# MakiseChris666/MVXNet-Makise

Hardware: AMD Instinct MI355X
Metric: KITTI frames/sec (voxelize+VFE+fusion+3Dconv fwd+bwd) (higher is better)
Workload: dtype f32 (bf16x6: three bf16 pieces = the f32 operand exactly, six MFMAs per product, f32 accumulate); 1 GPU; S2 ring frames (64-beam model, KITTI-like occupancy), 120000 raw pts -> 20000 pts after crop, grid 10x352x400, T=35, 4 frames/GPU/step: crop+cropToSight+lidar2Img, voxelize, fusion sampling+MLP, VFE, reindex+CML fwd+bwd, all-reduce, AdamW; convmath=bf16x6; mode=hot, frames_per_gpu=4, parallelism=dp1

## Files before the change

include/mvx_hip.h:

```cpp
#ifndef MVX_HIP_H
#define MVX_HIP_H
#include <stddef.h>
#include <stdint.h>

#ifdef __cplusplus
extern "C" {
#endif

#define MVX_STATS_REPLICAS 32

#define MVX_FLAG_RELU 1
#define MVX_FLAG_PREZEROED 2
#define MVX_FLAG_ACCUMULATE 4
#define MVX_FLAG_CONV2D 8
#define MVX_FLAG_TAPS2 16
#define MVX_FLAG_BG_TAPS 32
#define MVX_FLAG_SPLIT 64

#define MVX_FLAG_SPLIT3 128

#define MVX_FLAG_PRE_XCD_STRIPS 4096
#define MVX_FLAG_SPLIT_F16 512

#define MVX_FLAG_AMAX_COARSE 1024

#define MVX_FLAG_NO_BG_FILL 2048

#define MVX_OK 0
#define MVX_EINVAL (-1)
#define MVX_ESIZE (-2)

#define MVX_MAX_FRAMES 16
#define MVX_ROWS_SINGLE 0
#define MVX_ROWS_FUSION 1
#define MVX_ROWS_VFE 2
#define MVX_ROWS_VOXELS 3
#define MVX_ROWS_GRID 4
#define MVX_ROWS_REAL 5
typedef struct {
    int32_t n_frames;
    int32_t t;
    int32_t real_off[MVX_MAX_FRAMES + 1];
    int32_t vox_off[MVX_MAX_FRAMES + 1];
} mvx_frames_t;

int mvx_abi_version(void);
#define MVX_TUNE_SPLIT16_MIN_UNITS 1
#define MVX_TUNE_GATHER_NARROW_MAX_UNITS 2
#define MVX_TUNE_ROWGEMM_K128 3
int mvx_tuning_set(int32_t key, int64_t value);

int mvx_split_operand_amax(const float *amax_a, const float *amax_b);
int mvx_tensor_amax(const float *x, int64_t n, float *amax, int32_t flags, void *stream);
#define MVX_STATUS_F16_WEIGHT_RANGE 8
int mvx_split_f16_weight_check(const float *w, int64_t n, int32_t *status, void *stream);
uint64_t mvx_launch_count(void);

size_t mvx_voxelize_workspace_bytes(int32_t n_frames, int32_t cap_points);

int mvx_voxelize(const float *pcd, const int32_t *perm, const int32_t *n_points,
                 const int32_t *ext_idx, int32_t n_frames, int32_t cap_points, int32_t ncol,
                 double lo_x, double lo_y, double lo_z,
                 double size_x, double size_y, double size_z,
                 int32_t T, int32_t out_channels, int32_t cap_voxels,
                 float *voxels, int64_t *coords, int32_t *counts, int32_t *n_voxels,
                 int32_t *status, void *workspace, size_t workspace_bytes, void *stream);
int mvx_voxelize_frames(const float *pcd, const int32_t *perm, const int32_t *n_points,
                        const int32_t *ext_idx, int32_t n_frames, int32_t cap_points, int32_t ncol,
                        double lo_x, double lo_y, double lo_z,
                        double size_x, double size_y, double size_z,
                        int32_t T, int32_t out_channels, int32_t cap_voxels, int32_t concat,
                        float *voxels, int64_t *coords, int32_t *counts, int32_t *n_voxels, int32_t *vox_off,
                        int32_t *status, void *workspace, size_t workspace_bytes, void *stream);

int mvx_scatter_voxels(const float *feat, const int64_t *coords, float *grid, int32_t n_voxels,
                       int32_t channels, int32_t d, int32_t h, int32_t w, int32_t zero_grid,
                       int32_t *status, int32_t *occupancy, int32_t tile_h, int32_t tile_w,
                       uint32_t *site_bits, void *stream);
int mvx_gather_voxels(const float *grid, const int64_t *coords, float *feat, int32_t n_voxels,
// ... 219 lines not shown
                                            int32_t part, int32_t nparts, int64_t *part_rows, void *stream);
int mvx_vfe_bn_max_concat_frames(const float *y, const float *mean_inv, float *out, int32_t *argmax, int32_t n_voxels,
                                 int32_t t, int32_t channels, const int32_t *voff, const int32_t *vcnt, int32_t n_real,
                                 const mvx_frames_t *frames_host, void *stream);
int mvx_bn_segment_max_frames(const float *y, const float *mean_inv, float *out, int32_t *argmax, int32_t n_voxels,
                              int32_t t, int32_t channels, const int32_t *voff, const int32_t *vcnt, int32_t n_real,
                              const mvx_frames_t *frames_host, void *stream);
int mvx_voxel_row_offsets_frames(const int32_t *row_map, int32_t n_voxels, int32_t t, int32_t n_real, int32_t *voff,
                                 int32_t *vcnt, float *row_w, float *fusion_row_w, const mvx_frames_t *frames_host,
                                 void *stream);
int mvx_vfe_compact_input_frames(const float *voxels, int32_t vox_channels, const int32_t *rows_sel, const float *imfeat,
                                 int32_t feat_channels, int32_t n_real, int32_t n_voxels, float *out,
                                 const mvx_frames_t *frames_host, void *stream);
int mvx_vfe_compact_input_pitch_frames(const float *voxels, int32_t vox_channels, const int32_t *rows_sel, const float *imfeat,
                                       int32_t feat_channels, int32_t n_real, int32_t n_voxels, float *out, int32_t ld,
                                       const mvx_frames_t *frames_host, void *stream);
int mvx_vfe_compact_input_backward_frames(const float *grad_out, int32_t feat_channels, int32_t n_real, int32_t n_voxels,
                                          float *dimfeat, double *scratch, const mvx_frames_t *frames_host, void *stream);
int mvx_row_compact_map_frames(float *voxels, int32_t vox_channels, int64_t rows, int32_t *row_map, int32_t *rows_sel,
                               int32_t *n_real, void *workspace, size_t workspace_bytes, const mvx_frames_t *frames_host,
                               int32_t *real_off, void *stream);
int mvx_feature_sample_rows_frames(const float *voxels, int32_t vox_channels, const int32_t *rows_sel, int32_t n_real,
                                   const float *const *feats_host, const int32_t *feat_hw_host, int32_t n_levels,
                                   int32_t channels, float imsize_h, float imsize_w, float eps, float *out, int32_t *status,
                                   const mvx_frames_t *frames_host,
                                   float *out_amax , void *stream);
int mvx_feature_sample_rows_planes_frames(const float *voxels, int32_t vox_channels, const int32_t *rows_sel, int32_t n_real,
                                          const float *const *feats_host, const int32_t *feat_hw_host, int32_t n_levels,
                                          int32_t channels, float imsize_h, float imsize_w, float eps, float *out, int32_t *status,
                                          const mvx_frames_t *frames_host, float *out_amax, void *planes, int64_t plane_rows,
                                          void *stream);
size_t mvx_index_grid_bytes_frames(int32_t d, int32_t h, int32_t w, int32_t n_frames);
int mvx_index_grid_frames(const int64_t *coords, int32_t n_voxels, int32_t d, int32_t h, int32_t w, int32_t *grid,
                          int32_t *status, const mvx_frames_t *frames_host, void *stream);
int mvx_sparse_conv_output_frames(const float *p, const int32_t *index_grid, const float *bias, float *out, double *stats,
                                  int32_t din, int32_t dout, int32_t h, int32_t w, int32_t cout, int32_t stride_d,
                                  int32_t pad_d, int32_t flags, int32_t n_frames, void *stream);
int mvx_sparse_conv_output_tiles_frames(const float *p, const int32_t *index_grid, const float *bias, float *out, double *stats,
                                        int32_t din, int32_t dout, int32_t h, int32_t w, int32_t cout, int32_t stride_d,
                                        int32_t pad_d, int32_t flags, int32_t n_frames, const int32_t *tile_flags, void *stream);
int mvx_sparse_conv_gather_dz_frames(const float *dz, const int64_t *coords, int32_t n_voxels, float *g_rows, int32_t din,
                                     int32_t dout, int32_t h, int32_t w, int32_t cout, int32_t stride_d, int32_t pad_d,
                                     const mvx_frames_t *frames_host, void *stream);
int mvx_activity_dilate_frames(const void *src, int32_t src_is_index, int32_t din, int32_t dout, int32_t h, int32_t w,
                               int32_t stride_d, int32_t pad_d, int32_t mark_border, uint8_t *dst_mask,
                               int32_t *dst_halo_flags, int32_t *dst_tile_flags, int32_t n_frames, void *stream);
int mvx_tile_dilate_flags_frames(const int32_t *in_tile_flags, const int32_t *self_tile_flags, int32_t din, int32_t dout,
                                 int32_t h, int32_t w, int32_t stride_d, int32_t pad_d, int32_t *out_tile_flags,
                                 int32_t n_frames, void *stream);
int mvx_conv3d_background_frames(const float *w, const float *c_in, int32_t din, int32_t dout, int32_t cin, int32_t cout,
                                 int32_t stride_d, int32_t pad_d, float *bg_pre, int32_t n_frames, void *stream);
int mvx_bn_background_frames(const float *bg_pre, const float *bias, const float *mean_inv, int32_t planes, int32_t channels,
                             int32_t flags, float *y_bg, float *c_out, int32_t n_frames, void *stream);
int mvx_conv3d_forward_bg_frames(const float *in, const float *wpk, const float *bias, float *out, double *stats,
                                 int32_t din, int32_t dout, int32_t h, int32_t w, int32_t cin, int32_t cout,
                                 int32_t stride_d, int32_t pad_d, int32_t flags, const int32_t *in_halo_flags,
                                 const uint8_t *out_mask, const float *bg_pre, int32_t border_active, uint64_t *exec_stages,
                                 uint32_t *done_counter, double count, double eps, float *mean_inv, uint32_t *work_counter,
                                 int32_t n_frames, void *stream);
int mvx_conv3d_dgrad_tiles_frames(const float *dz, const float *wpk_dgrad, float *dx, int32_t din, int32_t dout, int32_t h,
                                  int32_t w, int32_t cin, int32_t cout, int32_t stride_d, int32_t pad_d,
                                  const int32_t *dx_tile_flags, uint64_t *exec_stages, uint32_t *work_counter,
                                  int32_t n_frames, void *stream);
int mvx_conv3d_input_grad_sums_frames(const float *w, const float *tap_sums, int32_t din, int32_t dout, int32_t cin,
                                      int32_t cout, int32_t stride_d, int32_t pad_d, float *plane_grad_sums,
                                      int32_t n_frames, void *stream);
size_t mvx_conv3d_wgrad_bg_workspace_bytes_frames(int32_t dout, int32_t h, int32_t w, int32_t cin, int32_t cout,
                                                  int32_t n_frames);
int mvx_conv3d_wgrad_bg_frames(const float *in, const float *dz, float *dw, int32_t din, int32_t dout, int32_t h, int32_t w,
                               int32_t cin, int32_t cout, int32_t stride_d, int32_t pad_d, int32_t flags,
                               const int32_t *in_halo_flags, const float *c_in, const float *tap_sums, void *workspace,
                               size_t workspace_bytes, int32_t n_frames, void *stream);
size_t mvx_bn_relu_backward_tiles_workspace_bytes_frames(int32_t planes, int32_t h, int32_t w, int32_t channels,
                                                         int32_t n_frames);
int mvx_bn_relu_backward_tiles_frames(const float *dyhat, const float *y, const float *mean_inv, const float *c_bg,
                                      const float *y_bg, const float *plane_grad_sums, const int32_t *tile_flags,
                                      int32_t planes, int32_t h, int32_t w, int32_t channels, float *dz, float *dbias,
                                      float *dz_inactive_sums, float *dz_amax ,
                                      int32_t flags, void *workspace, size_t workspace_bytes, int32_t n_frames, void *stream);
int mvx_cl_to_bev_frames(const float *cl, float *bev, int32_t d, int32_t h, int32_t w, int32_t channels, int32_t reverse,
                         int32_t n_frames, void *stream);
int mvx_bev_to_cl_broadcast(const float *bev, float *cl, int32_t d, int32_t h, int32_t w, int32_t channels, int32_t copies,
                            void *stream);

int mvx_conv2d_forward_frames(const float *in, const float *wpk, const float *bias, float *out, double *stats, int32_t h,
                              int32_t w, int32_t cin, int32_t cout, int32_t flags, uint32_t *done_counter, double eps,
                              float *mean_inv, uint32_t *work_counter, int32_t n_frames, void *stream);
int mvx_conv2d_dgrad_frames(const float *dz, const float *wpk_dgrad, float *dx, int32_t h, int32_t w, int32_t cin,
                            int32_t cout, int32_t flags, uint32_t *work_counter, int32_t n_frames, void *stream);
size_t mvx_conv2d_wgrad_workspace_bytes_frames(int32_t h, int32_t w, int32_t cin, int32_t cout, int32_t n_frames);
int mvx_conv2d_wgrad_frames(const float *in, const float *dz, float *dw, int32_t h, int32_t w, int32_t cin, int32_t cout,
                            int32_t flags, void *workspace, size_t workspace_bytes, int32_t n_frames, void *stream);
int mvx_space_to_depth_frames(const float *in, float *out, int32_t n_frames, int32_t planes, int32_t h, int32_t w,
                              int32_t channels, int32_t reverse, void *stream);
int mvx_d2s_bn_apply_frames(float *t, const float *mean_inv, float *out, int32_t n_frames, int32_t h, int32_t w, int32_t s,
                            int32_t channels, int32_t ld_out, int32_t col_offset, int32_t reverse, void *stream);
int mvx_bn_apply_strided_frames(float *y, const float *mean_inv, float *out, int64_t rows, int32_t channels, int32_t ld_out,
                                int32_t col_offset, int32_t n_frames, int32_t reverse, void *stream);
int mvx_row_stats_frames(const float *y, double *stats, int64_t rows, int32_t channels, int32_t n_frames, void *stream);

int mvx_bbox_pairwise(const float *boxes1, int32_t n1, const float *boxes2, int32_t n2, int32_t want_iou, float *out,
                      void *stream);
size_t mvx_classify_anchors_workspace_bytes(int32_t n_gt, int32_t anchors_per_loc, int32_t window_radius);
int mvx_classify_anchors(const float *gts, int32_t n_gt, const float *anchors, int32_t l, int32_t w,
                         int32_t anchors_per_loc, const int64_t *nls, const int64_t *nws, float neg_thr, float pos_thr,
                         int32_t window_radius, int64_t *pos_idx, int64_t *neg_idx, int64_t *gi, int64_t cap,
                         int32_t *counts, int32_t *status, void *workspace, size_t workspace_bytes, void *stream);
int mvx_classify_anchors_frames(const float *gts, const int32_t *gt_off_host, int32_t n_frames, const float *anchors, int32_t l,
                                int32_t w, int32_t anchors_per_loc, const int64_t *nls, const int64_t *nws, float neg_thr,
                                float pos_thr, int32_t window_radius, int64_t *pos_idx, int64_t *neg_idx, int64_t *gi,
                                int64_t cap, int32_t *counts, int32_t *status, void *workspace, size_t workspace_bytes,
                                void *stream);
size_t mvx_assign_anchors_frames_workspace_bytes(int32_t n_gt_total, int32_t n_frames, int32_t l, int32_t w,
                                                 int32_t anchors_per_loc);
int mvx_assign_anchors_frames(const float *gts, const int32_t *gt_off_host, int32_t n_frames, const float *anchors, int32_t l,
                              int32_t w, int32_t anchors_per_loc, float neg_thr, float pos_thr, float force_thr,
                              int32_t window_radius, int64_t *pos_idx, int64_t *neg_idx, int64_t *gi, int64_t cap,
                              int32_t *counts, float *gt_best, int32_t *status, void *workspace, size_t workspace_bytes,
                              void *stream);
int mvx_box_point_counts_frames(const float *points6, int32_t n_frames, int32_t cap_points, int32_t ld, const int32_t *n_points,
                                const float *boxes, const int32_t *gt_off, int32_t n_boxes_total, int32_t *counts, void *stream);
size_t mvx_ignore_anchors_frames_workspace_bytes(int32_t n_frames, int32_t l, int32_t w, int32_t anchors_per_loc);
int mvx_ignore_anchors_frames(const int64_t *pos_idx, const int64_t *neg_idx, const int64_t *gi, int64_t cap,
                              const int32_t *counts, int32_t n_frames, const int32_t *gt_off, const int32_t *gt_points,
                              int32_t min_points, const float *anchors, const float *anchor_quads, int32_t l, int32_t w,
// ... 160 lines not shown
```

mvxnet-makise_amd/csrc/activity.hip:

```cpp
#include "common.h"
#include "quad.h"

namespace {

constexpr int ATH = QTH, ATW = QTW;

__global__ void activity_sites(const void *__restrict__ src, int src_is_index, int Din, int Dout, int H, int W, int sd,
                               int pd, int mark_border, unsigned char *__restrict__ dst, int n_frames) {
    const size_t n = (size_t)n_frames * Dout * H * W;
    for (size_t e = blockIdx.x * (size_t)blockDim.x + threadIdx.x; e < n; e += (size_t)gridDim.x * blockDim.x) {
        const int x = (int)(e % W), y = (int)((e / W) % H), d = (int)(e / ((size_t)W * H));
        int on = mark_border && (y == 0 || y == H - 1 || x == 0 || x == W - 1);
        for (int kd = 0; kd < 3 && !on; ++kd) {
            const int ds = mvx_src_plane(d, Din, Dout, sd, pd, kd);
            if (ds < 0) continue;
            for (int a = -1; a <= 1 && !on; ++a) {
                const int yy = y + a;
                if (yy < 0 || yy >= H) continue;
                for (int b = -1; b <= 1; ++b) {
                    const int xx = x + b;
                    if (xx < 0 || xx >= W) continue;
                    const size_t s = ((size_t)ds * H + yy) * W + xx;
                    on |= src_is_index ? (((const int *)src)[s] >= 0) : (((const unsigned char *)src)[s] != 0);
                }
// ... 34 lines not shown
                } else {
                    const unsigned char *row = (const unsigned char *)src + s;
                    const unsigned v = *(const unsigned *)row;
                    m = ((v & 0xffu) ? 2u : 0u) | ((v & 0xff00u) ? 4u : 0u) | ((v & 0xff0000u) ? 8u : 0u) | ((v & 0xff000000u) ? 16u : 0u);
                    if (x > 0 && row[-1]) m |= 1u;
                    if (x + 4 < W && row[4]) m |= 32u;
                }
                on |= (m | (m >> 1) | (m >> 2)) & 15u;
            }
        }
        *(unsigned *)(dst + e * 4) = ((on & 1u) ? 1u : 0u) | ((on & 2u) ? 0x100u : 0u) | ((on & 4u) ? 0x10000u : 0u) | ((on & 8u) ? 0x1000000u : 0u);
    }
}

__global__ __launch_bounds__(256) void activity_halo_flags(const unsigned char *__restrict__ mask, int D, int H, int W,
                                                           int *__restrict__ flags, int *__restrict__ tile_flags) {
    const int tiles_x = (W + ATW - 1) / ATW;
    const int tx0 = (blockIdx.x % tiles_x) * ATW - 1, ty0 = (blockIdx.x / tiles_x) * ATH - 1;
    const int d = blockIdx.y;
    int on = 0, inner = 0;
    if (threadIdx.x < (ATH + 2) * (ATW + 2)) {
        const int hy = threadIdx.x / (ATW + 2), hx = threadIdx.x % (ATW + 2);
        const int y = ty0 + hy, x = tx0 + hx;
        if (y >= 0 && y < H && x >= 0 && x < W) on = mask[((size_t)d * H + y) * W + x];
        inner = on && hy >= 1 && hy <= ATH && hx >= 1 && hx <= ATW;
    }
    on = __syncthreads_or(on);
    inner = __syncthreads_or(inner);
    if (threadIdx.x == 0) {
        if (flags) flags[(size_t)d * gridDim.x + blockIdx.x] = on ? 1 : 0;
        if (tile_flags) tile_flags[(size_t)d * gridDim.x + blockIdx.x] = inner ? 1 : 0;
    }
}

__global__ void tile_dilate_flags(const int *__restrict__ in, const int *__restrict__ self, int Din, int Dout, int tiles_y,
                                  int tiles_x, int sd, int pd, int *__restrict__ out, int n_frames) {
    const int e = blockIdx.x * blockDim.x + threadIdx.x;
    const int nt = tiles_y * tiles_x;
    if (e >= n_frames * Dout * nt) return;
    const int d = e / nt, t = e - d * nt, ty = t / tiles_x, tx = t - ty * tiles_x;
    int on = self ? self[e] : 0;
    for (int kd = 0; kd < 3 && !on; ++kd) {
        const int ds = mvx_src_plane(d, Din, Dout, sd, pd, kd);
        if (ds < 0) continue;
        for (int a = -1; a <= 1 && !on; ++a)
            for (int b = -1; b <= 1; ++b) {
                const int yy = ty + a, xx = tx + b;
                if (yy >= 0 && yy < tiles_y && xx >= 0 && xx < tiles_x) on |= in[(size_t)ds * nt + yy * tiles_x + xx];
            }
    }
    out[e] = on ? 1 : 0;
}

__global__ __launch_bounds__(64) void conv_background(const float *__restrict__ w, const float *__restrict__ c_in, int Din,
                                                      int Dout, int Cin, int Cout, int sd, int pd,
                                                      float *__restrict__ bg_pre, float *__restrict__ bg_tap,
                                                      float *__restrict__ bg_cls) {
    const int n = blockIdx.x, d = blockIdx.y;
    double s = 0.0;
    double cls[9];
#pragma unroll
    for (int q = 0; q < 9; ++q) cls[q] = 0.0;
    for (int kd = 0; kd < 3; ++kd) {
        const int ds = mvx_src_plane(d, Din, Dout, sd, pd, kd);
        double sk = 0.0;
        if (ds >= 0)
            for (int e = threadIdx.x; e < Cin * 9; e += 64) {
                const int c = e / 9, k = e - c * 9, a = k / 3, b = k - a * 3;
                const double t = (double)w[(((size_t)n * Cin + c) * 3 + kd) * 9 + k] * (double)c_in[(size_t)ds * Cin + c];
                sk += t;
                if (bg_cls) {
#pragma unroll
                    for (int q = 0; q < 9; ++q) {
                        const int ry = q / 3, rx = q - ry * 3;
                        const bool inside = !(ry == 0 && a == 0) && !(ry == 2 && a == 2) && !(rx == 0 && b == 0) && !(rx == 2 && b == 2);
                        if (inside) cls[q] += t;
                    }
                }
            }
        s += sk;
        if (bg_tap) {
            sk = wave_sum_f64(sk);
            if (threadIdx.x == 0) bg_tap[((size_t)d * 3 + kd) * Cout + n] = (float)sk;
        }
    }
    s = wave_sum_f64(s);
    if (threadIdx.x == 0) bg_pre[(size_t)d * Cout + n] = (float)s;
    if (bg_cls) {
#pragma unroll
        for (int q = 0; q < 9; ++q) {
            const double v = wave_sum_f64(cls[q]);
            if (threadIdx.x == 0) bg_cls[((size_t)d * 9 + q) * Cout + n] = (float)v;
        }
    }
}

__global__ void bn_background(const float *__restrict__ bg_pre, const float *__restrict__ bias, const float *__restrict__ mi,
                              int D, int C, int relu, float *__restrict__ y_bg, float *__restrict__ c_out, int n_frames) {
    const int e = blockIdx.x * blockDim.x + threadIdx.x;
    if (e >= n_frames * D * C) return;
    const int c = e % C;
    mi += (size_t)(e / (D * C)) * 2 * C;
    float v = (bg_pre ? bg_pre[e] : 0.f) + (bias ? bias[c] : 0.f);
    if (relu) v = fmaxf(v, 0.f);
    if (y_bg) y_bg[e] = v;
    c_out[e] = (v - mi[c]) * mi[C + c];
}

__global__ __launch_bounds__(256) void bn_apply_tiles(const float *__restrict__ y, const float *__restrict__ mi,
                                                      const float *__restrict__ c_bg, const int *__restrict__ tile_flags,
                                                      float *__restrict__ out, int D, int H, int W, int C, int ntiles,
                                                      const int *__restrict__ read_flags) {
    const int t = blockIdx.x, d = blockIdx.y, frame = d / D;
    if (read_flags && !read_flags[(size_t)d * ntiles + t] && !tile_flags[(size_t)d * ntiles + t]) return;
    const TileThreads tt(C, t, W);
    const bool on = tile_flags[(size_t)d * ntiles + t] != 0;
    const float4 cb = ld4(c_bg + (size_t)d * C + tt.ct * 4);
    const float *fmi = mi + (size_t)frame * 2 * C;
    const float4 m = ld4(fmi + tt.ct * 4), iv = ld4(fmi + C + tt.ct * 4);
    tt.for_each_site([&](int, int gy, int gx) {
        if (gy >= H || gx >= W) return;
        const size_t off = (((size_t)d * H + gy) * W + gx) * C + tt.ct * 4;
        st4(out + off, on ? bn4(ld4(y + off), m, iv) : cb);
    });
}

__global__ void tile_read_flags(const int *__restrict__ hflag, int Din, int Dout, int ty_n, int tx_n, int sd, int pd,
                                int *__restrict__ read, int n_frames) {
    const int ntiles = ty_n * tx_n;
    const long long e = blockIdx.x * (long long)blockDim.x + threadIdx.x;
    if (e >= (long long)n_frames * Din * ntiles) return;
    const int p = (int)(e / ntiles), t = (int)(e - (long long)p * ntiles);
    const int ty = t / tx_n, tx = t - ty * tx_n;
    int r = 0;
    for (int kd = 0; kd < 3 && !r; ++kd) {
        const int d = mvx_dst_plane(p, Din, Dout, sd, pd, kd);
        if (d < 0) continue;
        for (int y = max(ty - 1, 0); y <= min(ty + 1, ty_n - 1) && !r; ++y)
            for (int x = max(tx - 1, 0); x <= min(tx + 1, tx_n - 1) && !r; ++x) {
                const int y0 = y & ~1, y1 = min(y0 + 1, ty_n - 1);
                const bool border = x == 0 || x == tx_n - 1 || y0 == 0 || y1 == ty_n - 1;
                int c = border ? 1 : 0;
                for (int k2 = 0; k2 < 3 && !c; ++k2) {
                    const int ds = mvx_src_plane(d, Din, Dout, sd, pd, k2);
                    if (ds >= 0) c = hflag[(size_t)ds * ntiles + y0 * tx_n + x] | hflag[(size_t)ds * ntiles + y1 * tx_n + x];
// ... 276 lines not shown
    MVX_CHECK_ARG(n_frames >= 1 && n_frames <= MVX_MAX_FRAMES);
    hipStream_t st = (hipStream_t)stream;
    const size_t n = (size_t)n_frames * dout * h * w;
    if (w % 4 == 0 && ((uintptr_t)src & 15) == 0 && ((uintptr_t)dst_mask & 3) == 0)
        hipLaunchKernelGGL(activity_sites4, dim3(mvx_cdiv(n / 4, 256) > 4096 ? 4096 : mvx_cdiv(n / 4, 256)), dim3(256), 0, st, src,
                           src_is_index, din, dout, h, w, stride_d, pad_d, mark_border, dst_mask, n_frames);
    else
        hipLaunchKernelGGL(activity_sites, dim3(mvx_cdiv(n, 256) > 4096 ? 4096 : mvx_cdiv(n, 256)), dim3(256), 0, st, src,
                           src_is_index, din, dout, h, w, stride_d, pad_d, mark_border, dst_mask, n_frames);
    MVX_LAUNCH_CHECK();
    if (dst_halo_flags || dst_tile_flags) {
        hipLaunchKernelGGL(activity_halo_flags, dim3(mvx_cdiv(w, ATW) * mvx_cdiv(h, ATH), dout * n_frames), dim3(256), 0, st,
                           (const unsigned char *)dst_mask, dout * n_frames, h, w, dst_halo_flags, dst_tile_flags);
        MVX_LAUNCH_CHECK();
    }
    return MVX_OK;
}

extern "C" int mvx_activity_dilate(const void *src, int32_t src_is_index, int32_t din, int32_t dout, int32_t h, int32_t w,
                                   int32_t stride_d, int32_t pad_d, int32_t mark_border, uint8_t *dst_mask,
                                   int32_t *dst_halo_flags, int32_t *dst_tile_flags, void *stream) {
    return mvx_activity_dilate_frames(src, src_is_index, din, dout, h, w, stride_d, pad_d, mark_border, dst_mask,
                                      dst_halo_flags, dst_tile_flags, 1, stream);
}

extern "C" int mvx_tile_dilate_flags_frames(const int32_t *in_tile_flags, const int32_t *self_tile_flags, int32_t din,
                                            int32_t dout, int32_t h, int32_t w, int32_t stride_d, int32_t pad_d,
                                            int32_t *out_tile_flags, int32_t n_frames, void *stream) {
    MVX_CHECK_ARG(in_tile_flags && out_tile_flags && din > 0 && dout > 0 && h > 0 && w > 0);
    MVX_CHECK_ARG(n_frames >= 1 && n_frames <= MVX_MAX_FRAMES);
    MVX_CHECK_ARG(stride_d >= 1 && stride_d <= 2 && pad_d >= 0 && pad_d <= 1);
    MVX_CHECK_ARG(dout == (din + 2 * pad_d - 3) / stride_d + 1);
    const int ty = (int)mvx_cdiv(h, ATH), tx = (int)mvx_cdiv(w, ATW);
    hipLaunchKernelGGL(tile_dilate_flags, dim3(mvx_cdiv((long long)n_frames * dout * ty * tx, 256)), dim3(256), 0,
                       (hipStream_t)stream, in_tile_flags, self_tile_flags, din, dout, ty, tx, stride_d, pad_d, out_tile_flags,
                       n_frames);
    MVX_LAUNCH_CHECK();
    return MVX_OK;
}

extern "C" int mvx_tile_dilate_flags(const int32_t *in_tile_flags, const int32_t *self_tile_flags, int32_t din, int32_t dout,
                                     int32_t h, int32_t w, int32_t stride_d, int32_t pad_d, int32_t *out_tile_flags,
                                     void *stream) {
    return mvx_tile_dilate_flags_frames(in_tile_flags, self_tile_flags, din, dout, h, w, stride_d, pad_d, out_tile_flags, 1,
                                        stream);
}

extern "C" int mvx_conv3d_background_frames(const float *w, const float *c_in, int32_t din, int32_t dout, int32_t cin,
                                            int32_t cout, int32_t stride_d, int32_t pad_d, float *bg_pre, int32_t n_frames,
                                            void *stream) {
    MVX_CHECK_ARG(w && c_in && bg_pre && din > 0 && dout > 0 && cin > 0 && cout > 0);
    MVX_CHECK_ARG(n_frames >= 1 && n_frames <= MVX_MAX_FRAMES);
    hipLaunchKernelGGL(conv_background, dim3(cout, dout * n_frames), dim3(64), 0, (hipStream_t)stream, w, c_in, din, dout, cin,
                       cout, stride_d, pad_d, bg_pre, (float *)nullptr, (float *)nullptr);
    MVX_LAUNCH_CHECK();
    return MVX_OK;
}

extern "C" int mvx_conv3d_background_taps_frames(const float *w, const float *c_in, int32_t din, int32_t dout, int32_t cin,
                                                 int32_t cout, int32_t stride_d, int32_t pad_d, float *bg, int32_t n_frames,
                                                 void *stream) {
    MVX_CHECK_ARG(w && c_in && bg && din > 0 && dout > 0 && cin > 0 && cout > 0);
    MVX_CHECK_ARG(n_frames >= 1 && n_frames <= MVX_MAX_FRAMES);
    hipLaunchKernelGGL(conv_background, dim3(cout, dout * n_frames), dim3(64), 0, (hipStream_t)stream, w, c_in, din, dout, cin,
                       cout, stride_d, pad_d, bg, bg + (size_t)dout * n_frames * cout, bg + (size_t)4 * dout * n_frames * cout);
    MVX_LAUNCH_CHECK();
    return MVX_OK;
}

extern "C" int mvx_conv3d_background(const float *w, const float *c_in, int32_t din, int32_t dout, int32_t cin,
                                     int32_t cout, int32_t stride_d, int32_t pad_d, float *bg_pre, void *stream) {
    return mvx_conv3d_background_frames(w, c_in, din, dout, cin, cout, stride_d, pad_d, bg_pre, 1, stream);
}

extern "C" int mvx_bn_background_frames(const float *bg_pre, const float *bias, const float *mean_inv, int32_t planes,
                                        int32_t channels, int32_t flags, float *y_bg, float *c_out, int32_t n_frames,
                                        void *stream) {
    MVX_CHECK_ARG(mean_inv && c_out && planes > 0 && channels > 0 && n_frames >= 1 && n_frames <= MVX_MAX_FRAMES);
    hipLaunchKernelGGL(bn_background, dim3(mvx_cdiv((long long)n_frames * planes * channels, 256)), dim3(256), 0,
                       (hipStream_t)stream, bg_pre, bias, mean_inv, planes, channels, flags & MVX_FLAG_RELU, y_bg, c_out, n_frames);
    MVX_LAUNCH_CHECK();
    return MVX_OK;
}

extern "C" int mvx_bn_apply_tiles_frames(const float *y, const float *mean_inv, const float *c_bg, const int32_t *tile_flags,
                                         float *out, int32_t planes, int32_t h, int32_t w, int32_t channels, int32_t n_frames,
                                         void *stream) {
    MVX_CHECK_ARG(y && mean_inv && c_bg && tile_flags && out && planes > 0 && h > 0 && w > 0);
    MVX_CHECK_ARG(channels > 0 && channels % 4 == 0 && channels <= 1024 && 256 % (channels / 4) == 0);
    MVX_CHECK_ARG(n_frames >= 1 && n_frames <= MVX_MAX_FRAMES);
    const int ntiles = (int)(mvx_cdiv(w, ATW) * mvx_cdiv(h, ATH));
    hipLaunchKernelGGL(bn_apply_tiles, dim3(ntiles, planes * n_frames), dim3(256), 0, (hipStream_t)stream, y, mean_inv, c_bg,
                       (const int *)tile_flags, out, planes, h, w, channels, ntiles, (const int *)nullptr);
    MVX_LAUNCH_CHECK();
    return MVX_OK;
}

extern "C" int mvx_bn_apply_tiles_read_frames(const float *y, const float *mean_inv, const float *c_bg, const int32_t *tile_flags,
                                              const int32_t *read_flags, float *out, int32_t planes, int32_t h, int32_t w,
                                              int32_t channels, int32_t n_frames, void *stream) {
    MVX_CHECK_ARG(y && mean_inv && c_bg && tile_flags && read_flags && out && planes > 0 && h > 0 && w > 0);
    MVX_CHECK_ARG(channels > 0 && channels % 4 == 0 && channels <= 1024 && 256 % (channels / 4) == 0);
    MVX_CHECK_ARG(n_frames >= 1 && n_frames <= MVX_MAX_FRAMES);
    const int ntiles = (int)(mvx_cdiv(w, ATW) * mvx_cdiv(h, ATH));
    hipLaunchKernelGGL(bn_apply_tiles, dim3(ntiles, planes * n_frames), dim3(256), 0, (hipStream_t)stream, y, mean_inv, c_bg,
                       (const int *)tile_flags, out, planes, h, w, channels, ntiles, (const int *)read_flags);
    MVX_LAUNCH_CHECK();
    return MVX_OK;
}

extern "C" int mvx_tile_read_flags_frames(const int32_t *in_halo_flags, int32_t din, int32_t dout, int32_t h, int32_t w,
                                          int32_t stride_d, int32_t pad_d, int32_t *read_flags, int32_t n_frames, void *stream) {
    MVX_CHECK_ARG(in_halo_flags && read_flags && din > 0 && dout > 0 && h > 0 && w > 0);
    MVX_CHECK_ARG(n_frames >= 1 && n_frames <= MVX_MAX_FRAMES && stride_d >= 1 && stride_d <= 2 && pad_d >= 0 && pad_d <= 1);
    MVX_CHECK_ARG(dout == (din + 2 * pad_d - 3) / stride_d + 1);
    const int ty = (int)mvx_cdiv(h, ATH), tx = (int)mvx_cdiv(w, ATW);
    hipLaunchKernelGGL(tile_read_flags, dim3(mvx_cdiv((long long)n_frames * din * ty * tx, 256)), dim3(256), 0, (hipStream_t)stream,
                       (const int *)in_halo_flags, din, dout, ty, tx, stride_d, pad_d, (int *)read_flags, n_frames);
// ... 22 lines not shown
```

mvxnet-makise_amd/csrc/conv3d.hip:

```cpp
#include "common.h"
#include "conv_kernels.h"

namespace {

#ifdef MVX_GATHER_STAMPS
__device__ unsigned long long g_stamps[256];
__device__ int g_stamp_unit[3] = {0, 0, 0};
__device__ volatile int g_stamp_wg = -1;
#define MVX_STAMP(k)                                                                                       \
    do {                                                                                                   \
        if (stamped && threadIdx.x == 0 && (k) < 256) g_stamps[(k)] = __builtin_amdgcn_s_memtime();        \
    } while (0)
#else
#define MVX_STAMP(k) do { } while (0)
#endif

constexpr int PITCH = BK + 4;

__global__ void pack_weights(const float *__restrict__ w, float *__restrict__ wpk, int Co, int Ci, int dgrad, int src2d) {
    const int K = dgrad ? Co : Ci, N = dgrad ? Ci : Co;
    const int nch = K / BK;
    const long long total = 27ll * K * N;
    for (long long e = blockIdx.x * (long long)blockDim.x + threadIdx.x; e < total;
         e += (long long)gridDim.x * blockDim.x) {
        const int k = (int)(e % BK);
        long long r = e / BK;
        const int n = (int)(r % N); r /= N;
        const int ch = (int)(r % nch); r /= nch;
        const int tap = (int)(r % 9);
        const int kd = (int)(r / 9);
        const int a = tap / 3, b = tap % 3;
        const int kk = ch * BK + k;
        const int co = dgrad ? kk : n, ci = dgrad ? n : kk;
        const int kh = dgrad ? 2 - a : a, kw = dgrad ? 2 - b : b;
        if (src2d) wpk[e] = kd == 1 ? w[(((long long)co * Ci + ci) * 3 + kh) * 3 + kw] : 0.f;
        else wpk[e] = w[((((long long)co * Ci + ci) * 3 + kd) * 3 + kh) * 3 + kw];
    }
}

constexpr int WROW = BN * BK;
constexpr int HROW = ((HW * PITCH + 63) / 64) * 64;

inline dim3 gather_grid(const Geom &g) { return dim3(mvx_cdiv(g.W, TW) * mvx_cdiv(g.H, TH), g.Dout * g.F, g.Cout / BN); }

template <int TLO, int THI, int NB2 = 2>
__device__ __forceinline__ void gather_unit(const int tile, const int d, const int nb, const int ntiles,
                                            float *__restrict__ s_halo, float *__restrict__ s_w, double (*s_red)[2 * BN],
                                            const float *__restrict__ in, const float *__restrict__ wpk,
                                            const float *__restrict__ bias, float *__restrict__ out,
                                            double *__restrict__ stats, const Geom &g, int relu,
                                            const int *__restrict__ in_hflag, const unsigned char *__restrict__ out_mask,
                                            const float *__restrict__ bg_pre, int border_active,
                                            unsigned long long *__restrict__ exec_stages,
                                            const int *__restrict__ only_tiles) {
    const int tiles_x = (g.W + TW - 1) / TW;
    const int tx0 = (tile % tiles_x) * TW, ty0 = (tile / tiles_x) * TH;
    const int tid = threadIdx.x, lane = tid & 63, wv = tid >> 6;
    const int li = lane & 31, lh = lane >> 5;
    const int nchunks = g.Cin / BK;
    constexpr int BNW = 32 * NB2;
    if (only_tiles && !only_tiles[(size_t)d * ntiles + tile]) return;

    f32x16 acc[1][2];
    f32x16 &acc0 = acc[0][0], &acc1 = acc[0][1];
#pragma unroll
    for (int r = 0; r < 16; ++r) { acc0[r] = 0.f; acc1[r] = 0.f; }

    const int my_ty = 2 * wv + (li >> 4), my_tx = li & 15;
    const int a_base = my_ty * HROW + my_tx * PITCH + 4 * lh;
    const int wkey = (li >> 1) & 7;
    int b_off[BK / 8];
#pragma unroll
    for (int q = 0; q < BK / 8; ++q) b_off[q] = li * BK + 4 * (((2 * q) | lh) ^ wkey);

    const bool on_border = tx0 == 0 || ty0 == 0 || tx0 + TW >= g.W || ty0 + TH >= g.H;
    const TilePlan plan = tile_plan<1>(g, d, on_border, in_hflag, border_active, ntiles, tile, tile);
    const bool active = plan.active;
    const int nstages = plan.nk * nchunks;

    if (exec_stages && active && threadIdx.x == 0 && (NB2 == 2 || !(nb & 1))) atomicAdd(exec_stages, (unsigned long long)nstages);
    if (active && nstages > 0) {

    int h_off[6];
    int h_lds[6];
#pragma unroll
    for (int u = 0; u < 6; ++u) {
        const int c = tid + 256 * u;
        h_off[u] = -1;
        h_lds[u] = -1;
        if (c < HH * HW * 8) {
            const int r = c >> 3, part = c & 7;
            const int ry = r / HW, rx = r - ry * HW;
            const int gy = ty0 - 1 + ry, gx = tx0 - 1 + rx;
            h_lds[u] = ry * HROW + rx * PITCH + part * 4;
            if (gy >= 0 && gy < g.H && gx >= 0 && gx < g.W) h_off[u] = (gy * g.W + gx) * g.Cin + part * 4;
        }
    }
    f32x4 hreg[6], wreg[6];
    auto load_halo = [&](int st) __attribute__((always_inline)) {
        int kd, ds, cc;
        plan_stage(plan, nchunks, st, kd, ds, cc);
        const float *img = in + (size_t)ds * g.H * g.W * g.Cin + cc * BK;
#pragma unroll
        for (int u = 0; u < 6; ++u)
            hreg[u] = h_off[u] >= 0 ? *(const f32x4 *)(img + h_off[u]) : f32x4{0.f, 0.f, 0.f, 0.f};
    };
    auto store_halo = [&]() __attribute__((always_inline)) {
#pragma unroll
        for (int u = 0; u < 6; ++u)
            if (h_lds[u] >= 0) *(f32x4 *)(s_halo + h_lds[u]) = hreg[u];
    };
    auto load_wrow = [&](int st, int row) __attribute__((always_inline)) {
        int kd, ds, cc;
        plan_stage(plan, nchunks, st, kd, ds, cc);
        const float *row0 = wpk + ((((size_t)kd * 9 + row * 3) * nchunks + cc) * g.Cout + (size_t)nb * BNW) * BK + (size_t)tid * 4;
        const size_t tap_stride = (size_t)nchunks * g.Cout * BK;
        if (NB2 == 2) {
#pragma unroll
            for (int v = 0; v < 6; ++v) wreg[v] = *(const f32x4 *)(row0 + (v >> 1) * tap_stride + (v & 1) * 1024);
        } else {
#pragma unroll
            for (int v = 0; v < 3; ++v) wreg[v] = *(const f32x4 *)(row0 + v * tap_stride);
        }
    };
    auto store_wrow = [&]() __attribute__((always_inline)) {
        if (NB2 == 2) {
#pragma unroll
            for (int v = 0; v < 6; ++v) {
// ... 595 lines not shown
    for (int kind = 0; kind < RK; ++kind) {
        const bool need = kind == 0 || (kind == 1 && ty0 == 0) || (kind == 2 && ty0 + TH >= H) || (kind == 3 && tx0 == 0) ||
                          (kind == 4 && tx0 + TW >= W) || (kind == 5 && ty0 == 0 && tx0 == 0) ||
                          (kind == 6 && ty0 == 0 && tx0 + TW >= W) || (kind == 7 && ty0 + TH >= H && tx0 == 0) ||
                          (kind == 8 && ty0 + TH >= H && tx0 + TW >= W);
        if (!need) continue;
        float4 s = make_float4(0.f, 0.f, 0.f, 0.f);
        for (int sidx = st; sidx < TH * TW; sidx += spb) {
            const int gy = ty0 + sidx / TW, gx = tx0 + sidx % TW;
            if (gy >= H || gx >= W) continue;
            const bool top = gy == 0, bot = gy == H - 1, lef = gx == 0, rig = gx == W - 1;
            const bool in = kind == 0 || (kind == 1 && top) || (kind == 2 && bot) || (kind == 3 && lef) || (kind == 4 && rig) ||
                            (kind == 5 && top && lef) || (kind == 6 && top && rig) || (kind == 7 && bot && lef) ||
                            (kind == 8 && bot && rig);
            if (!in) continue;
            const float4 v = *(const float4 *)(dz + (((size_t)d * H + gy) * W + gx) * C + ct * 4);
            s.x += v.x; s.y += v.y; s.z += v.z; s.w += v.w;
        }
        __syncthreads();
        red[threadIdx.x][0] = s.x; red[threadIdx.x][1] = s.y; red[threadIdx.x][2] = s.z; red[threadIdx.x][3] = s.w;
        __syncthreads();
        if (st == 0)
            for (int j = 0; j < 4; ++j) {
                double tt = 0.0;
                for (int q = 0; q < spb; ++q) tt += (double)red[q * c4n + ct][j];
                atomicAdd(Rp + (size_t)kind * C + ct * 4 + j, tt);
            }
    }
}

__global__ void region_tap_sums(const double *__restrict__ R, const float *__restrict__ extra_total, int D, int C,
                                float *__restrict__ T) {
    const int e = blockIdx.x * blockDim.x + threadIdx.x;
    if (e >= D * 9 * C) return;
    const int n = e % C, tap = (e / C) % 9, d = e / (9 * C);
    const int a = tap / 3, b = tap % 3;
    double k[RK];
    for (int q = 0; q < RK; ++q) {
        double t = 0.0;
        for (int rep = 0; rep < RREP; ++rep) t += R[(((size_t)rep * D + d) * RK + q) * C + n];
        k[q] = t;
    }
    if (extra_total) k[0] += (double)extra_total[(size_t)d * C + n];
    double t = k[0];
    if (a == 0) t -= k[1];
    if (a == 2) t -= k[2];
    if (b == 0) t -= k[3];
    if (b == 2) t -= k[4];
    if (a == 0 && b == 0) t += k[5];
    if (a == 0 && b == 2) t += k[6];
    if (a == 2 && b == 0) t += k[7];
    if (a == 2 && b == 2) t += k[8];
    T[e] = (float)t;
}

__global__ void wgrad_rank1(const float *__restrict__ T, const float *__restrict__ c_in, float *__restrict__ dw, Geom g) {
    const size_t total = (size_t)27 * g.Cin * g.Cout;
    for (size_t e = blockIdx.x * (size_t)blockDim.x + threadIdx.x; e < total; e += (size_t)gridDim.x * blockDim.x) {
        const int tap = (int)(e % 9), kd = (int)((e / 9) % 3);
        const int ci = (int)((e / 27) % g.Cin), co = (int)(e / ((size_t)27 * g.Cin));
        float s = 0.f;
        for (int d = 0; d < g.Dout * g.F; ++d) {
            const int ds = mvx_src_plane(d, g.Din, g.Dout, g.sd, g.pd, kd);
            if (ds < 0) continue;
            s += c_in[(size_t)ds * g.Cin + ci] * T[((size_t)d * 9 + tap) * g.Cout + co];
        }
        dw[e] += s;
    }
}

__global__ void wgrad_reduce(const float *__restrict__ slabs, float *__restrict__ dw, int nstrips, int Ci, int accumulate,
                             int dst2d, Strips ks, int zero_block) {
    const size_t per = (size_t)27 * Ci * BN;
    slabs += (size_t)blockIdx.y * nstrips * per;
    dw += (size_t)blockIdx.y * (dst2d ? per / 3 : per);
    for (size_t e = blockIdx.x * (size_t)blockDim.x + threadIdx.x; e < per; e += (size_t)gridDim.x * blockDim.x) {
        const int co = (int)(e % BN);
        size_t r = e / BN;
        const int ci = (int)(r % Ci); r /= Ci;
        const int tap = (int)(r % 9);
        const int kd = (int)(r / 9);
        const int nkd = kd == 0 ? ks.n[0] : (kd == 1 ? ks.n[1] : ks.n[2]);
        const int nk = nkd < nstrips ? nkd : nstrips;
        float s = 0.f;
        for (int k = 0; k < nk; ++k) s += slabs[(size_t)k * per + e];
        if (dst2d && kd != 1) continue;
        if (zero_block > 0) {
            const int ta = tap / 3, tb = tap % 3;
            if (ta > 1 || tb > 1 || !((s2d_tap_mask(ci / zero_block) >> (ta * 2 + tb)) & 1u)) s = 0.f;
        }
        float *dst = dst2d ? dw + (((size_t)co * Ci + ci) * 3 + tap / 3) * 3 + tap % 3
                           : dw + ((((size_t)co * Ci + ci) * 3 + kd) * 3 + tap / 3) * 3 + tap % 3;
        *dst = accumulate ? *dst + s : s;
    }
}

__global__ __launch_bounds__(64) void input_grad_sums(const float *__restrict__ w, const float *__restrict__ T, Geom g,
                                                      float *__restrict__ A) {
    const int c = blockIdx.x, d = blockIdx.y;
    double s = 0.0;
    for (int kd = 0; kd < 3; ++kd) {
        const int dp = mvx_dst_plane(d, g.Din, g.Dout, g.sd, g.pd, kd);
        if (dp < 0) continue;
        for (int e = threadIdx.x; e < g.Cout * 9; e += 64) {
            const int n = e / 9, k = e - n * 9;
            s += (double)w[(((size_t)n * g.Cin + c) * 3 + kd) * 9 + k] * (double)T[((size_t)dp * 9 + k) * g.Cout + n];
// ... 51 lines not shown
                               (int)grid.x, (int)grid.y, (int)grid.z);                                                            \
        else                                                                                                                     \
            hipLaunchKernelGGL((conv3d_gather_pf<TLO, THI, NB2>), grid, dim3(256), 0, st, a.in, wpk, a.bias, a.out, a.stats, g,   \
                               a.relu, a.in_hflag, a.out_mask, a.bg_pre, a.border_active, a.exec_stages, a.only_tiles,            \
                               a.done_counter, a.fin_count, a.fin_eps, a.fin_mean_inv);                                           \
    } while (0)
#define MVX_LAUNCH_GATHER(TLO, THI)                                                                                              \
    do {                                                                                                                         \
        if (narrow) MVX_LAUNCH_GATHER_N(TLO, THI, 1);                                                                            \
        else MVX_LAUNCH_GATHER_N(TLO, THI, 2);                                                                                   \
    } while (0)
    if (g.tap_lo == 0 && g.tap_hi == 3) MVX_LAUNCH_GATHER(0, 3);
    else if (g.tap_lo == 0 && g.tap_hi == 2) MVX_LAUNCH_GATHER(0, 2);
    else MVX_LAUNCH_GATHER(1, 3);
#undef MVX_LAUNCH_GATHER
#undef MVX_LAUNCH_GATHER_N
}

extern "C" void mvx_conv3d_tile_shape(int32_t *tile_h, int32_t *tile_w) {
    if (tile_h) *tile_h = TH;
    if (tile_w) *tile_w = TW;
}

extern "C" int mvx_conv3d_forward(const float *in, const float *wpk, const float *bias, float *out,
                                  double *stats, int32_t din, int32_t dout, int32_t h, int32_t w,
                                  int32_t cin, int32_t cout, int32_t stride_d, int32_t pad_d,
                                  int32_t flags, uint32_t *work_counter, void *stream) {
    MVX_CHECK_ARG(in && wpk && out);
    int rc = conv_check_forward(din, dout, h, w, cin, cout, stride_d, pad_d);
    if (rc) return rc;
    hipStream_t st = (hipStream_t)stream;
    hipError_t e = conv_zero_stats(stats, nullptr, cout, 1, flags, st);
    if (e != hipSuccess) return (int)e;
    Geom g{din, dout, h, w, cin, cout, stride_d, pad_d, 0};
    GatherArgs a;
    a.in = in; a.bias = bias; a.out = out; a.stats = stats; a.relu = flags & MVX_FLAG_RELU;
    a.work_counter = (unsigned *)work_counter;
    launch_gather(st, g, wpk, a);
    MVX_LAUNCH_CHECK();
    return MVX_OK;
}

extern "C" int mvx_conv3d_forward_bg_frames(const float *in, const float *wpk, const float *bias, float *out, double *stats,
                                            int32_t din, int32_t dout, int32_t h, int32_t w, int32_t cin, int32_t cout,
                                            int32_t stride_d, int32_t pad_d, int32_t flags, const int32_t *in_halo_flags,
                                            const uint8_t *out_mask, const float *bg_pre, int32_t border_active,
                                            uint64_t *exec_stages, uint32_t *done_counter, double count, double eps,
                                            float *mean_inv, uint32_t *work_counter, int32_t n_frames, void *stream) {
    MVX_CHECK_ARG(in && wpk && out && in_halo_flags && out_mask && bg_pre);
    int rc = conv_check_forward(din, dout, h, w, cin, cout, stride_d, pad_d);
    if (rc) return rc;
    if ((rc = conv_check_frames(n_frames))) return rc;
    MVX_CHECK_ARG(!done_counter || (stats && mean_inv && count > 0));
    hipStream_t st = (hipStream_t)stream;
    hipError_t e = conv_zero_stats(stats, done_counter, cout, n_frames, flags, st);
    if (e != hipSuccess) return (int)e;
    Geom g{din, dout, h, w, cin, cout, stride_d, pad_d, 0, n_frames};
    GatherArgs a;
    a.in = in; a.bias = bias; a.out = out; a.stats = stats; a.relu = flags & MVX_FLAG_RELU;
    a.in_hflag = in_halo_flags; a.out_mask = out_mask; a.bg_pre = bg_pre;
    a.border_active = (border_active ? 1 : 0) | ((flags & MVX_FLAG_BG_TAPS) ? 2 : 0);
    a.exec_stages = (unsigned long long *)exec_stages;
    a.done_counter = (unsigned *)done_counter; a.fin_count = count; a.fin_eps = eps; a.fin_mean_inv = mean_inv;
    a.work_counter = (unsigned *)work_counter;
    launch_gather(st, g, wpk, a);
    MVX_LAUNCH_CHECK();
    return MVX_OK;
}

extern "C" int mvx_conv3d_forward_bg(const float *in, const float *wpk, const float *bias, float *out, double *stats,
                                     int32_t din, int32_t dout, int32_t h, int32_t w, int32_t cin, int32_t cout,
                                     int32_t stride_d, int32_t pad_d, int32_t flags, const int32_t *in_halo_flags,
                                     const uint8_t *out_mask, const float *bg_pre, int32_t border_active,
                                     uint64_t *exec_stages, uint32_t *done_counter, double count, double eps,
                                     float *mean_inv, uint32_t *work_counter, void *stream) {
    return mvx_conv3d_forward_bg_frames(in, wpk, bias, out, stats, din, dout, h, w, cin, cout, stride_d, pad_d, flags,
                                        in_halo_flags, out_mask, bg_pre, border_active, exec_stages, done_counter, count, eps,
                                        mean_inv, work_counter, 1, stream);
}

static int launch_dgrad(const float *dz, const float *wpk_dgrad, float *dx, int32_t din, int32_t dout, int32_t h,
                        int32_t w, int32_t cin, int32_t cout, int32_t stride_d, int32_t pad_d, const int32_t *only_tiles,
                        uint64_t *exec_stages, uint32_t *work_counter, void *stream, int32_t n_frames = 1, int32_t flags = 0) {
    MVX_CHECK_ARG(dz && wpk_dgrad && dx);
    int rc = conv_check_frames(n_frames);
    if (rc) return rc;
    if ((rc = conv_check_geom(din, dout, h, w, cout, cin, stride_d, pad_d))) return rc;
    Geom g{dout, din, h, w, cout, cin, stride_d, pad_d, 1, n_frames};
    conv_set_taps2(g, flags, CONV_INPUT_GRAD, BN);
    GatherArgs a;
    a.in = dz; a.out = dx; a.only_tiles = only_tiles; a.exec_stages = (unsigned long long *)exec_stages;
    a.work_counter = (unsigned *)work_counter;
    launch_gather((hipStream_t)stream, g, wpk_dgrad, a);
    MVX_LAUNCH_CHECK();
    return MVX_OK;
}

extern "C" int mvx_conv3d_dgrad(const float *dz, const float *wpk_dgrad, float *dx, int32_t din,
                                int32_t dout, int32_t h, int32_t w, int32_t cin, int32_t cout,
                                int32_t stride_d, int32_t pad_d, uint32_t *work_counter, void *stream) {
    return launch_dgrad(dz, wpk_dgrad, dx, din, dout, h, w, cin, cout, stride_d, pad_d, nullptr, nullptr, work_counter, stream);
}

extern "C" int mvx_conv3d_dgrad_tiles(const float *dz, const float *wpk_dgrad, float *dx, int32_t din, int32_t dout,
                                      int32_t h, int32_t w, int32_t cin, int32_t cout, int32_t stride_d, int32_t pad_d,
                                      const int32_t *dx_tile_flags, uint64_t *exec_stages, uint32_t *work_counter,
                                      void *stream) {
    MVX_CHECK_ARG(dx_tile_flags);
    return launch_dgrad(dz, wpk_dgrad, dx, din, dout, h, w, cin, cout, stride_d, pad_d, dx_tile_flags, exec_stages,
                        work_counter, stream);
}

extern "C" int mvx_conv3d_dgrad_tiles_frames(const float *dz, const float *wpk_dgrad, float *dx, int32_t din, int32_t dout,
                                             int32_t h, int32_t w, int32_t cin, int32_t cout, int32_t stride_d, int32_t pad_d,
// ... 33 lines not shown
    const int per = wgrad_strips(h, w, cin);
    const int nstrips = (conv_ntiles(h, w) + per - 1) / per;
    MVX_CHECK_ARG(workspace_bytes >= mvx_conv3d_wgrad_workspace_bytes(h, w, cin, cout));
    Geom g{din, dout, h, w, cin, cout, stride_d, pad_d, 0};
    hipStream_t st = (hipStream_t)stream;
    if (cin % W4_C == 0)
        launch_wgrad4<false>(flags, dim3(nstrips, 3 * (cin / W4_C), nblk), st, in, dz, (float *)workspace, g, per, nullptr, nullptr,
                             nullptr, Strips{{nstrips, nstrips, nstrips}}, am);
    else
        hipLaunchKernelGGL(conv3d_wgrad, dim3(nstrips, 3 * (cin / BK)), dim3(WG_THREADS), 0, st, in, dz,
                           (float *)workspace, g, per);
    MVX_LAUNCH_CHECK();
    const size_t per_slab = (size_t)27 * cin * BN;
    hipLaunchKernelGGL(wgrad_reduce, dim3(mvx_cdiv(per_slab, 256), nblk), dim3(256), 0, st, (const float *)workspace, dw,
                       nstrips, cin, flags & MVX_FLAG_ACCUMULATE, (flags & MVX_FLAG_CONV2D) ? 1 : 0,
                       Strips{{nstrips, nstrips, nstrips}}, 0);
    MVX_LAUNCH_CHECK();
    return MVX_OK;
}

static int wgrad_bg_strips(int cin) {
    const int s = 128 / (cin / W4_C);
    return s < 1 ? 1 : s;
}
static size_t wgrad_bg_slab_bytes(int cin) { return (size_t)wgrad_bg_strips(cin) * 27 * cin * BN * sizeof(float); }

extern "C" size_t mvx_plane_tap_sums_workspace_bytes(int32_t planes, int32_t channels) {
    return planes > 0 && channels > 0 ? sizeof(double) * RREP * planes * RK * channels : 0;
}

extern "C" int mvx_plane_tap_sums(const float *dz, int32_t planes, int32_t h, int32_t w, int32_t channels,
                                  const int32_t *tile_flags, const float *inactive_sums, float *tap_sums,
                                  void *workspace, size_t workspace_bytes, void *stream) {
    MVX_CHECK_ARG(dz && tap_sums && workspace && planes > 0 && h > 0 && w > 0 && channels > 0);
    MVX_CHECK_ARG(channels % 4 == 0 && 256 % (channels / 4) == 0);
    MVX_CHECK_ARG((tile_flags == nullptr) == (inactive_sums == nullptr));
    MVX_CHECK_ARG(workspace_bytes >= mvx_plane_tap_sums_workspace_bytes(planes, channels));
    hipStream_t st = (hipStream_t)stream;
    double *R = (double *)workspace;
    hipError_t e = hipMemsetAsync(R, 0, sizeof(double) * RREP * planes * RK * channels, st);
    if (e != hipSuccess) return (int)e;
    if (tile_flags)
        hipLaunchKernelGGL(plane_region_sums_tiles, dim3(conv_ntiles(h, w), planes), dim3(256), 0, st, dz,
                           tile_flags, planes, h, w, channels, R);
    else
        hipLaunchKernelGGL(plane_region_sums, dim3(h, planes), dim3(256), 0, st, dz, planes, h, w, channels, R);
    MVX_LAUNCH_CHECK();
    hipLaunchKernelGGL(region_tap_sums, dim3(mvx_cdiv((long long)planes * 9 * channels, 64)), dim3(64), 0, st,
                       (const double *)R, inactive_sums, planes, channels, tap_sums);
    MVX_LAUNCH_CHECK();
    return MVX_OK;
}

extern "C" int mvx_conv3d_input_grad_sums_frames(const float *w, const float *tap_sums, int32_t din, int32_t dout, int32_t cin,
                                                 int32_t cout, int32_t stride_d, int32_t pad_d, float *plane_grad_sums,
                                                 int32_t n_frames, void *stream) {
    MVX_CHECK_ARG(w && tap_sums && plane_grad_sums && din > 0 && dout > 0 && cin > 0 && cout > 0);
    if (int rc = conv_check_frames(n_frames)) return rc;
    Geom g{din, dout, 0, 0, cin, cout, stride_d, pad_d, 0, n_frames};
    hipLaunchKernelGGL(input_grad_sums, dim3(cin, din * n_frames), dim3(64), 0, (hipStream_t)stream, w, tap_sums, g,
                       plane_grad_sums);
    MVX_LAUNCH_CHECK();
    return MVX_OK;
}

extern "C" int mvx_conv3d_input_grad_sums(const float *w, const float *tap_sums, int32_t din, int32_t dout, int32_t cin,
                                          int32_t cout, int32_t stride_d, int32_t pad_d, float *plane_grad_sums,
                                          void *stream) {
    return mvx_conv3d_input_grad_sums_frames(w, tap_sums, din, dout, cin, cout, stride_d, pad_d, plane_grad_sums, 1, stream);
}

extern "C" size_t mvx_conv3d_wgrad_bg_workspace_bytes_frames(int32_t dout, int32_t h, int32_t w, int32_t cin, int32_t cout,
                                                            int32_t n_frames) {
    if (dout <= 0 || h <= 0 || w <= 0 || cin <= 0 || cout != BN || cin % W4_C || n_frames <= 0) return 0;
    return conv_carve_wgrad(nullptr, wgrad_bg_slab_bytes(cin), dout * n_frames, conv_ntiles(h, w), false).bytes;
}

extern "C" size_t mvx_conv3d_wgrad_bg_workspace_bytes(int32_t dout, int32_t h, int32_t w, int32_t cin, int32_t cout) {
    return mvx_conv3d_wgrad_bg_workspace_bytes_frames(dout, h, w, cin, cout, 1);
}

extern "C" int mvx_conv3d_wgrad_bg_frames(const float *in, const float *dz, float *dw, int32_t din, int32_t dout, int32_t h,
                                          int32_t w, int32_t cin, int32_t cout, int32_t stride_d, int32_t pad_d, int32_t flags,
                                          const int32_t *in_halo_flags, const float *c_in, const float *tap_sums,
                                          void *workspace, size_t workspace_bytes, int32_t n_frames, void *stream) {
    const SplitAmax am = mvxi_take_split_amax();
    MVX_CHECK_ARG(in && dz && dw && workspace && in_halo_flags && c_in && tap_sums);
    int rc = conv_check_geom(din, dout, h, w, cin, cout, stride_d, pad_d);
    if (rc) return rc;
    if (cout != BN || cin % W4_C) return MVX_ESIZE;
    if ((rc = conv_check_frames(n_frames))) return rc;
    const int ntiles = conv_ntiles(h, w);
    const WgradWorkspace ws = conv_carve_wgrad(workspace, wgrad_bg_slab_bytes(cin), dout * n_frames, ntiles, false);
    MVX_CHECK_ARG(workspace_bytes >= ws.bytes);
    const int nstrips = wgrad_bg_strips(cin);
    Geom g{din, dout, h, w, cin, cout, stride_d, pad_d, 0, n_frames};
    hipStream_t st = (hipStream_t)stream;
    int nd[3], ndsum = 0;
    for (int kd = 0; kd < 3; ++kd) {
        nd[kd] = 0;
        for (int d = 0; d < dout; ++d) {
            const int ds = d * stride_d - pad_d + kd;
            nd[kd] += ds >= 0 && ds < din;
        }
        ndsum += nd[kd];
    }
    Strips ks;
    int widest = 1;
    for (int kd = 0; kd < 3; ++kd) {
        int share = ndsum > 0 ? (2 * nstrips * nd[kd]) / ndsum : nstrips;
        if (share < 1) share = 1;
        if (share > nstrips) share = nstrips;
        ks.n[kd] = share;
        if (share > widest) widest = share;
    }
    hipLaunchKernelGGL(wgrad_step_list, dim3(3), dim3(1024), 0, st, in_halo_flags, g, ntiles, ws.list, ws.count);
    MVX_LAUNCH_CHECK();
    launch_wgrad4<false>(flags, dim3(widest, 3 * (cin / W4_C)), st, in, dz, ws.slabs, g, 0, ws.list, ws.count, c_in, ks, am);
    MVX_LAUNCH_CHECK();
    const size_t per_slab = (size_t)27 * cin * BN;
    hipLaunchKernelGGL(wgrad_reduce, dim3(mvx_cdiv(per_slab, 256)), dim3(256), 0, st, (const float *)ws.slabs, dw, widest, cin,
                       flags & MVX_FLAG_ACCUMULATE, 0, ks, 0);
    MVX_LAUNCH_CHECK();
    hipLaunchKernelGGL(wgrad_rank1, dim3(mvx_cdiv(per_slab, 256)), dim3(256), 0, st, tap_sums, c_in, dw, g);
    MVX_LAUNCH_CHECK();
    return MVX_OK;
}

extern "C" int mvx_conv3d_wgrad_bg(const float *in, const float *dz, float *dw, int32_t din, int32_t dout, int32_t h,
                                   int32_t w, int32_t cin, int32_t cout, int32_t stride_d, int32_t pad_d, int32_t flags,
                                   const int32_t *in_halo_flags, const float *c_in, const float *tap_sums,
                                   void *workspace, size_t workspace_bytes, void *stream) {
    return mvx_conv3d_wgrad_bg_frames(in, dz, dw, din, dout, h, w, cin, cout, stride_d, pad_d, flags, in_halo_flags, c_in,
                                      tap_sums, workspace, workspace_bytes, 1, stream);
}

extern "C" int mvx_conv2d_forward_frames(const float *in, const float *wpk, const float *bias, float *out, double *stats,
                                         int32_t h, int32_t w, int32_t cin, int32_t cout, int32_t flags,
                                         uint32_t *done_counter, double eps, float *mean_inv, uint32_t *work_counter,
                                         int32_t n_frames, void *stream) {
    MVX_CHECK_ARG(in && wpk && out);
    int rc = conv_check_frames(n_frames);
    if (rc) return rc;
    if ((rc = conv_check_geom(1, 1, h, w, cin, cout, 1, 1))) return rc;
    MVX_CHECK_ARG(!done_counter || (stats && mean_inv));
    hipStream_t st = (hipStream_t)stream;
    hipError_t e = conv_zero_stats(stats, done_counter, cout, n_frames, flags, st);
    if (e != hipSuccess) return (int)e;
    Geom g{1, 1, h, w, cin, cout, 1, 1, 0, n_frames};
    conv_set_taps2(g, flags, CONV_FORWARD, BK);
    GatherArgs a;
    a.in = in; a.bias = bias; a.out = out; a.stats = stats; a.relu = flags & MVX_FLAG_RELU;
    a.done_counter = (unsigned *)done_counter; a.fin_count = (double)h * w; a.fin_eps = eps; a.fin_mean_inv = mean_inv;
    a.work_counter = (unsigned *)work_counter;
    launch_gather(st, g, wpk, a);
    MVX_LAUNCH_CHECK();
    return MVX_OK;
}

extern "C" int mvx_conv2d_dgrad_frames(const float *dz, const float *wpk_dgrad, float *dx, int32_t h, int32_t w, int32_t cin,
                                       int32_t cout, int32_t flags, uint32_t *work_counter, int32_t n_frames, void *stream) {
    return launch_dgrad(dz, wpk_dgrad, dx, 1, 1, h, w, cin, cout, 1, 1, nullptr, nullptr, work_counter, stream, n_frames, flags);
}

static int conv2d_wgrad_strips(int cin, int cout) {
    int s = 256 / ((cin / W4_C) * (cout / BN));
    if (s > 128) s = 128;
    return s < 1 ? 1 : s;
}

static size_t conv2d_wgrad_slab_bytes(int cin, int cout) {
    return (size_t)(cout / BN) * conv2d_wgrad_strips(cin, cout) * 27 * cin * BN * sizeof(float);
}

extern "C" size_t mvx_conv2d_wgrad_workspace_bytes_frames(int32_t h, int32_t w, int32_t cin, int32_t cout, int32_t n_frames) {
    if (h <= 0 || w <= 0 || cin <= 0 || cout <= 0 || cin % W4_C || cout % BN || n_frames <= 0) return 0;
    return conv_carve_wgrad(nullptr, conv2d_wgrad_slab_bytes(cin, cout), n_frames, conv_ntiles(h, w), true).bytes;
}

// ... 37 lines not shown
```

mvxnet-makise_amd/csrc/conv3d_split.hip:

```cpp
#include "common.h"
#include "conv_kernels.h"
#include "rowgemm_common.h"

namespace {

constexpr int TH2 = 16;

__global__ void pack_weights_split(const float *__restrict__ w, unsigned short *__restrict__ wsp, int Co, int Ci, int dgrad, int np, int fmt) {
    const int K = dgrad ? Co : Ci, N = dgrad ? Ci : Co;
    const int nch = K / BK;
    const long long total = 27ll * K * N;
    for (long long e = blockIdx.x * (long long)blockDim.x + threadIdx.x; e < total; e += (long long)gridDim.x * blockDim.x) {
        const int k = (int)(e % BK);
        long long r = e / BK;
        const int n = (int)(r % N); r /= N;
        const int ch = (int)(r % nch); r /= nch;
        const int tap = (int)(r % 9);
        const int kd = (int)(r / 9);
        const int a = tap / 3, b = tap % 3;
        const int kk = ch * BK + k;
        const int co = dgrad ? kk : n, ci = dgrad ? n : kk;
        const int kh = dgrad ? 2 - a : a, kw = dgrad ? 2 - b : b;
        float x = w[((((long long)co * Ci + ci) * 3 + kd) * 3 + kh) * 3 + kw];
        const long long row = (((long long)kd * 9 + tap) * nch + ch) * N + n;
        for (int q = 0; q < np; ++q) {
            if (fmt == 0) {
                const __bf16 pb = (__bf16)x;
                wsp[(row * np + q) * BK + k] = __builtin_bit_cast(unsigned short, pb);
                x -= (float)pb;
            } else {
                if (q == 0) x *= SPLIT_F16_WSCALE;
                const _Float16 pb = (_Float16)x;
                wsp[(row * np + q) * BK + k] = __builtin_bit_cast(unsigned short, pb);
                x -= (float)pb;
            }
        }
    }
}

template <int NP, int BKT, int MT, bool WIN, int FMT>
__global__ __launch_bounds__(256, 2) void conv3d_gather_splitT(const float *__restrict__ in,
                                                               const unsigned short *__restrict__ wsp,
                                                               const float *__restrict__ bias,
                                                               float *__restrict__ out, double *__restrict__ stats,
                                                               Geom g, int relu, const int *__restrict__ in_hflag,
                                                               const unsigned char *__restrict__ out_mask,
                                                               const float *__restrict__ bg_pre, int border_active,
                                                               const int *__restrict__ only_tiles,
                                                               unsigned long long *__restrict__ exec_stages,
                                                               const float *__restrict__ in_amax) {
    float a_scale = 1.f;
    if constexpr (FMT == 1) a_scale = split_scale_of(in_amax);
    constexpr int THT = TH * MT, HHT = THT + 2;
    constexpr int ROWBT = NP * BKT * 2 + 16;
    constexpr int HROW = (HW * ROWBT + 255) / 256 * 256;
    constexpr int PPR = NP * BKT / 8;
    constexpr int PT = BN * PPR;
    constexpr int NWU = (3 * PT + 255) / 256;
    constexpr int PARTS = BKT / 4;
    constexpr int NH = (HHT * HW * PARTS + 255) / 256;
    constexpr int KS = BKT / 16;
    __shared__ __attribute__((aligned(256))) unsigned char s_halo[HHT * HROW];
    __shared__ __attribute__((aligned(16))) unsigned char s_w[3][BN * ROWBT];
    __shared__ float s_red[4][2 * BN];
    const int tiles_x = (g.W + TW - 1) / TW, tiles_y8 = (g.H + TH - 1) / TH;
    const int ntiles8 = tiles_x * tiles_y8;
    const int tx = blockIdx.x % tiles_x, tyb = blockIdx.x / tiles_x;
    const int tx0 = tx * TW, ty0 = tyb * THT;
    const int t_top = (MT * tyb) * tiles_x + tx;
    const bool has_bot = MT == 2 && 2 * tyb + 1 < tiles_y8;
    const int t_bot = has_bot ? t_top + tiles_x : t_top;
    const int d = blockIdx.y, nb = blockIdx.z;
    const int tid = threadIdx.x, lane = tid & 63, wv = tid >> 6, li = lane & 31, lh = lane >> 5;
    const int nchunks = g.Cin / BKT;
    if (only_tiles && !(only_tiles[(size_t)d * ntiles8 + t_top] | only_tiles[(size_t)d * ntiles8 + t_bot])) return;
    const bool on_border = tx0 == 0 || ty0 == 0 || tx0 + TW >= g.W || ty0 + THT >= g.H;
    const TilePlan plan = tile_plan<MT>(g, d, on_border, in_hflag, border_active, ntiles8, t_top, t_bot);

    f32x16 acc[MT][2];
#pragma unroll
    for (int m = 0; m < MT; ++m)
#pragma unroll
        for (int n = 0; n < 2; ++n)
#pragma unroll
            for (int r = 0; r < 16; ++r) acc[m][n][r] = 0.f;
    int a_base[MT];
#pragma unroll
    for (int m = 0; m < MT; ++m) a_base[m] = (2 * MT * wv + 2 * m + (li >> 4)) * HROW + (li & 15) * ROWBT + lh * 16;
    const int b_base = li * ROWBT + lh * 16;

    typedef unsigned u32x4 __attribute__((ext_vector_type(4)));
    u32x4 wreg[NWU];
    auto load_w3 = [&](int kd, int a, int cc) __attribute__((always_inline)) {
        const int c32 = (cc * BKT) / BK, half = BKT == 16 ? (cc & 1) : 0;
#pragma unroll
        for (int u = 0; u < NWU; ++u) {
            int c = tid + 256 * u;
            if (3 * PT % 256 && c >= 3 * PT) c = 3 * PT - 1;
            const int t = c / PT, rem = c - t * PT;
            const int n = rem / PPR, piece = rem - n * PPR;
            const int q = piece / (BKT / 8), sub = piece - q * (BKT / 8);
            const unsigned char *row = (const unsigned char *)wsp +
                (((((size_t)kd * 9 + a * 3 + t) * (g.Cin / BK) + c32) * g.Cout + (size_t)nb * BN + n) * NP + q) * (BK * 2);
            wreg[u] = *(const u32x4 *)(row + half * 32 + sub * 16);
        }
    };
    auto store_w3 = [&]() __attribute__((always_inline)) {
#pragma unroll
        for (int u = 0; u < NWU; ++u) {
            const int c = tid + 256 * u;
            if (3 * PT % 256 == 0 || c < 3 * PT) {
                const int t = c / PT, rem = c - t * PT;
                const int n = rem / PPR, piece = rem - n * PPR;
                *(u32x4 *)(s_w[t] + n * ROWBT + piece * 16) = wreg[u];
            }
        }
    };

    const int nstages = plan.active ? plan.nk * nchunks : 0;
    if (exec_stages && nstages > 0 && threadIdx.x == 0)
        atomicAdd(exec_stages, (unsigned long long)(plan.nk * (g.Cin / BK)) * (has_bot ? 2 : 1));
    int h_off[NH], h_lds[NH];
#pragma unroll
    for (int u = 0; u < NH; ++u) {
        const int c = tid + 256 * u;
        h_off[u] = -1;
        h_lds[u] = -1;
        if (c < HHT * HW * PARTS) {
            const int r = c / PARTS, part = c - r * PARTS;
// ... 166 lines not shown
                               a.stats, g, a.relu, a.in_hflag, a.out_mask, a.bg_pre, a.border_active, a.only_tiles,                  \
                               a.exec_stages, am.a);                                                                                 \
    } while (0)
    if (fmt_of(flags)) { if (big) MVX_GO(2, 32, 2, 1); else MVX_GO(2, 32, 1, 1); }
    else if (pieces_of(flags) == 3) { if (big) MVX_GO(3, 16, 2, 0); else MVX_GO(3, 32, 1, 0); }
    else              { if (big) MVX_GO(2, 32, 2, 0); else MVX_GO(2, 32, 1, 0); }
#undef MVX_GO
}

}

extern "C" size_t mvx_conv3d_packed_weight_bytes_split(int32_t cout, int32_t cin, int32_t flags) {
    if (cout <= 0 || cin <= 0) return 0;
    return (size_t)27 * cout * cin * pieces_of(flags) * sizeof(unsigned short);
}

extern "C" int mvx_conv3d_pack_weights_split(const float *w, void *wsplit, int32_t cout, int32_t cin, int32_t for_dgrad,
                                             int32_t flags, void *stream) {
    MVX_CHECK_ARG(w && wsplit && cout > 0 && cin > 0);
    MVX_CHECK_ARG((for_dgrad ? cout : cin) % BK == 0);
    const long long total = 27ll * cout * cin;
    hipLaunchKernelGGL(pack_weights_split, dim3(mvx_cdiv(total, 256) > 2048 ? 2048 : mvx_cdiv(total, 256)), dim3(256), 0,
                       (hipStream_t)stream, w, (unsigned short *)wsplit, cout, cin, for_dgrad, pieces_of(flags), fmt_of(flags));
    MVX_LAUNCH_CHECK();
    return MVX_OK;
}

extern "C" int mvx_conv3d_forward_split(const float *in, const void *wsplit, const float *bias, float *out, double *stats,
                                        int32_t din, int32_t dout, int32_t h, int32_t w, int32_t cin, int32_t cout,
                                        int32_t stride_d, int32_t pad_d, int32_t flags, void *stream) {
    MVX_CHECK_ARG(in && wsplit && out);
    int rc = conv_check_forward(din, dout, h, w, cin, cout, stride_d, pad_d);
    if (rc) return rc;
    hipStream_t st = (hipStream_t)stream;
    hipError_t e = conv_zero_stats(stats, nullptr, cout, 1, flags, st);
    if (e != hipSuccess) return (int)e;
    Geom g{din, dout, h, w, cin, cout, stride_d, pad_d, 0};
    GatherArgs a;
    a.in = in; a.bias = bias; a.out = out; a.stats = stats; a.relu = flags & MVX_FLAG_RELU;
    launch_gather_split(st, flags, g, (const unsigned short *)wsplit, a);
    MVX_LAUNCH_CHECK();
    return MVX_OK;
}

extern "C" int mvx_conv3d_forward_bg_split_frames(const float *in, const void *wsplit, const float *bias, float *out,
                                                  double *stats, int32_t din, int32_t dout, int32_t h, int32_t w, int32_t cin,
                                                  int32_t cout, int32_t stride_d, int32_t pad_d, int32_t flags,
                                                  const int32_t *in_halo_flags, const uint8_t *out_mask, const float *bg_pre,
                                                  int32_t border_active, uint64_t *exec_stages, int32_t n_frames, void *stream) {
    MVX_CHECK_ARG(in && wsplit && out && in_halo_flags && out_mask && bg_pre);
    int rc = conv_check_frames(n_frames);
    if (rc) return rc;
    if ((rc = conv_check_forward(din, dout, h, w, cin, cout, stride_d, pad_d))) return rc;
    hipStream_t st = (hipStream_t)stream;
    hipError_t e = conv_zero_stats(stats, nullptr, cout, n_frames, flags, st);
    if (e != hipSuccess) return (int)e;
    Geom g{din, dout, h, w, cin, cout, stride_d, pad_d, 0, n_frames};
    GatherArgs a;
    a.in = in; a.bias = bias; a.out = out; a.stats = stats; a.relu = flags & MVX_FLAG_RELU;
    a.in_hflag = in_halo_flags; a.out_mask = out_mask; a.bg_pre = bg_pre;
    a.border_active = (border_active ? 1 : 0) | ((flags & MVX_FLAG_BG_TAPS) ? 2 : 0);
    a.exec_stages = (unsigned long long *)exec_stages;
    launch_gather_split(st, flags, g, (const unsigned short *)wsplit, a);
    MVX_LAUNCH_CHECK();
    return MVX_OK;
}

extern "C" int mvx_conv3d_forward_bg_split(const float *in, const void *wsplit, const float *bias, float *out, double *stats,
                                           int32_t din, int32_t dout, int32_t h, int32_t w, int32_t cin, int32_t cout,
                                           int32_t stride_d, int32_t pad_d, int32_t flags, const int32_t *in_halo_flags,
                                           const uint8_t *out_mask, const float *bg_pre, int32_t border_active,
                                           void *stream) {
    return mvx_conv3d_forward_bg_split_frames(in, wsplit, bias, out, stats, din, dout, h, w, cin, cout, stride_d, pad_d, flags,
                                              in_halo_flags, out_mask, bg_pre, border_active, nullptr, 1, stream);
}

static int launch_dgrad_split(const float *dz, const void *wsplit_dgrad, float *dx, int32_t din, int32_t dout, int32_t h,
                              int32_t w, int32_t cin, int32_t cout, int32_t stride_d, int32_t pad_d, int32_t flags,
                              const int32_t *only_tiles, uint64_t *exec_stages, int32_t n_frames, void *stream) {
    MVX_CHECK_ARG(dz && wsplit_dgrad && dx);
    int rc = conv_check_frames(n_frames);
    if (rc) return rc;
    if ((rc = conv_check_geom(din, dout, h, w, cout, cin, stride_d, pad_d))) return rc;
    Geom g{dout, din, h, w, cout, cin, stride_d, pad_d, 1, n_frames};
    conv_set_taps2(g, flags, CONV_INPUT_GRAD, BN);
    GatherArgs a;
    a.in = dz; a.out = dx; a.only_tiles = only_tiles; a.exec_stages = (unsigned long long *)exec_stages;
    launch_gather_split((hipStream_t)stream, flags, g, (const unsigned short *)wsplit_dgrad, a);
    MVX_LAUNCH_CHECK();
    return MVX_OK;
}

extern "C" int mvx_conv3d_dgrad_tiles_split_frames(const float *dz, const void *wsplit_dgrad, float *dx, int32_t din,
                                                   int32_t dout, int32_t h, int32_t w, int32_t cin, int32_t cout,
                                                   int32_t stride_d, int32_t pad_d, int32_t flags,
                                                   const int32_t *dx_tile_flags, uint64_t *exec_stages, int32_t n_frames,
                                                   void *stream) {
    MVX_CHECK_ARG(dx_tile_flags);
    return launch_dgrad_split(dz, wsplit_dgrad, dx, din, dout, h, w, cin, cout, stride_d, pad_d, flags, dx_tile_flags,
                              exec_stages, n_frames, stream);
}

extern "C" int mvx_conv3d_dgrad_tiles_split(const float *dz, const void *wsplit_dgrad, float *dx, int32_t din, int32_t dout,
                                            int32_t h, int32_t w, int32_t cin, int32_t cout, int32_t stride_d,
                                            int32_t pad_d, int32_t flags, const int32_t *dx_tile_flags, void *stream) {
    MVX_CHECK_ARG(dx_tile_flags);
    return launch_dgrad_split(dz, wsplit_dgrad, dx, din, dout, h, w, cin, cout, stride_d, pad_d, flags, dx_tile_flags, nullptr, 1,
                              stream);
}

extern "C" int mvx_conv3d_dgrad_split(const float *dz, const void *wsplit_dgrad, float *dx, int32_t din, int32_t dout,
                                      int32_t h, int32_t w, int32_t cin, int32_t cout, int32_t stride_d, int32_t pad_d,
                                      int32_t flags, void *stream) {
    return launch_dgrad_split(dz, wsplit_dgrad, dx, din, dout, h, w, cin, cout, stride_d, pad_d, flags, nullptr, nullptr, 1, stream);
// ... 26 lines not shown
```

mvxnet-makise_amd/csrc/conv_geom.h:

```cpp
#pragma once
#include "common.h"

namespace {

constexpr int TH = 8, TW = 16;
constexpr int HH = TH + 2, HW = TW + 2;
constexpr int BK = 32;
constexpr int BN = 64;

struct Geom {
    int Din, Dout, H, W, Cin, Cout;
    int sd, pd;
    int mode;
    int F = 1;
    int tap_lo = 0, tap_hi = 3;
    int s2d = 0;
};

__device__ __forceinline__ unsigned s2d_tap_mask(int p) {
    const int pr = p >> 1, pc = p & 1;
    unsigned m = 8u;
    if (pr) m |= 2u;
    if (pc) m |= 4u;
    if (pr && pc) m |= 1u;
    return m;
}

__device__ __forceinline__ int src_depth(const Geom &g, int d, int kd) {
    if (g.mode == 0) return mvx_src_plane(d, g.Din, g.Dout, g.sd, g.pd, kd);
    return mvx_dst_plane(d, g.Dout, g.Din, g.sd, g.pd, kd);
}

static inline int conv_check_geom(int32_t din, int32_t dout, int32_t h, int32_t w, int32_t cin, int32_t cout, int32_t sd,
                                  int32_t pd) {
    MVX_CHECK_ARG(din > 0 && dout > 0 && h > 0 && w > 0 && cin > 0 && cout > 0);
    MVX_CHECK_ARG(sd >= 1 && sd <= 2 && pd >= 0 && pd <= 1);
    if (cin % BK || cout % BN) {
        mvxi_drop_split_amax();
        return MVX_ESIZE;
    }
    return MVX_OK;
}

static inline int conv_check_forward(int32_t din, int32_t dout, int32_t h, int32_t w, int32_t cin, int32_t cout, int32_t sd,
                                     int32_t pd) {
    const int rc = conv_check_geom(din, dout, h, w, cin, cout, sd, pd);
    if (rc) return rc;
    MVX_CHECK_ARG(dout == (din + 2 * pd - 3) / sd + 1);
    return MVX_OK;
}

static inline int conv_check_frames(int32_t n_frames) {
    MVX_CHECK_ARG(n_frames >= 1 && n_frames <= MVX_MAX_FRAMES);
    return MVX_OK;
}

static inline int conv_ntiles(int32_t h, int32_t w) { return (int)(mvx_cdiv(w, TW) * mvx_cdiv(h, TH)); }

static inline hipError_t conv_zero_stats(double *stats, uint32_t *done_counter, int32_t cout, int32_t n_frames, int32_t flags,
                                         hipStream_t st) {
    if (flags & MVX_FLAG_PREZEROED) return hipSuccess;
    if (stats) {
        const hipError_t e = hipMemsetAsync(stats, 0, sizeof(double) * MVX_REP * 2 * cout * n_frames, st);
        if (e != hipSuccess) return e;
    }
    return done_counter ? hipMemsetAsync(done_counter, 0, sizeof(uint32_t), st) : hipSuccess;
}

enum ConvDir { CONV_FORWARD, CONV_INPUT_GRAD, CONV_WEIGHT_GRAD };
static inline void conv_set_taps2(Geom &g, int32_t flags, ConvDir dir, int granule) {
    if (!(flags & MVX_FLAG_TAPS2)) return;
    g.tap_lo = dir == CONV_INPUT_GRAD ? 1 : 0;
    g.tap_hi = g.tap_lo + 2;
    const int c = dir == CONV_INPUT_GRAD ? g.Cout : g.Cin;
    if (c % 4 == 0 && (c / 4) % granule == 0) g.s2d = c / 4;
}

struct GatherArgs {
    const float *in = nullptr, *bias = nullptr;
    float *out = nullptr;
    double *stats = nullptr;
    int relu = 0;
    const int *in_hflag = nullptr;
    const unsigned char *out_mask = nullptr;
    const float *bg_pre = nullptr;
    int border_active = 0;
    const int *only_tiles = nullptr;
    unsigned long long *exec_stages = nullptr;
    unsigned *done_counter = nullptr;
    double fin_count = 0.0, fin_eps = 0.0;
    float *fin_mean_inv = nullptr;
    unsigned *work_counter = nullptr;
};

struct WgradWorkspace {
    float *slabs;
    int *list, *count, *ones;
    size_t bytes;
};
static inline WgradWorkspace conv_carve_wgrad(void *workspace, size_t slab_bytes, int planes, int ntiles, bool with_ones) {
    const size_t steps = (size_t)planes * ntiles;
    WgradWorkspace c{nullptr, nullptr, nullptr, nullptr, slab_bytes + sizeof(int) * (3 * steps + 4 + (with_ones ? steps : 0))};
    if (workspace) {
        c.slabs = (float *)workspace;
        c.list = (int *)((char *)workspace + slab_bytes);
        c.count = c.list + 3 * steps;
// ... 7 lines not shown
```

mvxnet-makise_amd/csrc/conv_kernels.h:

```cpp
#pragma once
#include "conv_geom.h"
#include "split_common.h"

namespace {

struct TilePlan {
    int kd[3], ds[3], nk;
    unsigned skipped;
    bool active;
    bool idle_border;
};

template <int NT>
__device__ __forceinline__ TilePlan tile_plan(const Geom &g, const int d, const bool on_border,
                                              const int *__restrict__ in_hflag, const int border_active, const int ntiles,
                                              const int t0, const int t1) {
    TilePlan p{{0, 0, 0}, {0, 0, 0}, 0, 0u, true, false};
    const bool skip_taps = in_hflag && (border_active & 2) && !on_border;
    int any_flag = 0;
#pragma unroll
    for (int kd = 0; kd < 3; ++kd) {
        const int ds = src_depth(g, d, kd);
        if (ds >= 0) {
            int fl = 1;
            if (in_hflag) {
                fl = in_hflag[(size_t)ds * ntiles + t0];
                if (NT == 2) fl |= in_hflag[(size_t)ds * ntiles + t1];
            }
            any_flag |= fl;
            if (skip_taps && !fl) { p.skipped |= 1u << kd; continue; }
            if (p.nk == 0) { p.kd[0] = kd; p.ds[0] = ds; }
            else if (p.nk == 1) { p.kd[1] = kd; p.ds[1] = ds; }
            else { p.kd[2] = kd; p.ds[2] = ds; }
            ++p.nk;
        }
    }
    p.idle_border = in_hflag && (border_active & 2) && on_border && !any_flag;
    if (p.idle_border) p.nk = 0;
    if (in_hflag) p.active = (((border_active & 1) && on_border) || any_flag) != 0;
    return p;
}

__device__ __forceinline__ void plan_stage(const TilePlan &p, const int nchunks, const int st, int &kd, int &ds, int &cc) {
    const int i = st / nchunks;
    cc = st - i * nchunks;
    const int k0 = p.kd[0], k1 = p.kd[1], k2 = p.kd[2], s0 = p.ds[0], s1 = p.ds[1], s2 = p.ds[2];
    kd = i == 0 ? k0 : (i == 1 ? k1 : k2);
    ds = i == 0 ? s0 : (i == 1 ? s1 : s2);
}

template <int MT, int NB2, typename S>
__device__ __forceinline__ void gather_epilogue(f32x16 (&acc)[MT][2], const TilePlan &p, const Geom &g, const int d,
                                                const int nb, const int tx0, const int ty0, const unsigned unit,
                                                S (*s_red)[2 * BN], const float *__restrict__ bias,
                                                float *__restrict__ out, double *__restrict__ stats, const int relu,
                                                const unsigned char *__restrict__ out_mask,
                                                const float *__restrict__ bg_pre) {
    const int tid = threadIdx.x, lane = tid & 63, wv = tid >> 6, li = lane & 31, lh = lane >> 5;
    constexpr int BNW = 32 * NB2;
    const int n0 = nb * BNW + li, n1 = NB2 == 2 ? n0 + 32 : n0;
    const float bias0 = bias ? bias[n0] : 0.f, bias1 = bias ? bias[n1] : 0.f;
    float skip0 = 0.f, skip1 = 0.f;
    if (p.skipped && p.active) {
        const float *bg_tap = bg_pre + (size_t)g.Dout * g.F * g.Cout + (size_t)d * 3 * g.Cout;
#pragma unroll
        for (int kd = 0; kd < 3; ++kd)
            if ((p.skipped >> kd) & 1u) { skip0 += bg_tap[kd * g.Cout + n0]; skip1 += bg_tap[kd * g.Cout + n1]; }
    }
    float bgv0 = (bg_pre ? bg_pre[(size_t)d * g.Cout + n0] : 0.f) + bias0, bgv1 = (bg_pre ? bg_pre[(size_t)d * g.Cout + n1] : 0.f) + bias1;
    if (relu) { bgv0 = fmaxf(bgv0, 0.f); bgv1 = fmaxf(bgv1, 0.f); }
    S s1a = 0, s2a = 0, s1b = 0, s2b = 0;
#pragma unroll
    for (int m = 0; m < MT; ++m) {
        const int py = ty0 + 2 * MT * wv + 2 * m;
        if (p.idle_border) {
            const float *bg_cls = bg_pre + (size_t)4 * g.Dout * g.F * g.Cout + (size_t)d * 9 * g.Cout;
#pragma unroll
            for (int r = 0; r < 16; ++r) {
                const int row = mfma32_row(r) + 4 * lh;
                const int gy = py + (row >> 4), gx = tx0 + (row & 15);
                const int q = 3 * (gy == 0 ? 0 : (gy >= g.H - 1 ? 2 : 1)) + (gx == 0 ? 0 : (gx >= g.W - 1 ? 2 : 1));
                acc[m][0][r] = bg_cls[q * g.Cout + n0];
                acc[m][1][r] = bg_cls[q * g.Cout + n1];
            }
        }
        unsigned site_on = p.active ? 0xffffu : 0u;
        if (out_mask && p.active) {
            unsigned char mk[16];
#pragma unroll
            for (int r = 0; r < 16; ++r) {
                const int row = mfma32_row(r) + 4 * lh;
                const int gy = min(py + (row >> 4), g.H - 1), gx = min(tx0 + (row & 15), g.W - 1);
                mk[r] = out_mask[((size_t)d * g.H + gy) * g.W + gx];
            }
            site_on = 0u;
#pragma unroll
            for (int r = 0; r < 16; ++r) site_on |= (mk[r] ? 1u : 0u) << r;
        }
#pragma unroll
        for (int r = 0; r < 16; ++r) {
            const int row = mfma32_row(r) + 4 * lh;
            const int gy = py + (row >> 4), gx = tx0 + (row & 15);
            float v0 = (acc[m][0][r] + skip0) + bias0, v1 = (acc[m][1][r] + skip1) + bias1;
            if (relu) { v0 = fmaxf(v0, 0.f); v1 = fmaxf(v1, 0.f); }
            if (out_mask && !((site_on >> r) & 1u)) { v0 = bgv0; v1 = bgv1; }
            if (gy < g.H && gx < g.W) {
                float *o = out + (((size_t)d * g.H + gy) * g.W + gx) * g.Cout;
                o[n0] = v0;
                if (NB2 == 2) o[n1] = v1;
                s1a += (S)v0; s2a += (S)v0 * (S)v0;
                s1b += (S)v1; s2b += (S)v1 * (S)v1;
            }
        }
    }
    if (stats) {
        s1a += __shfl_xor(s1a, 32, 64); s2a += __shfl_xor(s2a, 32, 64);
        s1b += __shfl_xor(s1b, 32, 64); s2b += __shfl_xor(s2b, 32, 64);
        __syncthreads();
        if (lh == 0) {
            s_red[wv][li] = s1a; s_red[wv][32 + li] = s1b;
            s_red[wv][BN + li] = s2a; s_red[wv][BN + 32 + li] = s2b;
        }
        __syncthreads();
        if (tid < 2 * BNW) {
            const int which = tid / BNW, c = tid % BNW, j = which * BN + c;
            const double t = (double)s_red[0][j] + (double)s_red[1][j] + (double)s_red[2][j] + (double)s_red[3][j];
            const unsigned rep = unit % MVX_REP;
            double *fstats = stats + (size_t)(d / g.Dout) * MVX_REP * 2 * g.Cout;
            atomicAdd(fstats + ((size_t)rep * 2 + which) * g.Cout + nb * BNW + c, t);
        }
    }
}

struct Strips { int n[3]; };
constexpr int W4_THREADS = 512;
constexpr int W4_C = 64;
constexpr int W4_NX = (HH * HW * 16 + W4_THREADS - 1) / W4_THREADS;
constexpr int W4_NZ = TH * TW * 16 / W4_THREADS;

__host__ __device__ constexpr int w4_own(bool t2, int grp, int i) {
    return t2 ? (grp == 0 ? (i < 3 ? i : i + 2) : (i < 2 ? i + 3 : (i < 4 ? i + 5 : -1)))
              : (grp == 0 ? i : (i < 4 ? i + 5 : -1));
}
__host__ __device__ constexpr int w4_ncomp(bool t2, int grp) { return t2 ? 2 : (grp == 0 ? 5 : 4); }

struct W4Walk {
    int tiles_x, ntiles, kd, cc, strip, nstrips;
    int dlo, per, nsteps;
    const int *list;

    __device__ __forceinline__ bool init(const Geom &g, const int tiles_per_strip, const int *__restrict__ step_list,
                                         const int *__restrict__ step_count, const Strips &ks) {
        tiles_x = (g.W + TW - 1) / TW;
        ntiles = tiles_x * ((g.H + TH - 1) / TH);
        const int nchunks = g.Cin / W4_C;
        kd = blockIdx.y / nchunks, cc = blockIdx.y % nchunks;
        strip = blockIdx.x, nstrips = step_list ? (kd == 0 ? ks.n[0] : (kd == 1 ? ks.n[1] : ks.n[2])) : (int)gridDim.x;
        if (strip >= nstrips) return false;
        int dhi = -1;
        dlo = 0;
        for (int d = 0; d < g.Dout; ++d) {
            const int ds = d * g.sd - g.pd + kd;
            if (ds >= 0 && ds < g.Din) { if (dhi < 0) dlo = d; dhi = d; }
        }
        const int nd = dhi >= dlo ? dhi - dlo + 1 : 0;
        per = tiles_per_strip;
        list = step_list ? step_list + (size_t)kd * g.Dout * g.F * ntiles : nullptr;
        const int nlist = step_list ? step_count[kd] : 0;
        nsteps = step_list ? (nlist > strip ? (nlist - strip + nstrips - 1) / nstrips : 0) : nd * per;
        return true;
    }
    __device__ __forceinline__ void step_of(const int i, int &d, int &t) const {
        if (list) { const int e = list[strip + i * nstrips]; d = e / ntiles; t = e - d * ntiles; }
        else { d = dlo + i / per; t = strip * per + i % per; }
    }
    __device__ __forceinline__ int next_live(int i) const {
        if (list) return i < nsteps ? i : nsteps;
        while (i < nsteps && strip * per + i % per >= ntiles) ++i;
        return i < nsteps ? i : nsteps;
    }
    __device__ __forceinline__ void load_step(const int i, const Geom &g, const float *__restrict__ in,
                                              const float *__restrict__ dz, const float *__restrict__ c_in,
                                              f32x4 (&xr)[W4_NX], f32x4 (&zr)[W4_NZ]) const {
        const int tid = threadIdx.x;
        int d, t;
        step_of(i, d, t);
        const int ds = mvx_src_plane(d, g.Din, g.Dout, g.sd, g.pd, kd);
        const int tx0 = (t % tiles_x) * TW, ty0 = (t / tiles_x) * TH;
#pragma unroll
        for (int u = 0; u < W4_NX; ++u) {
            const int c = tid + W4_THREADS * u;
            f32x4 v = {0.f, 0.f, 0.f, 0.f};
            if (c < HH * HW * 16) {
                const int r = c >> 4, part = c & 15;
                const int gy = ty0 - 1 + r / HW, gx = tx0 - 1 + r % HW;
                if (gy >= 0 && gy < g.H && gx >= 0 && gx < g.W) {
                    v = *(const f32x4 *)(in + (((size_t)ds * g.H + gy) * g.W + gx) * g.Cin + cc * W4_C + part * 4);
                    if (c_in) v -= *(const f32x4 *)(c_in + (size_t)ds * g.Cin + cc * W4_C + part * 4);
                }
            }
            xr[u] = v;
        }
#pragma unroll
        for (int u = 0; u < W4_NZ; ++u) {
            const int c = tid + W4_THREADS * u;
            const int r = c >> 4, part = c & 15;
            const int gy = ty0 + (r >> 4), gx = tx0 + (r & 15);
            f32x4 v = {0.f, 0.f, 0.f, 0.f};
            if (gy < g.H && gx < g.W)
                v = *(const f32x4 *)(dz + (((size_t)d * g.H + gy) * g.W + gx) * g.Cout + part * 4);
            zr[u] = v;
        }
    }
};

template <bool T2>
__device__ __forceinline__ unsigned w4_slots(const Geom &g, const int cc, const int grp) {
    if (!(T2 && g.s2d > 0)) return 0x1fu;
    const unsigned m = s2d_tap_mask((cc * W4_C) / g.s2d);
    return grp == 0 ? (m & 3u) : ((m >> 2) & 3u);
}

template <bool T2>
__device__ __forceinline__ void w4_store_slabs(const f32x16 (&acc)[5], float *__restrict__ slabs, const W4Walk &wk,
                                               const Geom &g, const float o_scale) {
    const int lane = threadIdx.x & 63, wv = threadIdx.x >> 6, li = lane & 31, lh = lane >> 5;
    const int grp = wv >> 2, wm = (wv >> 1) & 1, wn = wv & 1;
#pragma unroll
    for (int i = 0; i < 5; ++i) {
        const int t9 = grp == 0 ? w4_own(T2, 0, i) : w4_own(T2, 1, i);
        if (t9 < 0) continue;
        float *o = slabs + ((((size_t)wk.strip * 3 + wk.kd) * 9 + t9) * g.Cin + wk.cc * W4_C + wm * 32) * BN + wn * 32;
#pragma unroll
        for (int r = 0; r < 16; ++r) {
            const int row = mfma32_row(r) + 4 * lh;
            o[(size_t)row * BN + li] = acc[i][r] * o_scale;
        }
    }
}

}
```

mvxnet-makise_amd/modules/Extension.py:

```python
import ctypes
import os

import numpy as np
import torch

_HERE = os.path.dirname(os.path.abspath(__file__))
LIB_PATH = os.environ.get('MVX_HIP_LIB', os.path.join(os.path.dirname(_HERE), 'lib', 'libmvx_hip.so'))
ABI_VERSION = 10

_p = ctypes.c_void_p
_i32 = ctypes.c_int32
_i64 = ctypes.c_int64
_f64 = ctypes.c_double
_f32 = ctypes.c_float
_sz = ctypes.c_size_t

PROTOTYPES = {
    'mvx_abi_version': (_i32, []),
    'mvx_tuning_set': (_i32, [_i32, _i64]),
    'mvx_launch_count': (ctypes.c_uint64, []),
    'mvx_voxelize_workspace_bytes': (_sz, [_i32, _i32]),
    'mvx_voxelize': (_i32, [_p, _p, _p, _p, _i32, _i32, _i32, _f64, _f64, _f64, _f64, _f64, _f64,
                            _i32, _i32, _i32, _p, _p, _p, _p, _p, _p, _sz, _p]),
    'mvx_voxelize_frames': (_i32, [_p, _p, _p, _p, _i32, _i32, _i32, _f64, _f64, _f64, _f64, _f64, _f64,
# ... 56 lines not shown
                                     _i32, _p, _p, _f64, _f64, _p, _p, _p]),
    'mvx_linear_forward_bn': (_i32, [_p, _i32, _p, _i32, _i32, _p, _p, _i32, _p, _p, _i64, _i32, _i32, _i32, _p, _f64, _f64, _p, _p]),
    'mvx_conv3d_wgrad_bg_workspace_bytes': (_sz, [_i32, _i32, _i32, _i32, _i32]),
    'mvx_conv3d_wgrad_bg': (_i32, [_p, _p, _p, _i32, _i32, _i32, _i32, _i32, _i32, _i32, _i32, _i32, _p, _p, _p, _p, _sz, _p]),
    'mvx_conv3d_forward_bg_split': (_i32, [_p, _p, _p, _p, _p, _i32, _i32, _i32, _i32, _i32, _i32, _i32, _i32, _i32, _p, _p, _p,
                                           _i32, _p]),
    'mvx_conv3d_dgrad_tiles_split': (_i32, [_p, _p, _p, _i32, _i32, _i32, _i32, _i32, _i32, _i32, _i32, _i32, _p, _p]),
    'mvx_conv3d_forward_bg_split_frames': (_i32, [_p, _p, _p, _p, _p, _i32, _i32, _i32, _i32, _i32, _i32, _i32, _i32, _i32, _p, _p,
                                                  _p, _i32, _p, _i32, _p]),
    'mvx_conv3d_dgrad_tiles_split_frames': (_i32, [_p, _p, _p, _i32, _i32, _i32, _i32, _i32, _i32, _i32, _i32, _i32, _p, _p, _i32, _p]),
    'mvx_conv2d_forward_split_frames': (_i32, [_p, _p, _p, _p, _p, _i32, _i32, _i32, _i32, _i32, _i32, _p]),
    'mvx_conv2d_dgrad_split_frames': (_i32, [_p, _p, _p, _i32, _i32, _i32, _i32, _i32, _i32, _p]),
    'mvx_plane_tap_sums_workspace_bytes': (_sz, [_i32, _i32]),
    'mvx_plane_tap_sums': (_i32, [_p, _i32, _i32, _i32, _i32, _p, _p, _p, _p, _sz, _p]),
    'mvx_tile_dilate_flags': (_i32, [_p, _p, _i32, _i32, _i32, _i32, _i32, _i32, _p, _p]),
    'mvx_conv3d_input_grad_sums': (_i32, [_p, _p, _i32, _i32, _i32, _i32, _i32, _i32, _p, _p]),
    'mvx_conv3d_dgrad_tiles': (_i32, [_p, _p, _p, _i32, _i32, _i32, _i32, _i32, _i32, _i32, _i32, _p, _p, _p, _p]),
    'mvx_bn_relu_backward_tiles_workspace_bytes': (_sz, [_i32, _i32, _i32, _i32]),
    'mvx_bn_relu_backward_tiles': (_i32, [_p, _p, _p, _p, _p, _p, _p, _i32, _i32, _i32, _i32, _p, _p, _p, _i32, _p, _sz, _p]),
    'mvx_linear_forward_bn_frames': (_i32, [_p, _i32, _p, _i32, _i32, _p, _p, _i32, _p, _p, _i64, _i32, _i32, _i32, _p, _f64, _p, _p, _i32, _p]),
    'mvx_bn_finalize_frames': (_i32, [_p, _f64, _f64, _p, _i32, _i32, _p]),
    'mvx_bn_apply_frames': (_i32, [_p, _p, _p, _i64, _i32, _p, _i32, _p]),
    'mvx_bn_backward_scratch_bytes_frames': (_sz, [_i32, _i32]),
    'mvx_split_operand_amax': (_i32, [_p, _p]),
    'mvx_tensor_amax': (_i32, [_p, _i64, _p, _i32, _p]),
    'mvx_split_f16_weight_check': (_i32, [_p, _i64, _p, _p]),
    'mvx_bn_relu_backward_frames': (_i32, [_p, _p, _p, _f64, _p, _p, _p, _p, _i64, _i32, _i32, _p, _i32, _p, _p]),
    'mvx_bn_relu_backward_planes_frames': (_i32, [_p, _p, _p, _f64, _p, _p, _p, _p, _i64, _i32, _i32, _p, _i32, _p, _p]),
    'mvx_bn_relu_backward_planes_part_frames': (_i32, [_p, _p, _p, _f64, _p, _p, _p, _p, _i64, _i32, _i32, _p, _i32, _i32, _i32, _p,
                                                       _p]),
    'mvx_vfe_bn_max_concat_frames': (_i32, [_p, _p, _p, _p, _i32, _i32, _i32, _p, _p, _i32, _p, _p]),
    'mvx_bn_segment_max_frames': (_i32, [_p, _p, _p, _p, _i32, _i32, _i32, _p, _p, _i32, _p, _p]),
    'mvx_voxel_row_offsets_frames': (_i32, [_p, _i32, _i32, _i32, _p, _p, _p, _p, _p, _p]),
    'mvx_vfe_compact_input_frames': (_i32, [_p, _i32, _p, _p, _i32, _i32, _i32, _p, _p, _p]),
    'mvx_vfe_compact_input_pitch_frames': (_i32, [_p, _i32, _p, _p, _i32, _i32, _i32, _p, _i32, _p, _p]),
    'mvx_vfe_compact_input_backward_frames': (_i32, [_p, _i32, _i32, _i32, _p, _p, _p, _p]),
    'mvx_row_compact_map_frames': (_i32, [_p, _i32, _i64, _p, _p, _p, _p, _sz, _p, _p, _p]),
    'mvx_feature_sample_rows_frames': (_i32, [_p, _i32, _p, _i32, _p, _p, _i32, _i32, _f32, _f32, _f32, _p, _p, _p, _p, _p]),
    'mvx_feature_sample_rows_planes_frames': (_i32, [_p, _i32, _p, _i32, _p, _p, _i32, _i32, _f32, _f32, _f32, _p, _p, _p, _p, _p,
                                                     _i64, _p]),
    'mvx_index_grid_bytes_frames': (_sz, [_i32, _i32, _i32, _i32]),
    'mvx_index_grid_frames': (_i32, [_p, _i32, _i32, _i32, _i32, _p, _p, _p, _p]),
    'mvx_sparse_conv_output_frames': (_i32, [_p, _p, _p, _p, _p, _i32, _i32, _i32, _i32, _i32, _i32, _i32, _i32, _i32, _p]),
    'mvx_sparse_conv_output_tiles_frames': (_i32, [_p, _p, _p, _p, _p, _i32, _i32, _i32, _i32, _i32, _i32, _i32, _i32, _i32, _p, _p]),
    'mvx_sparse_conv_gather_dz_frames': (_i32, [_p, _p, _i32, _p, _i32, _i32, _i32, _i32, _i32, _i32, _i32, _p, _p]),
    'mvx_activity_dilate_frames': (_i32, [_p, _i32, _i32, _i32, _i32, _i32, _i32, _i32, _i32, _p, _p, _p, _i32, _p]),
    'mvx_tile_dilate_flags_frames': (_i32, [_p, _p, _i32, _i32, _i32, _i32, _i32, _i32, _p, _i32, _p]),
    'mvx_conv3d_background_frames': (_i32, [_p, _p, _i32, _i32, _i32, _i32, _i32, _i32, _p, _i32, _p]),
    'mvx_bn_apply_tiles_frames': (_i32, [_p, _p, _p, _p, _p, _i32, _i32, _i32, _i32, _i32, _p]),
    'mvx_bn_apply_tiles_bev_frames': (_i32, [_p, _p, _p, _p, _p, _i32, _i32, _i32, _i32, _i32, _p]),
    'mvx_bn_apply_tiles_read_frames': (_i32, [_p, _p, _p, _p, _p, _p, _i32, _i32, _i32, _i32, _i32, _p]),
    'mvx_tile_read_flags_frames': (_i32, [_p, _i32, _i32, _i32, _i32, _i32, _i32, _p, _i32, _p]),
    'mvx_conv3d_background_taps_frames': (_i32, [_p, _p, _i32, _i32, _i32, _i32, _i32, _i32, _p, _i32, _p]),
    'mvx_bn_background_frames': (_i32, [_p, _p, _p, _i32, _i32, _i32, _p, _p, _i32, _p]),
    'mvx_conv3d_forward_bg_frames': (_i32, [_p, _p, _p, _p, _p, _i32, _i32, _i32, _i32, _i32, _i32, _i32, _i32, _i32, _p, _p, _p,
                                            _i32, _p, _p, _f64, _f64, _p, _p, _i32, _p]),
    'mvx_conv3d_dgrad_tiles_frames': (_i32, [_p, _p, _p, _i32, _i32, _i32, _i32, _i32, _i32, _i32, _i32, _p, _p, _p, _i32, _p]),
    'mvx_conv3d_input_grad_sums_frames': (_i32, [_p, _p, _i32, _i32, _i32, _i32, _i32, _i32, _p, _i32, _p]),
    'mvx_conv3d_wgrad_bg_workspace_bytes_frames': (_sz, [_i32, _i32, _i32, _i32, _i32, _i32]),
    'mvx_conv3d_wgrad_bg_frames': (_i32, [_p, _p, _p, _i32, _i32, _i32, _i32, _i32, _i32, _i32, _i32, _i32, _p, _p, _p, _p, _sz, _i32, _p]),
    'mvx_bn_relu_backward_tiles_workspace_bytes_frames': (_sz, [_i32, _i32, _i32, _i32, _i32]),
    'mvx_bn_relu_backward_tiles_frames': (_i32, [_p, _p, _p, _p, _p, _p, _p, _i32, _i32, _i32, _i32, _p, _p, _p, _p, _i32, _p, _sz, _i32, _p]),
    'mvx_cl_to_bev_frames': (_i32, [_p, _p, _i32, _i32, _i32, _i32, _i32, _i32, _p]),
    'mvx_bev_to_cl_broadcast': (_i32, [_p, _p, _i32, _i32, _i32, _i32, _i32, _p]),
    'mvx_conv2d_forward_frames': (_i32, [_p, _p, _p, _p, _p, _i32, _i32, _i32, _i32, _i32, _p, _f64, _p, _p, _i32, _p]),
    'mvx_conv2d_dgrad_frames': (_i32, [_p, _p, _p, _i32, _i32, _i32, _i32, _i32, _p, _i32, _p]),
    'mvx_conv2d_wgrad_workspace_bytes_frames': (_sz, [_i32, _i32, _i32, _i32, _i32]),
    'mvx_conv2d_wgrad_frames': (_i32, [_p, _p, _p, _i32, _i32, _i32, _i32, _i32, _p, _sz, _i32, _p]),
    'mvx_space_to_depth_frames': (_i32, [_p, _p, _i32, _i32, _i32, _i32, _i32, _i32, _p]),
    'mvx_d2s_bn_apply_frames': (_i32, [_p, _p, _p, _i32, _i32, _i32, _i32, _i32, _i32, _i32, _i32, _p]),
    'mvx_bn_apply_strided_frames': (_i32, [_p, _p, _p, _i64, _i32, _i32, _i32, _i32, _i32, _p]),
    'mvx_row_stats_frames': (_i32, [_p, _p, _i64, _i32, _i32, _p]),
    'mvx_bbox_pairwise': (_i32, [_p, _i32, _p, _i32, _i32, _p, _p]),
    'mvx_classify_anchors_workspace_bytes': (_sz, [_i32, _i32, _i32]),
    'mvx_classify_anchors': (_i32, [_p, _i32, _p, _i32, _i32, _i32, _p, _p, _f32, _f32, _i32, _p, _p, _p, _i64, _p, _p, _p, _sz, _p]),
    'mvx_classify_anchors_frames': (_i32, [_p, _p, _i32, _p, _i32, _i32, _i32, _p, _p, _f32, _f32, _i32, _p, _p, _p, _i64, _p, _p, _p, _sz, _p]),
    'mvx_assign_anchors_frames_workspace_bytes': (_sz, [_i32, _i32, _i32, _i32, _i32]),
    'mvx_assign_anchors_frames': (_i32, [_p, _p, _i32, _p, _i32, _i32, _i32, _f32, _f32, _f32, _i32, _p, _p, _p, _i64, _p, _p, _p, _p,
                                         _sz, _p]),
    'mvx_box_point_counts_frames': (_i32, [_p, _i32, _i32, _i32, _p, _p, _p, _i32, _p, _p]),
    'mvx_ignore_anchors_frames_workspace_bytes': (_sz, [_i32, _i32, _i32, _i32]),
    'mvx_ignore_anchors_frames': (_i32, [_p, _p, _p, _i64, _p, _i32, _p, _p, _i32, _p, _p, _i32, _i32, _i32, _p, _p, _p, _p, _p, _f32,
                                         _p, _p, _p, _i64, _p, _p, _p, _p, _sz, _p]),
    'mvx_voxel_loss': (_i32, [_p, _i64, _i64, _i64, _p, _i64, _i64, _i64, _p, _i64, _p, _i64, _p, _p, _i32, _i32, _p, _i32, _p,
                              _i32, _i32, _i32, _f32, _f32, _f32, _p, _i64, _i64, _i64, _p, _i64, _i64, _i64, _p, _p, _p]),
    'mvx_focal_loss_frames_workspace_bytes': (_i64, [_i32, _i32, _i32, _i32]),
    'mvx_focal_loss_frames': (_i32, [_p, _i32, _i32, _i32, _i32, _p, _p, _p, _i64, _p, _p, _i32, _p, _p, _f32, _f32, _f32, _f32,
                                     _p, _p, _p, _i64, _p]),
    'mvx_focal_loss_dir_frames_workspace_bytes': (_i64, [_i32, _i32, _i32, _i32, _i32]),
    'mvx_focal_loss_dir_frames': (_i32, [_p, _i32, _p, _i32, _i32, _i32, _i32, _i32, _p, _p, _p, _i64, _p, _p, _i32, _p, _p, _f32, _f32,
                                         _f32, _f32, _f32, _f32, _p, _i32, _p, _i32, _p, _p, _i64, _p]),
    'mvx_detect_workspace_bytes': (_sz, [_i32, _i32, _i32]),
    'mvx_detect_frames': (_i32, [_p, _i64, _i64, _i64, _i64, _p, _i64, _i64, _i64, _i64, _p, _i32, _i32, _i32, _i32, _f32, _f32, _i32,
                                 _i32, _i32, _p, _p, _p, _p, _p, _p, _p, _p, _p, _p, _sz, _p]),
    'mvx_detect_frames_dir': (_i32, [_p, _i64, _i64, _i64, _i64, _p, _i64, _i64, _i64, _i64, _p, _i64, _i64, _i64, _i64, _f32, _p, _i32,
                                     _i32, _i32, _i32, _f32, _f32, _i32, _i32, _i32, _p, _p, _p, _p, _p, _p, _p, _p, _p, _p, _sz, _p]),
    'mvx_kitti_eval_workspace_bytes': (_sz, [_i32, _i32]),
    'mvx_kitti_eval_overlaps': (_i32, [_i32, _p, _p, _p, _p, _p, _p, _p, _p, _p, _p, _p]),
    'mvx_kitti_eval_tp_scores': (_i32, [_i32, _p, _p, _p, _i32, _p, _p, _i32, _p, _p, _p, _p, _p, _p, _p]),
    'mvx_kitti_eval_thresholds': (_i32, [_i32, _i32, _i64, _p, _p, _p, _p, _p, _p]),
    'mvx_kitti_eval_counts': (_i32, [_i32, _p, _p, _p, _i32, _p, _p, _i32, _p, _p, _p, _p, _p, _p, _p, _p, _p, _p, _p, _p,
                                     _sz, _p]),
    'mvx_gt_paste_workspace_bytes': (_sz, [_i32, _i32, _i32]),
    'mvx_gt_paste_ground_frames': (_i32, [_p, _p, _i32, _i32, _f64, _f64, _f64, _f64, _f64, _i32, _i32, _p, _sz, _p]),
    'mvx_gt_paste_place_frames': (_i32, [_p, _i32, _i32, _f32, _f32, _f32, _f32, _f32, _p, _p, _p, _p, _i32, _i32, _i32, _p, _p, _i32,
                                         _i32, _p, _p, _p, _i32, _p, _p, _p, _p, _p, _p]),
    'mvx_gt_paste_points_frames': (_i32, [_p, _p, _p, _i32, _i32, _p, _i32, _p, _p, _i32, _p, _p]),
    'mvx_gt_paste_image_frames': (_i32, [_p, _i32, _i32, _i32, _p, _i32, _p, _p, _p, _p, _i32, _i64, _p]),
    'mvx_geom_workspace_bytes': (_sz, [_i32, _i32]),
    'mvx_geom_place_frames': (_i32, [_p, _p, _i32, _i32, _p, _i32, _p, _f32, _p, _p, _p, _p, _p, _p, _p, _p, _p]),
    'mvx_geom_points_frames': (_i32, [_p, _p, _i32, _i32, _p, _p, _i32, _p, _p, _p, _p, _p, _p, _p, _sz, _p]),
    'mvx_gtdb_workspace_bytes': (_sz, [_i32, _i32]),
    'mvx_gtdb_match': (_i32, [_p, _p, _p, _i32, _p, _p, _i32, _p, _i32, _f32, _p, _p, _p, _p, _p, _p]),
# ... 180 lines not shown
```

mvxnet-makise_amd/modules/_hip.py:

```python
import collections
import ctypes
import math
import os

import torch

from modules import Extension as X

VoxelizeResult = collections.namedtuple('VoxelizeResult', 'voxels coords counts n_voxels status')

_ws_cache = {}
STATS_REPLICAS = 32
FLAG_RELU, FLAG_PREZEROED, FLAG_ACCUMULATE, FLAG_CONV2D = 1, 2, 4, 8
FLAG_SPLIT = 64
FLAG_SPLIT3 = 128
FLAG_AMAX_COARSE = 1024
FLAG_NO_BG_FILL = 2048
FLAG_SPLIT_F16 = 512


def split_flags(split, row=False):
    if not split:
        return 0
    return (FLAG_SPLIT if row else 0) | (FLAG_SPLIT3 if int(split) == 3 else 0) | (FLAG_SPLIT_F16 if int(split) == 4 else 0)
# ... 70 lines not shown
    am = amax_of(t)
    if am is not None:
        tag_amax(t2, am * abs(float(f)))
    return t2


STATUS_F16_WEIGHT_RANGE = 8
_W16_STATUS = {}


def fp16_weight_status(device):
    idx = device.index if device.index is not None else torch.cuda.current_device()
    st = _W16_STATUS.get(idx)
    if st is None:
        st = _W16_STATUS[idx] = torch.zeros((1,), dtype=torch.int32, device=torch.device('cuda', idx))
    return st


def guard_fp16_weight(w):
    base = w._base if w._base is not None else w
    seen = base.__dict__.setdefault('_mvx_w16', {})
    tag = (base._version, w.data_ptr())
    if seen.get(tuple(w.shape)) != tag:
        seen[tuple(w.shape)] = tag
        wc = w.detach()
        wc = wc if wc.is_contiguous() else wc.contiguous()
        X.call('mvx_split_f16_weight_check', wc, wc.numel(), fp16_weight_status(w.device))


def raise_on_status(word):
    word = int(word)
    if word & STATUS_F16_WEIGHT_RANGE:
        raise X.MvxHipError('convmath fp16x3: a weight reached |w| >= 255.9 (or is not finite): its fp16 pieces overflow.  The results '
                            'of this step are invalid; use convmath bf16x6 (three bf16 pieces: the exponent range of f32)')
    if word & 1:
        raise AssertionError('projected point outside the feature map (imhead/Pipe.py:71)')
    if word:
        raise X.MvxHipError('a kernel reported a data-dependent error (status %d)' % word)


def grad_split(split, dz):
    if split and int(split) == 4 and amax_of(dz) is None:
        return 3
    return split


def split_pieces():
    import modules.config as cfg
    m = cfg.config.get('convmath', 'f32')
    if m not in ('f32', 'bf16x3', 'bf16x6', 'fp16x3'):
        raise X.MvxHipError('convmath must be f32, bf16x3, bf16x6 or fp16x3, not %r' % (m,))
    return {'f32': 0, 'bf16x3': 2, 'bf16x6': 3, 'fp16x3': 4}[m]
FLAG_BG_TAPS = 32

GRAD_SINK = False


ASYNC_WGRAD = False
_SIDE = {}


def side_stream(device):
    st = _SIDE.get(device.index)
    if st is None:
        st = torch.cuda.Stream(device=device, priority=0)
        _SIDE[device.index] = st
    return st


_KEEP = {}
_COMM = {}
_TAIL = {}


def comm_stream(device):
    st = _COMM.get(device.index)
    if st is None:
        st = _COMM[device.index] = torch.cuda.Stream(device)
    return st


def mark_tail(device):
    if device.index in _SIDE:
        ev = torch.cuda.Event()
        ev.record(_SIDE[device.index])
        _TAIL[device.index] = [ev, None]


def tail_events(device):
    t = _TAIL.pop(device.index, None)
    return tuple(t) if t is not None and t[1] is not None else None


def drop_tail(device=None):
    if device is None:
        _TAIL.clear()
    else:
        _TAIL.pop(device.index, None)


def join_side_stream(device=None):
    for idx, st in _SIDE.items():
        if device is None or device.index == idx:
            cur = torch.cuda.current_stream(st.device)
            t = _TAIL.get(idx)
            if t is not None:
# ... 531 lines not shown


class Background:
    __slots__ = ('c', 'y_bg', 'mask', 'hflag', 'tflag', 'bflag', 'back')

    def __init__(self, c, mask, hflag, tflag=None, y_bg=None, back=None, bflag=None):
        self.c, self.mask, self.hflag, self.tflag, self.y_bg, self.back = c, mask, hflag, tflag, y_bg, back
        self.bflag = bflag if bflag is not None else tflag


EXEC_STAGES = None
STAGE_FLOP = 2.0 * 9 * 128 * 32 * 64


def n_tiles(H, W):
    return ((H + 7) // 8) * ((W + 15) // 16)


def _exec_stages(device):
    global EXEC_STAGES
    if KERNEL_TIMERS is None:
        return None
    if EXEC_STAGES is None:
        EXEC_STAGES = torch.zeros((1,), dtype=torch.int64, device=device)
    return EXEC_STAGES


def activity_dilate(src, src_is_index, din, H, W, sd, pd, mark_border, want_tile_flags=False, F=1):
    dout = conv_out_depth(din, sd, pd)
    mask = torch.empty((F * dout, H, W), dtype=torch.uint8, device=src.device)
    hflag = torch.empty((F * dout, n_tiles(H, W)), dtype=torch.int32, device=src.device)
    tflag = torch.empty_like(hflag) if want_tile_flags else None
    X.call('mvx_activity_dilate_frames', src, 1 if src_is_index else 0, din, dout, H, W, sd, pd, 1 if mark_border else 0, mask,
           hflag, tflag, F)
    return (mask, hflag, tflag) if want_tile_flags else (mask, hflag)


def conv3d_background(w, c_in, din, sd, pd):
    cout, cin = w.shape[0], w.shape[1]
    dout = conv_out_depth(din, sd, pd)
    bg_pre = torch.empty((dout, cout), dtype=torch.float32, device=w.device)
    X.call('mvx_conv3d_background', w.contiguous(), c_in, din, dout, cin, cout, sd, pd, bg_pre)
    return bg_pre


def conv3d_background_taps(w, c_in, din, sd, pd, F=1):
    cout, cin = w.shape[0], w.shape[1]
    dout = conv_out_depth(din, sd, pd)
    bg_all = torch.empty((F * dout * 13, cout), dtype=torch.float32, device=w.device)
    X.call('mvx_conv3d_background_taps_frames', w, c_in, din, dout, cin, cout, sd, pd, bg_all, F)
    return bg_all


def bn_background(bg_pre, bias, mi, planes, channels, relu=True, want_y=False, F=1):
    c_out = torch.empty((F * planes, channels), dtype=torch.float32, device=mi.device)
    y_bg = torch.empty_like(c_out) if want_y else None
    X.call('mvx_bn_background_frames', bg_pre, bias, mi, planes, channels, FLAG_RELU if relu else 0, y_bg, c_out, F)
    return (c_out, y_bg) if want_y else c_out


def bn_apply_tiles(y, mi, c_bg, tflag, F=1, read=None, out=None):
    FD, H, W, C = y.shape
    if out is None:
        out = torch.empty_like(y)
    nbytes = (lambda: (tflag.ne(0).sum() + (torch.logical_or(tflag.ne(0), read.ne(0)).sum() if read is not None else tflag.numel()))
              * (128 * C * 4)) if KERNEL_TIMERS is not None else 0
    with _timed_bytes('bn_apply', nbytes):
        if read is not None:
            X.call('mvx_bn_apply_tiles_read_frames', y, mi, c_bg, tflag, read, out, FD // F, H, W, C, F)
        else:
            X.call('mvx_bn_apply_tiles_frames', y, mi, c_bg, tflag, out, FD // F, H, W, C, F)
    return out


def bn_apply_tiles_bev(y, mi, c_bg, tflag, F=1):
    FD, H, W, C = y.shape
    D = FD // F
    bev = torch.empty((F, C * D, H, W), dtype=torch.float32, device=y.device)
    nbytes = (lambda: (tflag.ne(0).sum() + tflag.numel()) * (128 * C * 4)) if KERNEL_TIMERS is not None else 0
    with _timed_bytes('bn_apply', nbytes):
        X.call('mvx_bn_apply_tiles_bev_frames', y, mi, c_bg, tflag, bev, D, H, W, C, F)
    return bev


def plane_tap_sums(dz, tile_flags=None, inactive_sums=None):
    D, H, W, C = dz.shape
    T = torch.empty((D, 9, C), dtype=torch.float32, device=dz.device)
    ws = workspace(X.lib.mvx_plane_tap_sums_workspace_bytes(D, C), dz.device, 'tap_sums')
    X.call('mvx_plane_tap_sums', dz, D, H, W, C, tile_flags, inactive_sums, T, ws, ws.numel())
    return T


def tile_dilate_flags(in_tflag, self_tflag, din, H, W, sd, pd, F=1):
    dout = conv_out_depth(din, sd, pd)
    out = torch.empty((F * dout, n_tiles(H, W)), dtype=torch.int32, device=in_tflag.device)
    X.call('mvx_tile_dilate_flags_frames', in_tflag, self_tflag, din, dout, H, W, sd, pd, out, F)
    return out


def tile_read_flags(hflag, din, H, W, sd, pd, F=1):
    dout = conv_out_depth(din, sd, pd)
    out = torch.empty_like(hflag)
    X.call('mvx_tile_read_flags_frames', hflag, din, dout, H, W, sd, pd, out, F)
    return out


def conv3d_input_grad_sums(w, T, din, sd, pd, F=1):
    cout, cin = w.shape[0], w.shape[1]
    A = torch.empty((F * din, cin), dtype=torch.float32, device=w.device)
    X.call('mvx_conv3d_input_grad_sums_frames', w.contiguous(), T, din, T.shape[0] // F, cin, cout, sd, pd, A, F)
    return A


def conv3d_dgrad_tiles(dz, wpk_d, din, cin, sd, pd, tflag, split=False, F=1):
    FD, H, W, cout = dz.shape
    dout = FD // F
    dx = torch.empty((F * din, H, W, cin), dtype=torch.float32, device=dz.device)
    counter = _exec_stages(dz.device)
    with _Timed('conv3d_gather_tiles', F * conv_flops(din, dout, H, W, cout, cin, sd, pd, True) if KERNEL_TIMERS is not None else 0):
        if split:
            bind_amax(split, dz)
            X.call('mvx_conv3d_dgrad_tiles_split_frames', dz, wpk_d, dx, din, dout, H, W, cin, cout, sd, pd, split_flags(split),
                   tflag, counter, F)
        else:
            X.call('mvx_conv3d_dgrad_tiles_frames', dz, wpk_d, dx, din, dout, H, W, cin, cout, sd, pd, tflag, counter,
                   _work_counter(dz.device), F)
    return dx


def bn_relu_backward_tiles(dyhat, y, mi, bg, plane_grad_sums, dbias_out=None, want_inactive_sums=False, F=1):
    FD, H, W, C = y.shape
    dz = torch.empty_like(y)
    if dbias_out is not None:
        db, flags = dbias_out, FLAG_ACCUMULATE
    else:
        db, flags = torch.empty((C,), dtype=torch.float32, device=y.device), 0
    ws = workspace(X.lib.mvx_bn_relu_backward_tiles_workspace_bytes_frames(FD // F, H, W, C, F), y.device, 'bn_tiles')
    inact = torch.empty((FD, C), dtype=torch.float32, device=y.device) if want_inactive_sums else None
    amax = new_amax(y.device)
    bflag = bg.bflag
    nbytes = (lambda: bflag.ne(0).sum() * (128 * C * 4 * 5)) if KERNEL_TIMERS is not None else 0
    with _timed_bytes('bn_relu_backward_tiles', nbytes):
        X.call('mvx_bn_relu_backward_tiles_frames', dyhat, y, mi, bg.c, bg.y_bg, plane_grad_sums, bflag, FD // F, H, W, C, dz, db,
               inact, amax, flags, ws, ws.numel(), F)
    tag_amax(dz, amax)
    db = None if dbias_out is not None else db
    return (dz, db, inact) if want_inactive_sums else (dz, db)


def conv3d_forward_bg(x, wpk, bias, cout, sd, pd, bg_in, out_mask, bg_pre, relu=True, want_stats=True, finalize_eps=None,
                      split=False, F=None, bg_taps=False):
    nf = F or 1
    FD, H, W, cin = x.shape
    din = FD // nf
    dout = conv_out_depth(din, sd, pd)
    out = torch.empty((nf * dout, H, W, cout), dtype=torch.float32, device=x.device)
    stats, fz = _acc_f64(_per_frame(F, STATS_REPLICAS, 2, cout), x.device) if want_stats else (None, 0)
    flags = (FLAG_RELU if relu else 0) | fz | split_flags(split) | (FLAG_BG_TAPS if bg_taps else 0)
    fin, mi, npos = None, None, float(dout * H * W)
    if finalize_eps is not None and want_stats:
        fin = _fin_slot(x.device, fz)
        if fin is None:
            fin = torch.zeros((1,), dtype=torch.float64, device=x.device)
        mi = torch.empty(_per_frame(F, 2, cout), dtype=torch.float32, device=x.device)
    counter = _exec_stages(x.device)
    with _Timed('conv3d_gather_bg', nf * conv_flops(dout, din, H, W, cin, cout, sd, pd) if KERNEL_TIMERS is not None else 0):
        if split:
            X.call('mvx_conv3d_forward_bg_split_frames', x, wpk, bias, out, stats, din, dout, H, W, cin, cout, sd, pd, flags,
                   bg_in.hflag, out_mask, bg_pre, 1, counter, nf)
        else:
            X.call('mvx_conv3d_forward_bg_frames', x, wpk, bias, out, stats, din, dout, H, W, cin, cout, sd, pd, flags,
                   bg_in.hflag, out_mask, bg_pre, 1, counter, fin, npos, float(finalize_eps or 0.0), mi, _work_counter(x.device),
                   nf)
    if split and mi is not None:
        X.call('mvx_bn_finalize_frames', stats, npos, float(finalize_eps), mi, cout, nf)
    return (out, mi) if mi is not None else (out, stats)


def conv3d_wgrad_bg(x, dz, sd, pd, bg_in, tap_sums=None, accumulate_into=None, split=False, F=1, flops=0):
    FD, H, W, cin = x.shape
    din = FD // F
    dout, cout = dz.shape[0] // F, dz.shape[3]
    if accumulate_into is not None:
        dw, flags = accumulate_into, FLAG_ACCUMULATE
    else:
        dw, flags = torch.empty((cout, cin, 3, 3, 3), dtype=torch.float32, device=x.device), 0
    flags |= split_flags(split, True)
    nbytes = X.lib.mvx_conv3d_wgrad_bg_workspace_bytes_frames(dout, H, W, cin, cout, F)
    if tap_sums is None:
        tap_sums = plane_tap_sums(dz)
    with _wgrad_scope(accumulate_into, x, dz, tap_sums, bg_in.c, bg_in.hflag) as scope:
        ws = workspace(nbytes, x.device, 'wgrad_bg_side' if isinstance(scope, _SideStream) else 'wgrad_bg')
        with _Timed('conv3d_wgrad_bg', flops):
            bind_amax(split, None, dz)
            X.call('mvx_conv3d_wgrad_bg_frames', x, dz, dw, din, dout, H, W, cin, cout, sd, pd, flags, bg_in.hflag, bg_in.c,
                   tap_sums, ws, ws.numel(), F)
    return None if accumulate_into is not None else dw


def _ld(t):
    assert t.dim() == 2 and t.stride(1) == 1, 'need a row-major 2-D view'
    return t.stride(0) if t.shape[0] > 1 else max(t.stride(0), t.shape[1])


def _vptr(t):
    if t is None:
        return None
    if not t.is_cuda:
        raise X.MvxHipError('libmvx_hip needs device tensors (no CPU fallback)')
    import ctypes
    return ctypes.c_void_p(t.data_ptr())


def _fin_slot(device, zeroed):
    if zeroed:
        a = _ARENAS.get(_arena_key(device))
        v = a.take(1) if a is not None else None
        if v is not None:
            return v
    return None


def _work_counter(device):
    if _ARENA_ON:
        a = _ARENAS.get(_arena_key(device))
        v = a.take(1) if a is not None else None
        if v is not None:
            return v
    return torch.zeros((1,), dtype=torch.float64, device=device)


ROW_SPLIT = ('dgrad', 'wgrad', 'rpn')


def row_split(tag):
    np_ = split_pieces()
    if np_ == 2:
        return 2 if any(tag.startswith(k) for k in ROW_SPLIT) else 0
    if np_ in (3, 4):
        return np_
    return 0


def transposed_weight(w2):
    base = w2._base if w2._base is not None else w2
    cache = base.__dict__.setdefault('_mvx_wt', {})
    tag = (base._version, w2.data_ptr())
    hit = cache.get(tuple(w2.shape))
    if hit is None or hit[0] != tag:
# ... 1055 lines not shown
```

mvxnet-makise_amd/modules/frames.py:

```python
import os

import torch

import modules.config as cfg
from modules import _hip
from modules import Extension as X
from modules.layers.Blocks import conv_background_on, conv_split_math

R = _hip.STATS_REPLICAS


class FrameSet:

    def __init__(self, voxels, coords, vox_off, T):
        self.voxels, self.coords = voxels, coords
        self.vox_off = [int(v) for v in vox_off]
        self.F, self.T = len(vox_off) - 1, int(T)
        self.Vt = self.vox_off[-1]
        self.real_off = None
        self.desc = None
        self.sampled = None
        self.grid = None

    def enqueue_map(self):
# ... 170 lines not shown
        y, mi = linear_bn(x, w, b, fs, X.ROWS_FUSION, fs.fusion_row_w, eps, 'fusion_%dx%d' % (w.shape[0], w[0].numel()),
                          foreign=(i == 0))
        S.fusion.append((x, w, b, y, mi))
        x = bn_apply(y, mi, fs, X.ROWS_FUSION)
    return _vfe_forward(bb, fs, x, S, eps)


def _vfe_forward(bb, fs, x, S, eps):
    dev = fs.voxels.device
    F, T, Rt, Vt = fs.F, fs.T, fs.Rt, fs.Vt
    Fc = x.shape[1]
    ldr = (7 + Fc + 3) & ~3
    rows23 = _hip.vfe_compact_input(fs.vox2d, x, fs, pitch=ldr)
    S.fc = Fc
    S.vfe = []
    x = rows23
    for vfe in (bb.svfe.vfe1, bb.svfe.vfe2):
        w, b = vfe.fcn.fc.weight, vfe.fcn.fc.bias
        y, mi = linear_bn(x, _hip.padded_weight(w.reshape(w.shape[0], -1), x.shape[1]), b, fs, X.ROWS_VFE, fs.row_w, eps, 'vfe')
        out, am = _hip.vfe_bn_max_concat(y, mi, Vt, T, fs)
        S.vfe.append((x, w, b, y, mi, am))
        x = out
    w, b = bb.fcn.fc.weight, bb.fcn.fc.bias
    y, mi = linear_bn(x, w, b, fs, X.ROWS_VFE, fs.row_w, eps, 'vfe')
    feat, am = _hip.bn_segment_max(y, mi, Vt, T, fs)
    S.head = (x, w, b, y, mi, am)
    return feat, S


def grid_activity(model, fs):
    bb = model.backbone
    dev = fs.voxels.device
    F, Vt = fs.F, fs.Vt
    D0, H, W = cfg.voxelshape[2], cfg.voxelshape[0], cfg.voxelshape[1]
    idx_grid, st2 = _hip.index_grid(fs.coords, (D0, H, W), fs.desc)
    tensors = [idx_grid, st2]
    layers = []
    src, is_index, din = idx_grid, True, D0
    for li, m in enumerate((bb.cml.conv1, bb.cml.conv2, bb.cml.conv3)):
        lay = _hip.activity_dilate(src, is_index, din, H, W, m._sd, m._pd, li > 0, want_tile_flags=True, F=F)
        layers.append(lay)
        tensors += lay
        src, is_index, din = lay[0], False, _hip.conv_out_depth(din, m._sd, m._pd)
    c2 = bb.cml.conv2
    d1 = _hip.conv_out_depth(D0, bb.cml.conv1._sd, bb.cml.conv1._pd)
    bflag2 = _hip.tile_dilate_flags(layers[0][2], layers[1][2], d1, H, W, c2._sd, c2._pd, F=F)
    tensors.append(bflag2)
    reads = []
    din = d1
    for li, m in enumerate((bb.cml.conv2, bb.cml.conv3)):
        reads.append(_hip.tile_read_flags(layers[li][1], din, H, W, m._sd, m._pd, F=F))
        din = _hip.conv_out_depth(din, m._sd, m._pd)
    tensors += reads
    return dict(idx_grid=idx_grid, status=st2, layers=layers, bflag2=bflag2, reads=reads, tensors=tensors)


def cml_forward(model, fs, feat, S, status_sink, want_bev=True):
    bb = model.backbone
    dev = fs.voxels.device
    F, T, Rt, Vt = fs.F, fs.T, fs.Rt, fs.Vt
    eps = cfg.eps
    _hip.require_plain_batchnorm()
    D0, H, W = cfg.voxelshape[2], cfg.voxelshape[0], cfg.voxelshape[1]
    c1, c2, c3 = bb.cml.conv1, bb.cml.conv2, bb.cml.conv3
    w1, b1 = c1.conv.weight, c1.conv.bias
    cout, cin = w1.shape[0], w1.shape[1]
    w_all = w1.permute(2, 3, 4, 0, 1).reshape(27 * cout, cin).contiguous()
    P, _ = _hip.linear_forward(feat, w_all, None, relu=False, want_stats=False, split=_hip.row_split('conv1'))
    ga = fs.grid if fs.grid is not None else grid_activity(model, fs)
    fs.grid = None
    idx_grid = ga['idx_grid']
    status_sink.append(ga['status'])
    D1 = _hip.conv_out_depth(D0, c1._sd, c1._pd)
    y1 = torch.full((F * D1, H, W, cout), float('nan'), dtype=torch.float32, device=dev) if os.environ.get('MVX_POISON_BG') else None
    if 'sparse_out' in KNOCKOUT:
        y1, stats = _knocked(feat, (F * D1, H, W, cout)), torch.zeros((F, R, 2, cout), dtype=torch.float64, device=dev)
    else:
        y1, stats = _hip.sparse_conv_output_tiles(P, idx_grid, (D0, H, W), b1, cout, c1._sd, c1._pd, ga['layers'][0][2], F, out=y1)
    mi1 = _hip.bn_finalize(stats, D1 * H * W, eps, F)

    def dilate(li):
        return ga['layers'][li]

    def background(bg_pre, bias, mi, planes, C_):
        return _hip.bn_background(bg_pre, bias, mi, planes, C_, want_y=True, F=F)

    def bn_apply_bg(y, mi, c_bg, tflag, read=None):
        if 'bn_apply_cml' in KNOCKOUT:
            return y
        out = torch.full_like(y, float('nan')) if (read is not None and os.environ.get('MVX_POISON_BG')) else None
        return _hip.bn_apply_tiles(y, mi, c_bg, tflag, F, read, out)

    mask1, hflag1, tflag1 = dilate(0)
    cc1, ybg1 = background(None, b1, mi1, D1, cout)
    x1 = bn_apply_bg(y1, mi1, cc1, tflag1, ga['reads'][0])
    S.conv1 = dict(feat=feat, w=w1, b=b1, w_all=w_all, y=y1, mi=mi1, c=cc1, ybg=ybg1, tflag=tflag1, D0=D0, D1=D1)

    split = conv_split_math()
    if not conv_background_on():
        raise X.MvxHipError('the frame-set path needs convbackground (the default configuration)')
    S.split = split
    S.convs = []
    x_in, din, c_in, mask_in, hflag_in, tflag_in = x1, D1, cc1, mask1, hflag1, tflag1
    bflag_in = tflag1
    for li, m in enumerate((c2, c3)):
        w, b = m.conv.weight, m.conv.bias
        co, ci = w.shape[0], w.shape[1]
        sd, pd = m._sd, m._pd
        dout = _hip.conv_out_depth(din, sd, pd)
        wpk = m._packer(False, split)
        bg_pre = _hip.conv3d_background_taps(w, c_in, din, sd, pd, F)[:F * dout]
        mask_o, hflag_o, tflag_o = dilate(li + 1)
        if 'gather_fwd' in KNOCKOUT and not split:
            y, mi = _knocked(x_in, (F * dout, H, W, co)), _knocked(x_in, (F, 2, co))
        else:
            y, mi = _hip.conv3d_forward_bg(x_in, wpk, b, co, sd, pd, _hip.Background(c_in, mask_in, hflag_in), mask_o, bg_pre,
                                           finalize_eps=eps, split=split, F=F, bg_taps=True)
        c_o, ybg_o = background(bg_pre, b, mi, dout, co)
        if want_bev and li == 1 and co <= 64 and 'bn_apply_cml' not in KNOCKOUT and BEV_FUSED:
            mid = _hip.bn_apply_tiles_bev(y, mi, c_o, tflag_o, F)
            x_out = None
        else:
            x_out = bn_apply_bg(y, mi, c_o, tflag_o, ga['reads'][1] if li == 0 else None)
        rec = dict(x=x_in, w=w, b=b, y=y, mi=mi, din=din, dout=dout, sd=sd, pd=pd, m=m, c_in=c_in, hflag_in=hflag_in,
                   bflag_in=bflag_in, split=split)
        if li == 0:
            bflag_o = ga['bflag2']
            rec.update(c_out=c_o, ybg_out=ybg_o, bflag_out=bflag_o)
            c_in, bflag_in = c_o, bflag_o
        S.convs.append(rec)
        x_in, din, mask_in, hflag_in, tflag_in = x_out, dout, mask_o, hflag_o, tflag_o
    D3 = din
    S.D3, S.H, S.W, S.C3 = D3, H, W, co
    S.x3 = x_in
    if not want_bev:
        return None
    if x_in is None:
        return mid
    return _hip.cl_to_bev(x_in, F)


def _wgrad_bg_flops(rec, F):
    din, dout, sd, pd = rec['din'], rec['dout'], rec['sd'], rec['pd']
    hflag = rec['hflag_in']
    co, ci = rec['w'].shape[0], rec['w'].shape[1]

    def count():
        hf = hflag.view(F, din, -1).ne(0)
        steps = 0
        for kd in range(3):
            for d in range(dout):
                ds = d * sd - pd + kd
                if 0 <= ds < din:
                    steps = steps + hf[:, ds].sum()
        return float(steps) * (2.0 * 128 * ci * co * 9)
    return count


def _wgrad_bg(rec, dz, tap_sums, F, H, W):
    if 'wgrad_bg' in KNOCKOUT:
        return
    fl = _wgrad_bg_flops(rec, F) if _hip.KERNEL_TIMERS is not None else 0
    _hip.conv3d_wgrad_bg(rec['x'], dz, rec['sd'], rec['pd'], _hip.Background(rec['c_in'], None, rec['hflag_in']), tap_sums,
                         accumulate_into=_grad_of(rec['w']), split=rec.get('split'), F=F, flops=fl)


def _linear_wgrad_side(x, dz, w):
    if 'lin_wgrad' in KNOCKOUT:
        return
    _hip.linear_wgrad(x, dz, accumulate_into=_grad_of(w).view(w.shape[0], -1))


def middle_backward(model, S, grad_mid):
    old_async, _hip.ASYNC_WGRAD = _hip.ASYNC_WGRAD, True
    try:
        rows_backward(model, S, cml_backward(model, S, grad_mid))
    finally:
        _hip.ASYNC_WGRAD = old_async


_MUTATE = {}


def _mut(name, t):
    return _hip.mutate(_MUTATE, name, t) if _MUTATE else t


def cml_backward(model, S, grad_mid, g_cl=None):
    fs = S.fs
    F, T, Rt, Vt = fs.F, fs.T, fs.Rt, fs.Vt
    H, W, D3, C3 = S.H, S.W, S.D3, S.C3
    dev = fs.voxels.device
    gm = grad_mid.contiguous() if g_cl is None else None
    if g_cl is not None:
        g = g_cl
    elif gm.shape[0] == 1 and F > 1:
        g = _hip.bev_to_cl_broadcast(gm, D3, F)
    else:
        g = _hip.bev_to_cl(gm, D3)

    def tap_sums(dz, tile_flags=None, inactive=None):
        if 'tap_sums' in KNOCKOUT:
            return _knocked(dz, (dz.shape[0], 9, dz.shape[3]))
        return _hip.plane_tap_sums(dz, tile_flags, inactive)

    def tap_sums_side(name, dz, tile_flags=None, inactive=None):
        if not _hip.ASYNC_WGRAD or 'tap_sums' in KNOCKOUT:
            return _mut(name, tap_sums(dz, tile_flags, inactive)), None
        main = torch.cuda.current_stream(dev)
        with _hip._SideStream(dz, tile_flags, inactive):
            Tt = _mut(name, tap_sums(dz, tile_flags, inactive))
            ev = torch.cuda.Event()
            ev.record(torch.cuda.current_stream(dev))
        Tt.record_stream(main)
        return Tt, ev

    def dgrad_tiles(rec, dz, bflag):
        split = rec.get('split') or 0
        wpd = rec['m']._packer(True, split)
        if 'gather_dgrad' in KNOCKOUT and not split:
            return _knocked(dz, (F * rec['din'], H, W, rec['w'].shape[1]))
        return _hip.conv3d_dgrad_tiles(dz, wpd, rec['din'], rec['w'].shape[1], rec['sd'], rec['pd'], bflag, split, F)

    def input_grad_sums(rec, Tt):
        return _hip.conv3d_input_grad_sums(rec['w'], Tt, rec['din'], rec['sd'], rec['pd'], F)

    def bn_bwd_tiles(gin, y, mi, c_bg, y_bg, A, bflag, bias, want_inactive):
        if 'bn_bwd_tiles' in KNOCKOUT:
            return _knocked(y), (_knocked(y, (y.shape[0], y.shape[3])) if want_inactive else None)
        bg = _hip.Background(c_bg, None, None, y_bg=y_bg, bflag=bflag)
        out = _hip.bn_relu_backward_tiles(gin, y, mi, bg, A, _grad_of(bias), want_inactive, F)
        return out[0], (out[2] if want_inactive else None)

    r3, r2 = S.convs[1], S.convs[0]
    dz3 = bn_relu_backward(g, r3['y'], r3['mi'], fs, X.ROWS_GRID, None, _grad_of(r3['b']))
    T3, ev3 = tap_sums_side('T3', dz3)
    _wgrad_bg(r3, dz3, T3, F, H, W)
    g2 = dgrad_tiles(r3, dz3, r3['bflag_in'])
    if ev3 is not None:
        torch.cuda.current_stream(dev).wait_event(ev3)
    A2 = _mut('A2', input_grad_sums(r3, T3))
    dz2, inact2 = bn_bwd_tiles(g2, r2['y'], r2['mi'], r2['c_out'], r2['ybg_out'], A2, r2['bflag_out'], r2['b'], True)
    inact2 = _mut('inact2', inact2)
    T2, ev2 = tap_sums_side('T2', dz2, r2['bflag_out'], inact2)
    _wgrad_bg(r2, dz2, T2, F, H, W)
    g1 = dgrad_tiles(r2, dz2, r2['bflag_in'])
    if ev2 is not None:
        torch.cuda.current_stream(dev).wait_event(ev2)
    A1 = _mut('A1', input_grad_sums(r2, T2))
    c1 = S.conv1
    w1 = c1['w']
    cout, cin = w1.shape[0], w1.shape[1]
    dz1, _ = bn_bwd_tiles(g1, c1['y'], c1['mi'], c1['c'], c1['ybg'], A1, c1['tflag'], c1['b'], False)
    cm = model.backbone.cml.conv1
    G = _hip.sparse_conv_gather_dz(dz1, fs.coords, c1['D0'], cm._sd, cm._pd, fs.desc)
    with _hip._SideStream(c1['feat'], G):
        dw_all = _hip.linear_wgrad(c1['feat'], G)
    with _hip._SideStream(dw_all):
        _grad_of(w1).add_(dw_all.reshape(3, 3, 3, cout, cin).permute(3, 4, 0, 1, 2))
    dfeat, _ = _hip.linear_forward(G, c1['w_all'].t().contiguous(), None, relu=False, want_stats=False, label='linear_dgrad',
                                   split=_hip.row_split('dgrad'))
    return dfeat


def _rows_dgrad(dz, w2):
    if 'lin_dgrad' in KNOCKOUT:
        return torch.empty((dz.shape[0], w2.shape[1]), dtype=torch.float32, device=dz.device)
    gx, _ = _hip.linear_forward(dz, _hip.transposed_weight(w2), None, relu=False, want_stats=False, label='linear_dgrad',
                                split=_hip.row_split('dgrad'))
    return gx


def rows_backward(model, S, dfeat):
    fs = S.fs
    F, T, Rt, Vt = fs.F, fs.T, fs.Rt, fs.Vt
    dev = dfeat.device
    x, w, b, y, mi, am = S.head
    Cn = w.shape[0]
    dyh = _hip.segment_max_backward(dfeat, am, Vt, T, fs)
    dz = bn_relu_backward(dyh, y, mi, fs, X.ROWS_VFE, fs.row_w, _grad_of(b), dz=dyh)
    _linear_wgrad_side(x, dz, w)
    gx = _rows_dgrad(dz, w)
    for x, w, b, y, mi, am in reversed(S.vfe):
        Cn = w.shape[0]
        dyh = _hip.vfe_max_concat_backward(gx, am, Vt, T, fs)
        dz = bn_relu_backward(dyh, y, mi, fs, X.ROWS_VFE, fs.row_w, _grad_of(b), dz=dyh)
        w2 = w.reshape(w.shape[0], -1)
        if x.shape[1] != w2.shape[1] and 'lin_wgrad' not in KNOCKOUT:
            with _hip._SideStream(x, dz):
                dwp = _hip.linear_wgrad(x, dz)
                _grad_of(w).view(w2.shape).add_(dwp[:, :w2.shape[1]])
        else:
            _linear_wgrad_side(x, dz, w)
        gx = _rows_dgrad(dz, w)
    Fc = S.fc
    gim = _hip.vfe_compact_input_backward(gx, Fc, fs)
    gx = gim
# ... 16 lines not shown
```

Baseline: 538.3 frames/s.

## Track border-class background values so CML layer-3 work skips non-voxel tiles

Adds 9-class (interior, edges, corners) background values for the layer-2 output and 25-region tap sums for layer-3's dz. Layer 3's forward then reads a halo mask dilated from voxels rather than from the whole layer-2 activity, and its weight gradient uses a per-class rank-1 background correction. The aim is to cut the tiles the conv and wgrad kernels must gather and multiply, because border-adjacent background no longer has to be computed explicitly. In exchange it adds extra small kernels (25-region atomics in f64, per-class background conv, per-class rank-1 wgrad) and more edge-case logic where correctness depends on how the border classes are handled.

```diff
diff --git a/include/mvx_hip.h b/include/mvx_hip.h
--- a/include/mvx_hip.h
+++ b/include/mvx_hip.h
@@ -25,6 +25,9 @@
 #define MVX_FLAG_AMAX_COARSE 1024
 
 #define MVX_FLAG_NO_BG_FILL 2048
+
+#define MVX_FLAG_BG_CLS_OUT 8192
+#define MVX_FLAG_BG_CLS_IN 16384
 
 #define MVX_OK 0
 #define MVX_EINVAL (-1)
@@ -350,6 +353,9 @@
                                  int32_t stride_d, int32_t pad_d, float *bg_pre, int32_t n_frames, void *stream);
 int mvx_bn_background_frames(const float *bg_pre, const float *bias, const float *mean_inv, int32_t planes, int32_t channels,
                              int32_t flags, float *y_bg, float *c_out, int32_t n_frames, void *stream);
+int mvx_conv3d_background_cls_frames(const float *w, const float *c_in, const float *c_cls_in, int32_t din, int32_t dout,
+                                     int32_t cin, int32_t cout, int32_t stride_d, int32_t pad_d, float *bg, int32_t n_frames,
+                                     void *stream);
 int mvx_conv3d_forward_bg_frames(const float *in, const float *wpk, const float *bias, float *out, double *stats,
                                  int32_t din, int32_t dout, int32_t h, int32_t w, int32_t cin, int32_t cout,
                                  int32_t stride_d, int32_t pad_d, int32_t flags, const int32_t *in_halo_flags,
@@ -369,6 +375,13 @@
                                int32_t cin, int32_t cout, int32_t stride_d, int32_t pad_d, int32_t flags,
                                const int32_t *in_halo_flags, const float *c_in, const float *tap_sums, void *workspace,
                                size_t workspace_bytes, int32_t n_frames, void *stream);
+int mvx_conv3d_wgrad_bg_cls_frames(const float *in, const float *dz, float *dw, int32_t din, int32_t dout, int32_t h, int32_t w,
+                                   int32_t cin, int32_t cout, int32_t stride_d, int32_t pad_d, int32_t flags,
+                                   const int32_t *in_halo_flags, const float *c_cls_in, const float *tap_sums_cls,
+                                   void *workspace, size_t workspace_bytes, int32_t n_frames, void *stream);
+size_t mvx_plane_tap_sums_cls_workspace_bytes(int32_t planes, int32_t channels);
+int mvx_plane_tap_sums_cls(const float *dz, int32_t planes, int32_t h, int32_t w, int32_t channels, float *tap_sums,
+                           float *tap_sums_cls, void *workspace, size_t workspace_bytes, void *stream);
 size_t mvx_bn_relu_backward_tiles_workspace_bytes_frames(int32_t planes, int32_t h, int32_t w, int32_t channels,
                                                          int32_t n_frames);
 int mvx_bn_relu_backward_tiles_frames(const float *dyhat, const float *y, const float *mean_inv, const float *c_bg,
diff --git a/mvxnet-makise_amd/csrc/activity.hip b/mvxnet-makise_amd/csrc/activity.hip
--- a/mvxnet-makise_amd/csrc/activity.hip
+++ b/mvxnet-makise_amd/csrc/activity.hip
@@ -110,15 +110,26 @@
     out[e] = on ? 1 : 0;
 }
 
+__device__ __forceinline__ int src_cls5(const int r5, const int a) {
+    if (r5 == 0) return a - 1;
+    if (r5 == 1) return a == 0 ? 0 : 1;
+    if (r5 == 2) return 1;
+    if (r5 == 3) return a == 2 ? 2 : 1;
+    return a == 0 ? 1 : (a == 1 ? 2 : -1);
+}
+
 __global__ __launch_bounds__(64) void conv_background(const float *__restrict__ w, const float *__restrict__ c_in, int Din,
                                                       int Dout, int Cin, int Cout, int sd, int pd,
                                                       float *__restrict__ bg_pre, float *__restrict__ bg_tap,
-                                                      float *__restrict__ bg_cls) {
+                                                      float *__restrict__ bg_cls, const float *__restrict__ c_cls_in,
+                                                      float *__restrict__ bg_cls25) {
     const int n = blockIdx.x, d = blockIdx.y;
     double s = 0.0;
-    double cls[9];
+    double cls[9], cls25[25];
 #pragma unroll
     for (int q = 0; q < 9; ++q) cls[q] = 0.0;
+#pragma unroll
+    for (int q = 0; q < 25; ++q) cls25[q] = 0.0;
     for (int kd = 0; kd < 3; ++kd) {
         const int ds = mvx_src_plane(d, Din, Dout, sd, pd, kd);
         double sk = 0.0;
@@ -136,6 +147,22 @@
                     }
                 }
             }
+        if (ds >= 0 && bg_cls25)
+            for (int c = threadIdx.x; c < Cin; c += 64) {
+                double wk[9], c9[9];
+#pragma unroll
+                for (int k = 0; k < 9; ++k) {
+                    wk[k] = (double)w[(((size_t)n * Cin + c) * 3 + kd) * 9 + k];
+                    c9[k] = (double)c_cls_in[((size_t)ds * 9 + k) * Cin + c];
+                }
+#pragma unroll
+                for (int k = 0; k < 9; ++k)
+#pragma unroll
+                    for (int q = 0; q < 25; ++q) {
+                        const int sy = src_cls5(q / 5, k / 3), sx = src_cls5(q % 5, k % 3);
+                        if (sy >= 0 && sx >= 0) cls25[q] += wk[k] * c9[3 * sy + sx];
+                    }
+            }
         s += sk;
         if (bg_tap) {
             sk = wave_sum_f64(sk);
@@ -147,8 +174,15 @@
     if (bg_cls) {
 #pragma unroll
         for (int q = 0; q < 9; ++q) {
-            const double v = wave_sum_f64(cls[q]);
+            const double v = q == 4 ? s : wave_sum_f64(cls[q]);
             if (threadIdx.x == 0) bg_cls[((size_t)d * 9 + q) * Cout + n] = (float)v;
+        }
+    }
+    if (bg_cls25) {
+#pragma unroll
+        for (int q = 0; q < 25; ++q) {
+            const double v = q == 12 ? s : wave_sum_f64(cls25[q]);
+            if (threadIdx.x == 0) bg_cls25[((size_t)d * 25 + q) * Cout + n] = (float)v;
         }
     }
 }
@@ -531,7 +565,7 @@
     MVX_CHECK_ARG(w && c_in && bg_pre && din > 0 && dout > 0 && cin > 0 && cout > 0);
     MVX_CHECK_ARG(n_frames >= 1 && n_frames <= MVX_MAX_FRAMES);
     hipLaunchKernelGGL(conv_background, dim3(cout, dout * n_frames), dim3(64), 0, (hipStream_t)stream, w, c_in, din, dout, cin,
-                       cout, stride_d, pad_d, bg_pre, (float *)nullptr, (float *)nullptr);
+                       cout, stride_d, pad_d, bg_pre, (float *)nullptr, (float *)nullptr, (const float *)nullptr, (float *)nullptr);
     MVX_LAUNCH_CHECK();
     return MVX_OK;
 }
@@ -542,7 +576,20 @@
     MVX_CHECK_ARG(w && c_in && bg && din > 0 && dout > 0 && cin > 0 && cout > 0);
     MVX_CHECK_ARG(n_frames >= 1 && n_frames <= MVX_MAX_FRAMES);
     hipLaunchKernelGGL(conv_background, dim3(cout, dout * n_frames), dim3(64), 0, (hipStream_t)stream, w, c_in, din, dout, cin,
-                       cout, stride_d, pad_d, bg, bg + (size_t)dout * n_frames * cout, bg + (size_t)4 * dout * n_frames * cout);
+                       cout, stride_d, pad_d, bg, bg + (size_t)dout * n_frames * cout, bg + (size_t)4 * dout * n_frames * cout,
+                       (const float *)nullptr, (float *)nullptr);
+    MVX_LAUNCH_CHECK();
+    return MVX_OK;
+}
+
+extern "C" int mvx_conv3d_background_cls_frames(const float *w, const float *c_in, const float *c_cls_in, int32_t din, int32_t dout,
+                                                int32_t cin, int32_t cout, int32_t stride_d, int32_t pad_d, float *bg,
+                                                int32_t n_frames, void *stream) {
+    MVX_CHECK_ARG(w && c_in && c_cls_in && bg && din > 0 && dout > 0 && cin > 0 && cout > 0);
+    MVX_CHECK_ARG(n_frames >= 1 && n_frames <= MVX_MAX_FRAMES);
+    const size_t pc = (size_t)dout * n_frames * cout;
+    hipLaunchKernelGGL(conv_background, dim3(cout, dout * n_frames), dim3(64), 0, (hipStream_t)stream, w, c_in, din, dout, cin,
+                       cout, stride_d, pad_d, bg, bg + pc, bg + 4 * pc, c_cls_in, bg + 13 * pc);
     MVX_LAUNCH_CHECK();
     return MVX_OK;
 }
diff --git a/mvxnet-makise_amd/csrc/conv3d.hip b/mvxnet-makise_amd/csrc/conv3d.hip
--- a/mvxnet-makise_amd/csrc/conv3d.hip
+++ b/mvxnet-makise_amd/csrc/conv3d.hip
@@ -73,7 +73,7 @@
 #pragma unroll
     for (int q = 0; q < BK / 8; ++q) b_off[q] = li * BK + 4 * (((2 * q) | lh) ^ wkey);
 
-    const bool on_border = tx0 == 0 || ty0 == 0 || tx0 + TW >= g.W || ty0 + TH >= g.H;
+    const bool on_border = unit_on_border(g, tx0, ty0, TH, border_active);
     const TilePlan plan = tile_plan<1>(g, d, on_border, in_hflag, border_active, ntiles, tile, tile);
     const bool active = plan.active;
     const int nstages = plan.nk * nchunks;
@@ -775,6 +775,91 @@
     if (a == 2 && b == 0) t += k[7];
     if (a == 2 && b == 2) t += k[8];
     T[e] = (float)t;
+}
+
+constexpr int RK25 = 25;
+__global__ __launch_bounds__(256) void plane_region_sums25(const float *__restrict__ dz, int D, int H, int W, int C,
+                                                           double *__restrict__ R) {
+    __shared__ float red[256][4];
+    const int y = blockIdx.x, d = blockIdx.y;
+    const int c4n = C >> 2, ct = threadIdx.x % c4n, st = threadIdx.x / c4n, spb = 256 / c4n;
+    const float *row = dz + ((size_t)d * H + y) * W * C;
+    float4 s = make_float4(0.f, 0.f, 0.f, 0.f);
+    for (int x = st; x < W; x += spb) {
+        const float4 v = *(const float4 *)(row + (size_t)x * C + ct * 4);
+        s.x += v.x; s.y += v.y; s.z += v.z; s.w += v.w;
+    }
+    red[threadIdx.x][0] = s.x; red[threadIdx.x][1] = s.y; red[threadIdx.x][2] = s.z; red[threadIdx.x][3] = s.w;
+    __syncthreads();
+    if (st == 0) {
+        const unsigned rep = (unsigned)y % RREP;
+        double *Rp = R + ((size_t)rep * D + d) * RK25 * C;
+        const int iy = y == 0 ? 1 : (y == 1 ? 2 : (y == H - 2 ? 3 : (y == H - 1 ? 4 : 0)));
+        const int xs[4] = {0, 1, W - 2, W - 1};
+        double v[5][4];
+        for (int j = 0; j < 4; ++j) {
+            double t = 0.0;
+            for (int q = 0; q < spb; ++q) t += (double)red[q * c4n + ct][j];
+            v[0][j] = t;
+        }
+        for (int k = 0; k < 4; ++k) {
+            const float4 e = *(const float4 *)(row + (size_t)xs[k] * C + ct * 4);
+            v[k + 1][0] = (double)e.x; v[k + 1][1] = (double)e.y; v[k + 1][2] = (double)e.z; v[k + 1][3] = (double)e.w;
+        }
+        for (int k = 0; k < 5; ++k)
+            for (int j = 0; j < 4; ++j) {
+                atomicAdd(Rp + (size_t)k * C + ct * 4 + j, v[k][j]);
+                if (iy) atomicAdd(Rp + (size_t)(5 * iy + k) * C + ct * 4 + j, v[k][j]);
+            }
+    }
+}
+
+__device__ __forceinline__ int cls_set_coef(const int a, const int s, const int i) {
+    if (s == 0) return (a < 2 && i == 2 - a) ? 1 : 0;
+    if (s == 2) return (a > 0 && i == 5 - a) ? 1 : 0;
+    if (i == 0) return 1;
+    if (a == 0) return (i == 1 || i == 2) ? -1 : 0;
+    if (a == 1) return (i == 1 || i == 4) ? -1 : 0;
+    return (i == 4 || i == 3) ? -1 : 0;
+}
+
+__global__ void region_tap_sums_cls(const double *__restrict__ R, int D, int C, float *__restrict__ T, float *__restrict__ T_cls) {
+    const int e = blockIdx.x * blockDim.x + threadIdx.x;
+    if (e >= D * 9 * C) return;
+    const int n = e % C, tap = (e / C) % 9, d = e / (9 * C);
+    const int a = tap / 3, b = tap % 3;
+    double k[RK25];
+    for (int q = 0; q < RK25; ++q) {
+        double t = 0.0;
+        for (int rep = 0; rep < RREP; ++rep) t += R[(((size_t)rep * D + d) * RK25 + q) * C + n];
+        k[q] = t;
+    }
+    double all = 0.0;
+    for (int sy = 0; sy < 3; ++sy)
+        for (int sx = 0; sx < 3; ++sx) {
+            double t = 0.0;
+            for (int i = 0; i < 5; ++i)
+                for (int j = 0; j < 5; ++j) t += (double)(cls_set_coef(a, sy, i) * cls_set_coef(b, sx, j)) * k[5 * i + j];
+            T_cls[(((size_t)d * 9 + tap) * 9 + 3 * sy + sx) * C + n] = (float)t;
+            all += t;
+        }
+    T[e] = (float)all;
+}
+
+__global__ void wgrad_rank1_cls(const float *__restrict__ T_cls, const float *__restrict__ c_cls, float *__restrict__ dw, Geom g) {
+    const size_t total = (size_t)27 * g.Cin * g.Cout;
+    for (size_t e = blockIdx.x * (size_t)blockDim.x + threadIdx.x; e < total; e += (size_t)gridDim.x * blockDim.x) {
+        const int tap = (int)(e % 9), kd = (int)((e / 9) % 3);
+        const int ci = (int)((e / 27) % g.Cin), co = (int)(e / ((size_t)27 * g.Cin));
+        float s = 0.f;
+        for (int d = 0; d < g.Dout * g.F; ++d) {
+            const int ds = mvx_src_plane(d, g.Din, g.Dout, g.sd, g.pd, kd);
+            if (ds < 0) continue;
+            for (int q = 0; q < 9; ++q)
+                s += c_cls[((size_t)ds * 9 + q) * g.Cin + ci] * T_cls[(((size_t)d * 9 + tap) * 9 + q) * g.Cout + co];
+        }
+        dw[e] += s;
+    }
 }
 
 __global__ void wgrad_rank1(const float *__restrict__ T, const float *__restrict__ c_in, float *__restrict__ dw, Geom g) {
@@ -932,6 +1017,8 @@
     if (rc) return rc;
     if ((rc = conv_check_frames(n_frames))) return rc;
     MVX_CHECK_ARG(!done_counter || (stats && mean_inv && count > 0));
+    int border_bits = 0;
+    if ((rc = conv_bg_border_bits(flags, border_active, h, w, &border_bits))) return rc;
     hipStream_t st = (hipStream_t)stream;
     hipError_t e = conv_zero_stats(stats, done_counter, cout, n_frames, flags, st);
     if (e != hipSuccess) return (int)e;
@@ -939,7 +1026,7 @@
     GatherArgs a;
     a.in = in; a.bias = bias; a.out = out; a.stats = stats; a.relu = flags & MVX_FLAG_RELU;
     a.in_hflag = in_halo_flags; a.out_mask = out_mask; a.bg_pre = bg_pre;
-    a.border_active = (border_active ? 1 : 0) | ((flags & MVX_FLAG_BG_TAPS) ? 2 : 0);
+    a.border_active = border_bits;
     a.exec_stages = (unsigned long long *)exec_stages;
     a.done_counter = (unsigned *)done_counter; a.fin_count = count; a.fin_eps = eps; a.fin_mean_inv = mean_inv;
     a.work_counter = (unsigned *)work_counter;
@@ -1079,6 +1166,27 @@
     return MVX_OK;
 }
 
+extern "C" size_t mvx_plane_tap_sums_cls_workspace_bytes(int32_t planes, int32_t channels) {
+    return planes > 0 && channels > 0 ? sizeof(double) * RREP * planes * RK25 * channels : 0;
+}
+
+extern "C" int mvx_plane_tap_sums_cls(const float *dz, int32_t planes, int32_t h, int32_t w, int32_t channels, float *tap_sums,
+                                      float *tap_sums_cls, void *workspace, size_t workspace_bytes, void *stream) {
+    MVX_CHECK_ARG(dz && tap_sums && tap_sums_cls && workspace && planes > 0 && h >= 5 && w >= 5 && channels > 0);
+    MVX_CHECK_ARG(channels % 4 == 0 && 256 % (channels / 4) == 0);
+    MVX_CHECK_ARG(workspace_bytes >= mvx_plane_tap_sums_cls_workspace_bytes(planes, channels));
+    hipStream_t st = (hipStream_t)stream;
+    double *R = (double *)workspace;
+    hipError_t e = hipMemsetAsync(R, 0, sizeof(double) * RREP * planes * RK25 * channels, st);
+    if (e != hipSuccess) return (int)e;
+    hipLaunchKernelGGL(plane_region_sums25, dim3(h, planes), dim3(256), 0, st, dz, planes, h, w, channels, R);
+    MVX_LAUNCH_CHECK();
+    hipLaunchKernelGGL(region_tap_sums_cls, dim3(mvx_cdiv((long long)planes * 9 * channels, 64)), dim3(64), 0, st,
+                       (const double *)R, planes, channels, tap_sums, tap_sums_cls);
+    MVX_LAUNCH_CHECK();
+    return MVX_OK;
+}
+
 extern "C" int mvx_conv3d_input_grad_sums_frames(const float *w, const float *tap_sums, int32_t din, int32_t dout, int32_t cin,
                                                  int32_t cout, int32_t stride_d, int32_t pad_d, float *plane_grad_sums,
                                                  int32_t n_frames, void *stream) {
@@ -1107,10 +1215,10 @@
     return mvx_conv3d_wgrad_bg_workspace_bytes_frames(dout, h, w, cin, cout, 1);
 }
 
-extern "C" int mvx_conv3d_wgrad_bg_frames(const float *in, const float *dz, float *dw, int32_t din, int32_t dout, int32_t h,
-                                          int32_t w, int32_t cin, int32_t cout, int32_t stride_d, int32_t pad_d, int32_t flags,
-                                          const int32_t *in_halo_flags, const float *c_in, const float *tap_sums,
-                                          void *workspace, size_t workspace_bytes, int32_t n_frames, void *stream) {
+static int wgrad_bg_frames(const float *in, const float *dz, float *dw, int32_t din, int32_t dout, int32_t h, int32_t w,
+                           int32_t cin, int32_t cout, int32_t stride_d, int32_t pad_d, int32_t flags,
+                           const int32_t *in_halo_flags, const float *c_in, const float *tap_sums, void *workspace,
+                           size_t workspace_bytes, int32_t n_frames, bool cls, void *stream) {
     const SplitAmax am = mvxi_take_split_amax();
     MVX_CHECK_ARG(in && dz && dw && workspace && in_halo_flags && c_in && tap_sums);
     int rc = conv_check_geom(din, dout, h, w, cin, cout, stride_d, pad_d);
@@ -1121,7 +1229,9 @@
     const WgradWorkspace ws = conv_carve_wgrad(workspace, wgrad_bg_slab_bytes(cin), dout * n_frames, ntiles, false);
     MVX_CHECK_ARG(workspace_bytes >= ws.bytes);
     const int nstrips = wgrad_bg_strips(cin);
+    MVX_CHECK_ARG(!cls || (h >= 5 && w >= 5));
     Geom g{din, dout, h, w, cin, cout, stride_d, pad_d, 0, n_frames};
+    g.cls_in = cls ? 1 : 0;
     hipStream_t st = (hipStream_t)stream;
     int nd[3], ndsum = 0;
     for (int kd = 0; kd < 3; ++kd) {
@@ -1149,9 +1259,27 @@
     hipLaunchKernelGGL(wgrad_reduce, dim3(mvx_cdiv(per_slab, 256)), dim3(256), 0, st, (const float *)ws.slabs, dw, widest, cin,
                        flags & MVX_FLAG_ACCUMULATE, 0, ks, 0);
     MVX_LAUNCH_CHECK();
-    hipLaunchKernelGGL(wgrad_rank1, dim3(mvx_cdiv(per_slab, 256)), dim3(256), 0, st, tap_sums, c_in, dw, g);
+    if (cls) hipLaunchKernelGGL(wgrad_rank1_cls, dim3(mvx_cdiv(per_slab, 256)), dim3(256), 0, st, tap_sums, c_in, dw, g);
+    else hipLaunchKernelGGL(wgrad_rank1, dim3(mvx_cdiv(per_slab, 256)), dim3(256), 0, st, tap_sums, c_in, dw, g);
     MVX_LAUNCH_CHECK();
     return MVX_OK;
+}
+
+extern "C" int mvx_conv3d_wgrad_bg_frames(const float *in, const float *dz, float *dw, int32_t din, int32_t dout, int32_t h,
+                                          int32_t w, int32_t cin, int32_t cout, int32_t stride_d, int32_t pad_d, int32_t flags,
+                                          const int32_t *in_halo_flags, const float *c_in, const float *tap_sums,
+                                          void *workspace, size_t workspace_bytes, int32_t n_frames, void *stream) {
+    return wgrad_bg_frames(in, dz, dw, din, dout, h, w, cin, cout, stride_d, pad_d, flags, in_halo_flags, c_in, tap_sums, workspace,
+                           workspace_bytes, n_frames, false, stream);
+}
+
+extern "C" int mvx_conv3d_wgrad_bg_cls_frames(const float *in, const float *dz, float *dw, int32_t din, int32_t dout, int32_t h,
+                                              int32_t w, int32_t cin, int32_t cout, int32_t stride_d, int32_t pad_d,
+                                              int32_t flags, const int32_t *in_halo_flags, const float *c_cls_in,
+                                              const float *tap_sums_cls, void *workspace, size_t workspace_bytes,
+                                              int32_t n_frames, void *stream) {
+    return wgrad_bg_frames(in, dz, dw, din, dout, h, w, cin, cout, stride_d, pad_d, flags, in_halo_flags, c_cls_in, tap_sums_cls,
+                           workspace, workspace_bytes, n_frames, true, stream);
 }
 
 extern "C" int mvx_conv3d_wgrad_bg(const float *in, const float *dz, float *dw, int32_t din, int32_t dout, int32_t h,
diff --git a/mvxnet-makise_amd/csrc/conv3d_split.hip b/mvxnet-makise_amd/csrc/conv3d_split.hip
--- a/mvxnet-makise_amd/csrc/conv3d_split.hip
+++ b/mvxnet-makise_amd/csrc/conv3d_split.hip
@@ -74,7 +74,7 @@
     const int tid = threadIdx.x, lane = tid & 63, wv = tid >> 6, li = lane & 31, lh = lane >> 5;
     const int nchunks = g.Cin / BKT;
     if (only_tiles && !(only_tiles[(size_t)d * ntiles8 + t_top] | only_tiles[(size_t)d * ntiles8 + t_bot])) return;
-    const bool on_border = tx0 == 0 || ty0 == 0 || tx0 + TW >= g.W || ty0 + THT >= g.H;
+    const bool on_border = unit_on_border(g, tx0, ty0, THT, border_active);
     const TilePlan plan = tile_plan<MT>(g, d, on_border, in_hflag, border_active, ntiles8, t_top, t_bot);
 
     f32x16 acc[MT][2];
@@ -347,6 +347,8 @@
     int rc = conv_check_frames(n_frames);
     if (rc) return rc;
     if ((rc = conv_check_forward(din, dout, h, w, cin, cout, stride_d, pad_d))) return rc;
+    int border_bits = 0;
+    if ((rc = conv_bg_border_bits(flags, border_active, h, w, &border_bits))) return rc;
     hipStream_t st = (hipStream_t)stream;
     hipError_t e = conv_zero_stats(stats, nullptr, cout, n_frames, flags, st);
     if (e != hipSuccess) return (int)e;
@@ -354,7 +356,7 @@
     GatherArgs a;
     a.in = in; a.bias = bias; a.out = out; a.stats = stats; a.relu = flags & MVX_FLAG_RELU;
     a.in_hflag = in_halo_flags; a.out_mask = out_mask; a.bg_pre = bg_pre;
-    a.border_active = (border_active ? 1 : 0) | ((flags & MVX_FLAG_BG_TAPS) ? 2 : 0);
+    a.border_active = border_bits;
     a.exec_stages = (unsigned long long *)exec_stages;
     launch_gather_split(st, flags, g, (const unsigned short *)wsplit, a);
     MVX_LAUNCH_CHECK();
diff --git a/mvxnet-makise_amd/csrc/conv_geom.h b/mvxnet-makise_amd/csrc/conv_geom.h
--- a/mvxnet-makise_amd/csrc/conv_geom.h
+++ b/mvxnet-makise_amd/csrc/conv_geom.h
@@ -15,6 +15,7 @@
     int F = 1;
     int tap_lo = 0, tap_hi = 3;
     int s2d = 0;
+    int cls_in = 0;
 };
 
 __device__ __forceinline__ unsigned s2d_tap_mask(int p) {
@@ -52,6 +53,14 @@
 
 static inline int conv_check_frames(int32_t n_frames) {
     MVX_CHECK_ARG(n_frames >= 1 && n_frames <= MVX_MAX_FRAMES);
+    return MVX_OK;
+}
+
+static inline int conv_bg_border_bits(int32_t flags, int32_t border_active, int32_t h, int32_t w, int *bits) {
+    const int cls = flags & (MVX_FLAG_BG_CLS_OUT | MVX_FLAG_BG_CLS_IN);
+    MVX_CHECK_ARG(!cls || ((flags & MVX_FLAG_BG_TAPS) && h >= 5 && w >= 5));
+    *bits = (border_active ? 1 : 0) | ((flags & MVX_FLAG_BG_TAPS) ? 2 : 0) | ((flags & MVX_FLAG_BG_CLS_OUT) ? 4 : 0) |
+            ((flags & MVX_FLAG_BG_CLS_IN) ? 8 : 0);
     return MVX_OK;
 }
 
diff --git a/mvxnet-makise_amd/csrc/conv_kernels.h b/mvxnet-makise_amd/csrc/conv_kernels.h
--- a/mvxnet-makise_amd/csrc/conv_kernels.h
+++ b/mvxnet-makise_amd/csrc/conv_kernels.h
@@ -9,13 +9,23 @@
     unsigned skipped;
     bool active;
     bool idle_border;
+    bool cls_out;
+    bool cls_in;
 };
+
+__device__ __forceinline__ bool unit_on_border(const Geom &g, const int tx0, const int ty0, const int th, const int border_active) {
+    const int reach = (border_active & 8) ? 1 : 0;
+    return tx0 == 0 || ty0 == 0 || tx0 + TW + reach >= g.W || ty0 + th + reach >= g.H;
+}
+
+__device__ __forceinline__ int cls3(const int i, const int n) { return i == 0 ? 0 : (i >= n - 1 ? 2 : 1); }
+__device__ __forceinline__ int cls5(const int i, const int n) { return i <= 1 ? i : (i >= n - 1 ? 4 : (i == n - 2 ? 3 : 2)); }
 
 template <int NT>
 __device__ __forceinline__ TilePlan tile_plan(const Geom &g, const int d, const bool on_border,
                                               const int *__restrict__ in_hflag, const int border_active, const int ntiles,
                                               const int t0, const int t1) {
-    TilePlan p{{0, 0, 0}, {0, 0, 0}, 0, 0u, true, false};
+    TilePlan p{{0, 0, 0}, {0, 0, 0}, 0, 0u, true, false, false, false};
     const bool skip_taps = in_hflag && (border_active & 2) && !on_border;
     int any_flag = 0;
 #pragma unroll
@@ -38,6 +48,8 @@
     p.idle_border = in_hflag && (border_active & 2) && on_border && !any_flag;
     if (p.idle_border) p.nk = 0;
     if (in_hflag) p.active = (((border_active & 1) && on_border) || any_flag) != 0;
+    p.cls_out = (border_active & 4) && on_border;
+    p.cls_in = (border_active & 8) != 0;
     return p;
 }
 
@@ -73,15 +85,17 @@
 #pragma unroll
     for (int m = 0; m < MT; ++m) {
         const int py = ty0 + 2 * MT * wv + 2 * m;
+        const float *bg_cls = bg_pre ? bg_pre + (size_t)4 * g.Dout * g.F * g.Cout + (size_t)d * 9 * g.Cout : nullptr;
         if (p.idle_border) {
-            const float *bg_cls = bg_pre + (size_t)4 * g.Dout * g.F * g.Cout + (size_t)d * 9 * g.Cout;
+            const float *bg_cls25 = bg_pre + (size_t)13 * g.Dout * g.F * g.Cout + (size_t)d * 25 * g.Cout;
 #pragma unroll
             for (int r = 0; r < 16; ++r) {
                 const int row = mfma32_row(r) + 4 * lh;
                 const int gy = py + (row >> 4), gx = tx0 + (row & 15);
-                const int q = 3 * (gy == 0 ? 0 : (gy >= g.H - 1 ? 2 : 1)) + (gx == 0 ? 0 : (gx >= g.W - 1 ? 2 : 1));
-                acc[m][0][r] = bg_cls[q * g.Cout + n0];
-                acc[m][1][r] = bg_cls[q * g.Cout + n1];
+                const float *cl = p.cls_in ? bg_cls25 + (5 * cls5(gy, g.H) + cls5(gx, g.W)) * g.Cout
+                                           : bg_cls + (3 * cls3(gy, g.H) + cls3(gx, g.W)) * g.Cout;
+                acc[m][0][r] = cl[n0];
+                acc[m][1][r] = cl[n1];
             }
         }
         unsigned site_on = p.active ? 0xffffu : 0u;
@@ -96,6 +110,20 @@
             site_on = 0u;
 #pragma unroll
             for (int r = 0; r < 16; ++r) site_on |= (mk[r] ? 1u : 0u) << r;
+        }
+        if (p.cls_out && out_mask && site_on != 0xffffu) {
+#pragma unroll
+            for (int r = 0; r < 16; ++r) {
+                const int row = mfma32_row(r) + 4 * lh;
+                const int q = 3 * cls3(py + (row >> 4), g.H) + cls3(tx0 + (row & 15), g.W);
+                if (q != 4 && !((site_on >> r) & 1u)) {
+                    if (!p.idle_border) {
+                        acc[m][0][r] = bg_cls[q * g.Cout + n0];
+                        acc[m][1][r] = bg_cls[q * g.Cout + n1];
+                    }
+                    site_on |= 1u << r;
+                }
+            }
         }
 #pragma unroll
         for (int r = 0; r < 16; ++r) {
@@ -196,7 +224,10 @@
                 const int gy = ty0 - 1 + r / HW, gx = tx0 - 1 + r % HW;
                 if (gy >= 0 && gy < g.H && gx >= 0 && gx < g.W) {
                     v = *(const f32x4 *)(in + (((size_t)ds * g.H + gy) * g.W + gx) * g.Cin + cc * W4_C + part * 4);
-                    if (c_in) v -= *(const f32x4 *)(c_in + (size_t)ds * g.Cin + cc * W4_C + part * 4);
+                    if (c_in) {
+                        const size_t pc = g.cls_in ? (size_t)ds * 9 + 3 * cls3(gy, g.H) + cls3(gx, g.W) : (size_t)ds;
+                        v -= *(const f32x4 *)(c_in + pc * g.Cin + cc * W4_C + part * 4);
+                    }
                 }
             }
             xr[u] = v;
diff --git a/mvxnet-makise_amd/modules/Extension.py b/mvxnet-makise_amd/modules/Extension.py
--- a/mvxnet-makise_amd/modules/Extension.py
+++ b/mvxnet-makise_amd/modules/Extension.py
@@ -132,6 +132,7 @@
     'mvx_bn_apply_tiles_read_frames': (_i32, [_p, _p, _p, _p, _p, _p, _i32, _i32, _i32, _i32, _i32, _p]),
     'mvx_tile_read_flags_frames': (_i32, [_p, _i32, _i32, _i32, _i32, _i32, _i32, _p, _i32, _p]),
     'mvx_conv3d_background_taps_frames': (_i32, [_p, _p, _i32, _i32, _i32, _i32, _i32, _i32, _p, _i32, _p]),
+    'mvx_conv3d_background_cls_frames': (_i32, [_p, _p, _p, _i32, _i32, _i32, _i32, _i32, _i32, _p, _i32, _p]),
     'mvx_bn_background_frames': (_i32, [_p, _p, _p, _i32, _i32, _i32, _p, _p, _i32, _p]),
     'mvx_conv3d_forward_bg_frames': (_i32, [_p, _p, _p, _p, _p, _i32, _i32, _i32, _i32, _i32, _i32, _i32, _i32, _i32, _p, _p, _p,
                                             _i32, _p, _p, _f64, _f64, _p, _p, _i32, _p]),
@@ -139,6 +140,9 @@
     'mvx_conv3d_input_grad_sums_frames': (_i32, [_p, _p, _i32, _i32, _i32, _i32, _i32, _i32, _p, _i32, _p]),
     'mvx_conv3d_wgrad_bg_workspace_bytes_frames': (_sz, [_i32, _i32, _i32, _i32, _i32, _i32]),
     'mvx_conv3d_wgrad_bg_frames': (_i32, [_p, _p, _p, _i32, _i32, _i32, _i32, _i32, _i32, _i32, _i32, _i32, _p, _p, _p, _p, _sz, _i32, _p]),
+    'mvx_conv3d_wgrad_bg_cls_frames': (_i32, [_p, _p, _p, _i32, _i32, _i32, _i32, _i32, _i32, _i32, _i32, _i32, _p, _p, _p, _p, _sz, _i32, _p]),
+    'mvx_plane_tap_sums_cls_workspace_bytes': (_sz, [_i32, _i32]),
+    'mvx_plane_tap_sums_cls': (_i32, [_p, _i32, _i32, _i32, _i32, _p, _p, _p, _sz, _p]),
     'mvx_bn_relu_backward_tiles_workspace_bytes_frames': (_sz, [_i32, _i32, _i32, _i32, _i32]),
     'mvx_bn_relu_backward_tiles_frames': (_i32, [_p, _p, _p, _p, _p, _p, _p, _i32, _i32, _i32, _i32, _p, _p, _p, _p, _i32, _p, _sz, _i32, _p]),
     'mvx_cl_to_bev_frames': (_i32, [_p, _p, _i32, _i32, _i32, _i32, _i32, _i32, _p]),
diff --git a/mvxnet-makise_amd/modules/_hip.py b/mvxnet-makise_amd/modules/_hip.py
--- a/mvxnet-makise_amd/modules/_hip.py
+++ b/mvxnet-makise_amd/modules/_hip.py
@@ -146,6 +146,7 @@
         raise X.MvxHipError('convmath must be f32, bf16x3, bf16x6 or fp16x3, not %r' % (m,))
     return {'f32': 0, 'bf16x3': 2, 'bf16x6': 3, 'fp16x3': 4}[m]
 FLAG_BG_TAPS = 32
+FLAG_BG_CLS_OUT, FLAG_BG_CLS_IN = 8192, 16384
 
 GRAD_SINK = False
 
@@ -783,6 +784,18 @@
     return bg_all
 
 
+def conv3d_background_cls(w, c_in, c_cls_in, din, sd, pd, F=1):
+    cout, cin = w.shape[0], w.shape[1]
+    dout = conv_out_depth(din, sd, pd)
+    bg_all = torch.empty((F * dout * 38, cout), dtype=torch.float32, device=w.device)
+    X.call('mvx_conv3d_background_cls_frames', w, c_in, c_cls_in, din, dout, cin, cout, sd, pd, bg_all, F)
+    return bg_all
+
+
+def bn_background_cls(bg_all, bias, mi, planes, channels, relu=True, F=1):
+    return bn_background(bg_all[4 * F * planes:13 * F * planes], bias, mi, 9 * planes, channels, relu, False, F)
+
+
 def bn_background(bg_pre, bias, mi, planes, channels, relu=True, want_y=False, F=1):
     c_out = torch.empty((F * planes, channels), dtype=torch.float32, device=mi.device)
     y_bg = torch.empty_like(c_out) if want_y else None
@@ -820,6 +833,15 @@
     ws = workspace(X.lib.mvx_plane_tap_sums_workspace_bytes(D, C), dz.device, 'tap_sums')
     X.call('mvx_plane_tap_sums', dz, D, H, W, C, tile_flags, inactive_sums, T, ws, ws.numel())
     return T
+
+
+def plane_tap_sums_cls(dz):
+    D, H, W, C = dz.shape
+    T = torch.empty((D, 9, C), dtype=torch.float32, device=dz.device)
+    Tc = torch.empty((D, 9, 9, C), dtype=torch.float32, device=dz.device)
+    ws = workspace(X.lib.mvx_plane_tap_sums_cls_workspace_bytes(D, C), dz.device, 'tap_sums')
+    X.call('mvx_plane_tap_sums_cls', dz, D, H, W, C, T, Tc, ws, ws.numel())
+    return T, Tc
 
 
 def tile_dilate_flags(in_tflag, self_tflag, din, H, W, sd, pd, F=1):
@@ -880,14 +902,15 @@
 
 
 def conv3d_forward_bg(x, wpk, bias, cout, sd, pd, bg_in, out_mask, bg_pre, relu=True, want_stats=True, finalize_eps=None,
-                      split=False, F=None, bg_taps=False):
+                      split=False, F=None, bg_taps=False, cls_out=False, cls_in=False):
     nf = F or 1
     FD, H, W, cin = x.shape
     din = FD // nf
     dout = conv_out_depth(din, sd, pd)
     out = torch.empty((nf * dout, H, W, cout), dtype=torch.float32, device=x.device)
     stats, fz = _acc_f64(_per_frame(F, STATS_REPLICAS, 2, cout), x.device) if want_stats else (None, 0)
-    flags = (FLAG_RELU if relu else 0) | fz | split_flags(split) | (FLAG_BG_TAPS if bg_taps else 0)
+    flags = (FLAG_RELU if relu else 0) | fz | split_flags(split) | (FLAG_BG_TAPS if bg_taps else 0) | \
+        (FLAG_BG_CLS_OUT if cls_out else 0) | (FLAG_BG_CLS_IN if cls_in else 0)
     fin, mi, npos = None, None, float(dout * H * W)
     if finalize_eps is not None and want_stats:
         fin = _fin_slot(x.device, fz)
@@ -908,7 +931,7 @@
     return (out, mi) if mi is not None else (out, stats)
 
 
-def conv3d_wgrad_bg(x, dz, sd, pd, bg_in, tap_sums=None, accumulate_into=None, split=False, F=1, flops=0):
+def conv3d_wgrad_bg(x, dz, sd, pd, bg_in, tap_sums=None, accumulate_into=None, split=False, F=1, flops=0, cls=False):
     FD, H, W, cin = x.shape
     din = FD // F
     dout, cout = dz.shape[0] // F, dz.shape[3]
@@ -919,13 +942,13 @@
     flags |= split_flags(split, True)
     nbytes = X.lib.mvx_conv3d_wgrad_bg_workspace_bytes_frames(dout, H, W, cin, cout, F)
     if tap_sums is None:
-        tap_sums = plane_tap_sums(dz)
+        tap_sums = plane_tap_sums_cls(dz)[1] if cls else plane_tap_sums(dz)
     with _wgrad_scope(accumulate_into, x, dz, tap_sums, bg_in.c, bg_in.hflag) as scope:
         ws = workspace(nbytes, x.device, 'wgrad_bg_side' if isinstance(scope, _SideStream) else 'wgrad_bg')
         with _Timed('conv3d_wgrad_bg', flops):
             bind_amax(split, None, dz)
-            X.call('mvx_conv3d_wgrad_bg_frames', x, dz, dw, din, dout, H, W, cin, cout, sd, pd, flags, bg_in.hflag, bg_in.c,
-                   tap_sums, ws, ws.numel(), F)
+            X.call('mvx_conv3d_wgrad_bg_cls_frames' if cls else 'mvx_conv3d_wgrad_bg_frames', x, dz, dw, din, dout, H, W, cin, cout,
+                   sd, pd, flags, bg_in.hflag, bg_in.c, tap_sums, ws, ws.numel(), F)
     return None if accumulate_into is not None else dw
 
 
diff --git a/mvxnet-makise_amd/modules/frames.py b/mvxnet-makise_amd/modules/frames.py
--- a/mvxnet-makise_amd/modules/frames.py
+++ b/mvxnet-makise_amd/modules/frames.py
@@ -246,7 +246,9 @@
         reads.append(_hip.tile_read_flags(layers[li][1], din, H, W, m._sd, m._pd, F=F))
         din = _hip.conv_out_depth(din, m._sd, m._pd)
     tensors += reads
-    return dict(idx_grid=idx_grid, status=st2, layers=layers, bflag2=bflag2, reads=reads, tensors=tensors)
+    vox2 = _hip.activity_dilate(layers[0][0], False, d1, H, W, c2._sd, c2._pd, False, F=F)
+    tensors += vox2
+    return dict(idx_grid=idx_grid, status=st2, layers=layers, bflag2=bflag2, reads=reads, vox2=vox2, tensors=tensors)
 
 
 def cml_forward(model, fs, feat, S, status_sink, want_bev=True):
@@ -297,20 +299,30 @@
     S.convs = []
     x_in, din, c_in, mask_in, hflag_in, tflag_in = x1, D1, cc1, mask1, hflag1, tflag1
     bflag_in = tflag1
+    vox2, c_cls = ga['vox2'], None
+    cls_field = H >= 5 and W >= 5
     for li, m in enumerate((c2, c3)):
         w, b = m.conv.weight, m.conv.bias
         co, ci = w.shape[0], w.shape[1]
         sd, pd = m._sd, m._pd
         dout = _hip.conv_out_depth(din, sd, pd)
         wpk = m._packer(False, split)
-        bg_pre = _hip.conv3d_background_taps(w, c_in, din, sd, pd, F)[:F * dout]
         mask_o, hflag_o, tflag_o = dilate(li + 1)
+        cls_out, cls_in = cls_field and li == 0, cls_field and li == 1
+        if cls_in:
+            bg_all = _hip.conv3d_background_cls(w, c_in, c_cls, din, sd, pd, F)
+        else:
+            bg_all = _hip.conv3d_background_taps(w, c_in, din, sd, pd, F)
+        bg_pre = bg_all[:F * dout]
+        mask_f, hflag_f = (vox2[0] if cls_out else mask_o), (vox2[1] if cls_in else hflag_in)
         if 'gather_fwd' in KNOCKOUT and not split:
             y, mi = _knocked(x_in, (F * dout, H, W, co)), _knocked(x_in, (F, 2, co))
         else:
-            y, mi = _hip.conv3d_forward_bg(x_in, wpk, b, co, sd, pd, _hip.Background(c_in, mask_in, hflag_in), mask_o, bg_pre,
-                                           finalize_eps=eps, split=split, F=F, bg_taps=True)
+            y, mi = _hip.conv3d_forward_bg(x_in, wpk, b, co, sd, pd, _hip.Background(c_in, mask_in, hflag_f), mask_f, bg_pre,
+                                           finalize_eps=eps, split=split, F=F, bg_taps=True, cls_out=cls_out, cls_in=cls_in)
         c_o, ybg_o = background(bg_pre, b, mi, dout, co)
+        if cls_out:
+            c_cls = _hip.bn_background_cls(bg_all, b, mi, dout, co, F=F)
         if want_bev and li == 1 and co <= 64 and 'bn_apply_cml' not in KNOCKOUT and BEV_FUSED:
             mid = _hip.bn_apply_tiles_bev(y, mi, c_o, tflag_o, F)
             x_out = None
@@ -318,6 +330,8 @@
             x_out = bn_apply_bg(y, mi, c_o, tflag_o, ga['reads'][1] if li == 0 else None)
         rec = dict(x=x_in, w=w, b=b, y=y, mi=mi, din=din, dout=dout, sd=sd, pd=pd, m=m, c_in=c_in, hflag_in=hflag_in,
                    bflag_in=bflag_in, split=split)
+        if cls_in:
+            rec.update(c_cls=c_cls, hflag_vox=vox2[1])
         if li == 0:
             bflag_o = ga['bflag2']
             rec.update(c_out=c_o, ybg_out=ybg_o, bflag_out=bflag_o)
@@ -336,7 +350,7 @@
 
 def _wgrad_bg_flops(rec, F):
     din, dout, sd, pd = rec['din'], rec['dout'], rec['sd'], rec['pd']
-    hflag = rec['hflag_in']
+    hflag = rec.get('hflag_vox', rec['hflag_in'])
     co, ci = rec['w'].shape[0], rec['w'].shape[1]
 
     def count():
@@ -355,8 +369,10 @@
     if 'wgrad_bg' in KNOCKOUT:
         return
     fl = _wgrad_bg_flops(rec, F) if _hip.KERNEL_TIMERS is not None else 0
-    _hip.conv3d_wgrad_bg(rec['x'], dz, rec['sd'], rec['pd'], _hip.Background(rec['c_in'], None, rec['hflag_in']), tap_sums,
-                         accumulate_into=_grad_of(rec['w']), split=rec.get('split'), F=F, flops=fl)
+    cls = 'c_cls' in rec
+    bg = _hip.Background(rec['c_cls'], None, rec['hflag_vox']) if cls else _hip.Background(rec['c_in'], None, rec['hflag_in'])
+    _hip.conv3d_wgrad_bg(rec['x'], dz, rec['sd'], rec['pd'], bg, tap_sums, accumulate_into=_grad_of(rec['w']),
+                         split=rec.get('split'), F=F, flops=fl, cls=cls)
 
 
 def _linear_wgrad_side(x, dz, w):
@@ -393,21 +409,24 @@
     else:
         g = _hip.bev_to_cl(gm, D3)
 
-    def tap_sums(dz, tile_flags=None, inactive=None):
+    def tap_sums(name, dz, tile_flags=None, inactive=None, cls=False):
         if 'tap_sums' in KNOCKOUT:
-            return _knocked(dz, (dz.shape[0], 9, dz.shape[3]))
-        return _hip.plane_tap_sums(dz, tile_flags, inactive)
-
-    def tap_sums_side(name, dz, tile_flags=None, inactive=None):
+            return _knocked(dz, (dz.shape[0], 9, dz.shape[3])), (_knocked(dz, (dz.shape[0], 9, 9, dz.shape[3])) if cls else None)
+        if cls:
+            Tt, Tc = _hip.plane_tap_sums_cls(dz)
+            return _mut(name, Tt), _mut(name, Tc)
+        return _mut(name, _hip.plane_tap_sums(dz, tile_flags, inactive)), None
+
+    def tap_sums_side(name, dz, tile_flags=None, inactive=None, cls=False):
         if not _hip.ASYNC_WGRAD or 'tap_sums' in KNOCKOUT:
-            return _mut(name, tap_sums(dz, tile_flags, inactive)), None
+            return tap_sums(name, dz, tile_flags, inactive, cls) + (None,)
         main = torch.cuda.current_stream(dev)
         with _hip._SideStream(dz, tile_flags, inactive):
-            Tt = _mut(name, tap_sums(dz, tile_flags, inactive))
+            Tt, Tc = tap_sums(name, dz, tile_flags, inactive, cls)
             ev = torch.cuda.Event()
             ev.record(torch.cuda.current_stream(dev))
         Tt.record_stream(main)
-        return Tt, ev
+        return Tt, Tc, ev
 
     def dgrad_tiles(rec, dz, bflag):
         split = rec.get('split') or 0
@@ -428,15 +447,15 @@
 
     r3, r2 = S.convs[1], S.convs[0]
     dz3 = bn_relu_backward(g, r3['y'], r3['mi'], fs, X.ROWS_GRID, None, _grad_of(r3['b']))
-    T3, ev3 = tap_sums_side('T3', dz3)
-    _wgrad_bg(r3, dz3, T3, F, H, W)
+    T3, T3c, ev3 = tap_sums_side('T3', dz3, cls='c_cls' in r3)
+    _wgrad_bg(r3, dz3, T3c if T3c is not None else T3, F, H, W)
     g2 = dgrad_tiles(r3, dz3, r3['bflag_in'])
     if ev3 is not None:
         torch.cuda.current_stream(dev).wait_event(ev3)
     A2 = _mut('A2', input_grad_sums(r3, T3))
     dz2, inact2 = bn_bwd_tiles(g2, r2['y'], r2['mi'], r2['c_out'], r2['ybg_out'], A2, r2['bflag_out'], r2['b'], True)
     inact2 = _mut('inact2', inact2)
-    T2, ev2 = tap_sums_side('T2', dz2, r2['bflag_out'], inact2)
+    T2, _, ev2 = tap_sums_side('T2', dz2, r2['bflag_out'], inact2)
     _wgrad_bg(r2, dz2, T2, F, H, W)
     g1 = dgrad_tiles(r2, dz2, r2['bflag_in'])
     if ev2 is not None:
```

Result: no change. 543.3 frames/s, median of 6 (+0.9%).
